# noirmist/Pytorch_Pose_Proposal_Network

Hardware: NVIDIA B200
Metric: PPN decode+NMS+parse images/s (higher is better)
Workload: dtype f32

## Files before the change

### include/ppn_decode_bench.h

```cpp
#ifndef PPN_DECODE_BENCH_H_
#define PPN_DECODE_BENCH_H_

#include "ppn_decode.h"

#ifdef __cplusplus
extern "C" {
#endif

int ppn_profile_enable(int32_t on);
int ppn_profile_read(float* stage_ms , int32_t* n_calls);

int ppn_timeline(void* dev_records, int32_t max_records);

int ppn_debug_argmax_items(const PPNShape* shape, int32_t sms, int32_t* info , int32_t* first, int32_t* size, int32_t max_items);

int ppn_tune(const char* key, int32_t value);
int ppn_tune_get(const char* key, int32_t* value);

#ifdef __cplusplus
}
#endif
#endif
```

### pytorch_pose_proposal_network_b200/_lib.py

```python
from __future__ import annotations

import ctypes as C
import os

from . import build as _build

ABI_VERSION = 7
HEAD_F32, HEAD_F16, HEAD_BF16 = 0, 1, 2
GEMM_TF32, GEMM_F16, GEMM_BF16 = 0, 1, 2
FEAT_NCHW_F32, FEAT_NHWC_16 = 0, 1
FLAG_INPUT_COMPLETE = 1
FLAG_CLEAR_UNUSED = 2
MAX_CELLS = 1024
MAX_CHAINS = 32
MAX_CHAIN_STEPS = 192
IPC_HANDLE_BYTES = 64

i32p = C.POINTER(C.c_int32)
f32p = C.POINTER(C.c_float)
u16p = C.POINTER(C.c_uint16)


class PPNShape(C.Structure):
    _fields_ = [(n, C.c_int32) for n in
                ("B", "K", "E", "H", "W", "sH", "sW", "inW", "inH", "gridW", "gridH", "off_h", "off_w", "head_dtype")]


class PPNParams(C.Structure):
    _fields_ = [("det_thresh", C.c_float), ("nms_thresh", C.c_float), ("min_num_keypoints", C.c_int32),
                ("n_nms_parts", C.c_int32), ("n_chains", C.c_int32), ("flags", C.c_int32),
                ("chain_off", i32p), ("chain_limb", i32p), ("chain_part", i32p)]


class PPNHumans(C.Structure):
    _fields_ = [("count", C.c_void_p), ("root_cell", C.c_void_p), ("part_cell", C.c_void_p),
                ("part_score", C.c_void_p), ("part_box", C.c_void_p), ("R", C.c_int32)]


class PPNHeadOptions(C.Structure):
    _fields_ = [("operand", C.c_int32), ("feat_layout", C.c_int32)]


class PPNPeople(C.Structure):
    _fields_ = [("person_off", C.c_void_p), ("bbox", C.c_void_p), ("keypoints", C.c_void_p),
                ("visible", C.c_void_p), ("size", C.c_void_p)]


TARGET_NAMES = ("delta", "weight", "weight_ij", "tx", "ty", "tx_half", "ty_half", "tw", "th", "te")


class PPNTargets(C.Structure):
    _fields_ = [(n, C.c_void_p) for n in TARGET_NAMES]


class PPNLossOptions(C.Structure):
    _fields_ = [("limb_dtype", C.c_int32)]


EXPORTS = {
    "ppn_abi_version": (C.c_int, []),
    "ppn_strerror": (C.c_char_p, [C.c_int]),
    "ppn_workspace_bytes": (C.c_int, [C.POINTER(PPNShape), C.POINTER(PPNParams), C.POINTER(C.c_size_t)]),
    "ppn_parse_launches": (C.c_int, [C.POINTER(PPNShape), C.POINTER(PPNParams)]),
    "ppn_parse_plan": (C.c_int, [C.POINTER(PPNShape), C.POINTER(PPNParams), i32p]),
    "ppn_limb_argmax": (C.c_int, [C.c_void_p, C.POINTER(PPNShape), C.c_void_p, C.c_void_p]),
    "ppn_limb_stream_probe": (C.c_int, [C.c_void_p, C.POINTER(PPNShape), C.c_void_p, C.c_int32, C.c_void_p]),
    "ppn_decode_candidates": (C.c_int, [C.c_void_p, C.POINTER(PPNShape), C.c_int32, C.c_float,
                                        C.c_void_p, C.c_void_p, C.c_void_p, C.c_void_p, C.c_void_p]),
    "ppn_restore_xy": (C.c_int, [C.c_void_p, C.c_void_p, C.c_void_p, C.c_void_p, C.c_int64, C.POINTER(PPNShape), C.c_void_p]),
    "ppn_restore_size": (C.c_int, [C.c_void_p, C.c_void_p, C.c_void_p, C.c_void_p, C.c_int64, C.POINTER(PPNShape), C.c_void_p]),
    "ppn_nms": (C.c_int, [C.c_void_p, C.c_void_p, C.c_void_p, C.c_int32, C.c_int32, C.c_float, C.c_int32,
                          C.c_void_p, C.c_void_p, C.c_void_p]),
    "ppn_tree_parse": (C.c_int, [C.c_void_p, C.POINTER(PPNShape), C.POINTER(PPNParams), C.c_void_p, C.c_void_p,
                                 C.c_void_p, C.c_void_p, C.POINTER(PPNHumans), C.c_void_p]),
    "ppn_parse": (C.c_int, [C.c_void_p, C.POINTER(PPNShape), C.POINTER(PPNParams), C.POINTER(PPNHumans),
                            C.c_void_p, C.c_size_t, C.c_void_p]),
    "ppn_parse_host_scratch_bytes": (C.c_int, [C.POINTER(PPNShape), C.POINTER(PPNParams), C.c_int32,
                                               C.POINTER(C.c_size_t)]),
    "ppn_parse_host": (C.c_int, [C.c_void_p, C.POINTER(PPNShape), C.POINTER(PPNParams), C.POINTER(PPNHumans),
                                 C.c_void_p, C.c_size_t]),
    "ppn_part_centres": (C.c_int, [C.POINTER(PPNHumans), C.c_int32, C.c_int32, C.c_void_p, C.c_void_p]),
    "ppn_skeleton": (C.c_int, [C.POINTER(PPNHumans), C.c_int32, C.c_int32, C.c_int32, i32p, C.c_void_p, C.c_void_p, C.c_void_p, C.c_void_p]),
    "ppn_packed_bytes": (C.c_int, [C.c_int32, C.c_int32, C.POINTER(C.c_size_t), C.POINTER(C.c_size_t)]),
    "ppn_pack_humans": (C.c_int, [C.POINTER(PPNHumans), C.c_int32, C.c_int32, C.c_int32, C.c_void_p, C.c_size_t, C.c_void_p]),
    "ppn_parse_dense": (C.c_int, [C.c_void_p, C.POINTER(PPNShape), C.POINTER(PPNParams), C.POINTER(PPNHumans),
                                  C.c_void_p, C.c_size_t, C.c_int32, C.c_int32, C.c_void_p, C.c_size_t, C.c_void_p]),
    "ppn_parse_dense_remote": (C.c_int, [C.c_void_p, C.POINTER(PPNShape), C.POINTER(PPNParams), C.POINTER(PPNHumans),
                                         C.c_void_p, C.c_size_t, C.c_void_p, C.c_size_t, C.c_int32, C.c_int32,
                                         C.c_void_p, C.c_size_t, C.c_void_p]),
    "ppn_peer_alloc": (C.c_int, [C.c_size_t, C.POINTER(C.c_void_p), C.c_char_p]),
    "ppn_peer_open": (C.c_int, [C.c_char_p, C.POINTER(C.c_void_p)]),
    "ppn_peer_close": (C.c_int, [C.c_void_p]),
    "ppn_peer_free": (C.c_int, [C.c_void_p]),
    "ppn_peer_copy": (C.c_int, [C.c_void_p, C.c_void_p, C.c_size_t, C.c_void_p]),
    "ppn_peer_post": (C.c_int, [C.c_void_p, C.c_longlong, C.c_void_p]),
    "ppn_peer_wait": (C.c_int, [C.c_void_p, C.c_int32, C.c_longlong, C.c_uint32, C.c_void_p, C.c_void_p]),
    "ppn_head_workspace_bytes": (C.c_int, [C.POINTER(PPNShape), C.POINTER(C.c_size_t)]),
    "ppn_head_gemm_argmax": (C.c_int, [C.c_void_p, C.c_void_p, C.c_void_p, C.c_int32, C.POINTER(PPNShape), C.c_void_p, C.c_void_p,
                                       C.c_void_p, C.c_void_p, C.c_void_p]),
    "ppn_head_parse": (C.c_int, [C.c_void_p, C.c_void_p, C.c_void_p, C.c_int32, C.POINTER(PPNShape), C.POINTER(PPNParams),
                                 C.POINTER(PPNHumans), C.c_void_p, C.c_size_t, C.c_void_p, C.c_void_p, C.c_void_p]),
    "ppn_head_workspace_bytes_opt": (C.c_int, [C.POINTER(PPNShape), C.c_int32, C.POINTER(PPNHeadOptions), C.POINTER(C.c_size_t)]),
    "ppn_head_gemm_argmax_opt": (C.c_int, [C.c_void_p, C.c_void_p, C.c_void_p, C.c_int32, C.POINTER(PPNShape), C.POINTER(PPNHeadOptions),
                                           C.c_void_p, C.c_size_t, C.c_void_p, C.c_void_p, C.c_void_p, C.c_void_p, C.c_void_p]),
    "ppn_head_parse_opt": (C.c_int, [C.c_void_p, C.c_void_p, C.c_void_p, C.c_int32, C.POINTER(PPNShape), C.POINTER(PPNParams),
                                     C.POINTER(PPNHeadOptions), C.POINTER(PPNHumans), C.c_void_p, C.c_size_t, C.c_void_p, C.c_void_p,
                                     C.c_void_p]),
    "ppn_encode_targets": (C.c_int, [C.POINTER(PPNPeople), C.POINTER(PPNShape), i32p, C.POINTER(PPNTargets), C.c_void_p]),
    "ppn_loss_workspace_bytes": (C.c_int, [C.POINTER(PPNShape), C.POINTER(C.c_size_t)]),
    "ppn_loss_forward": (C.c_int, [C.c_void_p, C.POINTER(PPNShape), C.POINTER(PPNTargets), C.c_void_p, C.c_void_p,
                                   C.c_size_t, C.c_void_p]),
    "ppn_loss_backward": (C.c_int, [C.c_void_p, C.POINTER(PPNShape), C.POINTER(PPNTargets), C.c_void_p, C.c_void_p,
                                    C.c_void_p]),
    "ppn_loss_workspace_bytes_opt": (C.c_int, [C.POINTER(PPNShape), C.POINTER(PPNLossOptions), C.POINTER(C.c_size_t)]),
    "ppn_loss_forward_opt": (C.c_int, [C.c_void_p, C.POINTER(PPNShape), C.POINTER(PPNTargets), C.POINTER(PPNLossOptions),
                                       C.c_void_p, C.c_void_p, C.c_size_t, C.c_void_p]),
    "ppn_loss_backward_opt": (C.c_int, [C.c_void_p, C.POINTER(PPNShape), C.POINTER(PPNTargets), C.POINTER(PPNLossOptions),
                                        C.c_void_p, C.c_void_p, C.c_void_p]),
    "ppn_encode_targets_opt": (C.c_int, [C.POINTER(PPNPeople), C.POINTER(PPNShape), i32p, C.POINTER(PPNTargets), C.c_int32,
                                         C.c_void_p]),
    "ppn_loss_forward_logits": (C.c_int, [C.c_void_p, C.POINTER(PPNShape), C.POINTER(PPNTargets), C.POINTER(PPNLossOptions),
                                          C.c_void_p, C.c_void_p, C.c_size_t, C.c_void_p]),
    "ppn_loss_backward_logits": (C.c_int, [C.c_void_p, C.POINTER(PPNShape), C.POINTER(PPNTargets), C.POINTER(PPNLossOptions),
                                           C.c_void_p, C.c_void_p, C.c_void_p]),
    "ppn_sigmoid": (C.c_int, [C.c_void_p, C.c_int32, C.c_void_p, C.c_size_t, C.c_void_p]),
    "ppn_debug_argmax_items": (C.c_int, [C.POINTER(PPNShape), C.c_int32, i32p, i32p, i32p, C.c_int32]),
    "ppn_timeline": (C.c_int, [C.c_void_p, C.c_int32]),
    "ppn_profile_enable": (C.c_int, [C.c_int32]),
    "ppn_profile_read": (C.c_int, [f32p, i32p]),
    "ppn_tune": (C.c_int, [C.c_char_p, C.c_int32]),
    "ppn_tune_get": (C.c_int, [C.c_char_p, i32p]),
}

_lib = None


class PPNError(RuntimeError):
    def __init__(self, code: int, where: str):
        self.code = code
        msg = lib().ppn_strerror(code)
        super().__init__(f"{where}: {msg.decode() if msg else 'error'} (code {code})")


def lib_path() -> str:
    return os.environ.get("PPN_DECODE_LIB", _build.LIB_PATH)


def lib():
    global _lib
    if _lib is not None:
        return _lib
    path = lib_path()
    if not os.path.exists(path):
        raise ImportError(
            f"{path} not found: build it with `python -m pytorch_pose_proposal_network_b200.build` "
            "(needs nvcc); this package has no CPU or PyTorch fallback")
    handle = C.CDLL(path)
    for name, (restype, argtypes) in EXPORTS.items():
        try:
            fn = getattr(handle, name)
        except AttributeError as e:
            raise ImportError(f"{path} does not export {name}") from e
        fn.restype = restype
        fn.argtypes = argtypes
    if handle.ppn_abi_version() != ABI_VERSION:
        raise ImportError(f"{path}: ABI version {handle.ppn_abi_version()} != {ABI_VERSION}")
    _lib = handle
    return _lib


def check(code: int, where: str):
    if code != 0:
        raise PPNError(code, where)


def tune(**knobs):
    for k, v in knobs.items():
        check(lib().ppn_tune(k.replace("_", ".", 1).encode(), int(v)), f"ppn_tune({k})")


def tune_get(key: str) -> int:
    v = C.c_int32()
    check(lib().ppn_tune_get(key.encode(), C.byref(v)), f"ppn_tune_get({key})")
    return v.value


STAGES = ("limb_argmax", "decode_candidates", "nms", "tree_parse")


def profile_enable(on: bool = True):
    check(lib().ppn_profile_enable(1 if on else 0), "ppn_profile_enable")


def profile_read():
    ms = (C.c_float * 4)()
    n = C.c_int32()
    check(lib().ppn_profile_read(ms, C.byref(n)), "ppn_profile_read")
    return dict(zip(STAGES, (float(v) for v in ms))), n.value
```

### pytorch_pose_proposal_network_b200/csrc/ppn_capi.cu

```cuda
#include <algorithm>
#include <cstdio>
#include <cstring>
#include <mutex>

#include "ppn_decode.h"
#include "ppn_decode_bench.h"
#include "ppn_kernels.h"

namespace {

ppn::Tuning g_tuning_shared;
std::mutex g_tune_mu;
ppn::Tuning tuning_now() {
    std::lock_guard<std::mutex> lock(g_tune_mu);
    return g_tuning_shared;
}

constexpr int kStages = 4;
constexpr int kMaxProfiled = 4096;
struct Profile {
    bool on = false;
    int used = 0;
    cudaEvent_t* ev = nullptr;
} g_prof;

inline cudaEvent_t* profile_slot() {
    if (!g_prof.on || g_prof.used >= kMaxProfiled) return nullptr;
    return g_prof.ev + (size_t)(g_prof.used++) * (2 * kStages);
}

struct SideLane {
    cudaStream_t stream = nullptr;
    cudaEvent_t fork = nullptr, join = nullptr;
};
thread_local SideLane t_side[64];

cudaError_t side_lane(SideLane** out) {
    int dev = 0;
    cudaError_t e = cudaGetDevice(&dev);
    if (e != cudaSuccess) return e;
    if (dev < 0 || dev >= 64) return cudaErrorInvalidDevice;
    SideLane& l = t_side[dev];
    if (!l.stream) {
        if ((e = cudaStreamCreateWithFlags(&l.stream, cudaStreamNonBlocking)) != cudaSuccess) return e;
        if ((e = cudaEventCreateWithFlags(&l.fork, cudaEventDisableTiming)) != cudaSuccess) return e;
        if ((e = cudaEventCreateWithFlags(&l.join, cudaEventDisableTiming)) != cudaSuccess) return e;
    }
    *out = &l;
    return cudaSuccess;
}

inline int cuda_rc(cudaError_t e) { return e == cudaSuccess ? PPN_OK : (int)e; }

struct Timeline { unsigned long long* buf = nullptr; int cap = 0, used = 0, phase = 0; } g_timeline;
inline ppn::Geom timeline_slot(ppn::Geom g) {
    if (g_timeline.buf && g_timeline.used < g_timeline.cap) { g.tl = g_timeline.buf; g.tl_slot = g_timeline.used++; g.tl_phase = g_timeline.phase; }
    else g.tl = nullptr;
    return g;
}

int check_shape(const PPNShape* s) {
    if (!s) return PPN_E_BADARG;
    if (s->B < 0 || s->K < 1 || s->E < 0 || s->H < 1 || s->W < 1 || s->sH < 1 || s->sW < 1) return PPN_E_BADARG;
    if (s->inW < 1 || s->inH < 1 || s->gridW < 0 || s->gridH < 0) return PPN_E_BADARG;
    if ((long long)s->sH * s->sW > 65535) return PPN_E_UNSUPPORTED;
    if (s->K > 255 || s->E > 255) return PPN_E_UNSUPPORTED;
    const long long per_img = ((long long)6 * s->K + (long long)s->sH * s->sW * s->E) * s->H * s->W;
    if (per_img > 0x7fffffffLL) return PPN_E_UNSUPPORTED;
    if (s->head_dtype < PPN_HEAD_F32 || s->head_dtype > PPN_HEAD_BF16) return PPN_E_BADARG;
    return PPN_OK;
}

ppn::Geom make_geom(const PPNShape* s) {
    ppn::Geom g;
    g.B = s->B; g.K = s->K; g.E = s->E; g.H = s->H; g.W = s->W; g.HW = s->H * s->W;
    g.sH = s->sH; g.sW = s->sW; g.S = s->sH * s->sW; g.C = 6 * s->K + g.S * s->E;
    g.off_h = s->off_h; g.off_w = s->off_w;
    g.gridW = (float)s->gridW; g.gridH = (float)s->gridH; g.inW = (float)s->inW; g.inH = (float)s->inH;
    g.img_stride = (size_t)g.C * g.HW;
    g.limb_off = (size_t)6 * g.K * g.HW;
    g.tl = nullptr;
    g.tl_slot = 0;
    g.tl_phase = 0;
    auto magic = [](int d) -> uint32_t { return d <= 1 ? 0u : (uint32_t)(((1ull << 32) + d - 1) / d); };
    g.magic_W = magic(g.W);
    g.magic_K = magic(g.K);
    g.dtype = s->head_dtype;
    return g;
}

int make_chains(const PPNShape* s, const PPNParams* p, ppn::ChainTable* ch) {
    if (!p) return PPN_E_BADARG;
    if (p->n_chains < 0 || p->n_chains > PPN_MAX_CHAINS) return PPN_E_CHAINS;
    if (p->n_chains > 0 && (!p->chain_off || !p->chain_limb || !p->chain_part)) return PPN_E_BADARG;
    std::memset(ch, 0, sizeof(*ch));
    ch->n_chains = p->n_chains;
    if (p->n_chains == 0) return PPN_OK;
    if (p->chain_off[0] != 0) return PPN_E_CHAINS;
    for (int c = 0; c < p->n_chains; ++c)
        if (p->chain_off[c + 1] < p->chain_off[c]) return PPN_E_CHAINS;
    const int total = p->chain_off[p->n_chains];
    if (total > PPN_MAX_CHAIN_STEPS) return PPN_E_CHAINS;
    for (int c = 0; c <= p->n_chains; ++c) ch->off[c] = (uint8_t)p->chain_off[c];
    for (int q = 0; q < total; ++q) {
        if (p->chain_limb[q] < 0 || p->chain_limb[q] >= s->E || p->chain_part[q] < 0 || p->chain_part[q] >= s->K)
            return PPN_E_CHAINS;
        ch->limb[q] = (uint8_t)p->chain_limb[q];
        ch->part[q] = (uint8_t)p->chain_part[q];
    }
    int limb_of[256], pred_of[256];
    for (int t = 0; t < 256; ++t) limb_of[t] = pred_of[t] = -1;
    ch->parallel_ok = 1;
    for (int c = 0; c < p->n_chains && ch->parallel_ok; ++c)
        for (int q = p->chain_off[c]; q < p->chain_off[c + 1]; ++q) {
            const int t = p->chain_part[q], e = p->chain_limb[q];
            const int pred = q == p->chain_off[c] ? 0 : p->chain_part[q - 1];
            if (t == 0) { ch->parallel_ok = 0; break; }
            if (limb_of[t] < 0) { limb_of[t] = e; pred_of[t] = pred; }
            else if (limb_of[t] != e || pred_of[t] != pred) { ch->parallel_ok = 0; break; }
        }
    return PPN_OK;
}

inline size_t elem_bytes(const PPNShape* s) { return s->head_dtype == PPN_HEAD_F32 ? 4 : 2; }
inline bool misaligned(const void* p, const PPNShape* s) { return (reinterpret_cast<uintptr_t>(p) & (elem_bytes(s) - 1)) != 0; }

inline size_t align_up(size_t v, size_t a) { return (v + a - 1) / a * a; }

struct Workspace {
    size_t amax, keep_idx, keep_count, total;
};

Workspace carve(const PPNShape* s, int n_parts) {
    Workspace w;
    const size_t B = (size_t)s->B, HW = (size_t)s->H * s->W, P = (size_t)n_parts;
    size_t off = 0;
    auto take = [&](size_t bytes) { const size_t at = off; off = align_up(off + bytes, 256); return at; };
    w.amax = take(B * s->E * HW * sizeof(uint16_t));
    w.keep_idx = take(B * P * HW * sizeof(int32_t));
    w.keep_count = take(B * P * sizeof(int32_t));
    w.total = off;
    return w;
}


int check_params(const PPNShape* s, const PPNParams* p) {
    if (!p) return PPN_E_BADARG;
    if (p->n_nms_parts < 1 || p->n_nms_parts > s->K) return PPN_E_BADARG;
    return PPN_OK;
}

int check_humans(const PPNHumans* h) {
    if (!h || !h->count || !h->root_cell || !h->part_cell || !h->part_score || !h->part_box || h->R < 1) return PPN_E_BADARG;
    return PPN_OK;
}

}

namespace {
struct PackedLayout { size_t header, idcell, score, box, total; };
PackedLayout packed_layout(int B, int cap) {
    PackedLayout l;
    l.header = 0;
    l.idcell = align_up((size_t)(2 + 3 * (size_t)B) * sizeof(int32_t), 256);
    l.score = l.idcell + align_up((size_t)cap * sizeof(uint32_t), 256);
    l.box = l.score + align_up((size_t)cap * sizeof(float), 256);
    l.total = l.box + align_up((size_t)cap * 4 * sizeof(float), 256);
    return l;
}
}

namespace {
int pack_after(const PPNHumans* out, const PPNShape* shape, const ppn::DenseTarget* d, cudaStream_t st) {
    if (out->R > 65536) return PPN_E_UNSUPPORTED;
    return cuda_rc(ppn::launch_pack_humans(out->count, out->part_cell, out->part_score, out->part_box, shape->B, out->R,
                                           shape->K, d->cap, d->header, d->idcell, d->score, d->box, st));
}
}

extern "C" {

int ppn_abi_version(void) { return PPN_ABI_VERSION; }

const char* ppn_strerror(int code) {
    switch (code) {
        case PPN_OK: return "ok";
        case PPN_E_BADARG: return "ppn: bad argument (null pointer, non-positive size or misaligned base)";
        case PPN_E_UNSUPPORTED: return "ppn: shape not supported by the kernels";
        case PPN_E_WORKSPACE: return "ppn: workspace smaller than ppn_workspace_bytes()";
        case PPN_E_CHAINS: return "ppn: track orders too long or indexing outside K/E";
        case PPN_E_NO_DEVICE: return "ppn: no usable CUDA device";
        default: break;
    }
    if (code > 0) return cudaGetErrorString((cudaError_t)code);
    return "ppn: unknown error";
}

int ppn_tune(const char* key, int32_t value) {
    if (!key) return PPN_E_BADARG;
    std::lock_guard<std::mutex> lock(g_tune_mu);
    ppn::Tuning& t = g_tuning_shared;
    if (!std::strcmp(key, "argmax.variant")) t.argmax_variant = value;
    else if (!std::strcmp(key, "argmax.stage_bytes")) t.argmax_stage_bytes = value <= 0 ? 0 : (value < 1024 ? 1024 : value);
    else if (!std::strcmp(key, "argmax.stages")) t.argmax_stages = value < 2 ? 2 : (value > 32 ? 32 : value);
    else if (!std::strcmp(key, "argmax.threads")) t.argmax_threads = value < 32 ? 32 : (value > 992 ? 992 : value);
    else if (!std::strcmp(key, "argmax.ctas_per_sm")) t.argmax_ctas_per_sm = value < 1 ? 1 : (value > 8 ? 8 : value);
    else if (!std::strcmp(key, "argmax.split")) t.argmax_split = value;
    else if (!std::strcmp(key, "argmax.cluster")) t.argmax_cluster = value;
    else if (!std::strcmp(key, "argmax.cluster_ring")) t.argmax_cluster_ring = value != 0;
    else if (!std::strcmp(key, "argmax.smem_cap")) t.argmax_smem_cap = value < 0 ? 0 : value;
    else if (!std::strcmp(key, "parse.overlap")) t.parse_overlap = value < 0 ? 0 : (value > 2 ? 2 : value);
    else if (!std::strcmp(key, "argmax.tail_opt")) t.argmax_tail_opt = value < 0 ? 0 : (value > 8 ? 8 : value);
    else if (!std::strcmp(key, "argmax16.threads")) t.argmax16_threads = value < 32 ? 32 : (value > 992 ? 992 : value);
    else if (!std::strcmp(key, "argmax16.stage_bytes")) t.argmax16_stage_bytes = value < 1024 ? 1024 : value;
    else if (!std::strcmp(key, "argmax.dynamic")) t.argmax_dynamic = value != 0;
    else if (!std::strcmp(key, "parse.stage_all")) t.parse_stage_all = value;
    else if (!std::strcmp(key, "parse.chain_calls")) t.parse_chain_calls = value != 0;
    else if (!std::strcmp(key, "parse.persist")) t.parse_persist = value < 0 ? 0 : (value > 4 ? 4 : value);
    else if (!std::strcmp(key, "parse.k12_threads")) t.parse_k12_threads = value < 0 ? 0 : value;
    else if (!std::strcmp(key, "parse.fused")) t.parse_fused = value < 0 ? -1 : (value != 0);
    else if (!std::strcmp(key, "parse.threads")) t.parse_threads = value;
    else if (!std::strcmp(key, "head.subs")) t.head_subs = (t.head_subs & 0x1300) | (value < 1 ? 0 : (value > 7 ? 7 : value));
    else if (!std::strcmp(key, "head.dry")) t.head_subs = (t.head_subs & 0x10ff) | ((value & 3) << 8);
    else if (!std::strcmp(key, "head.acc")) t.head_subs = (t.head_subs & 0x3ff) | (value == 128 ? 0x1000 : 0);
    else if (!std::strcmp(key, "host.chunk_images")) t.host_chunk_images = value < 1 ? 1 : value;
    else if (!std::strcmp(key, "encode.sweep")) t.encode_sweep = value != 0;
    else if (!std::strcmp(key, "encode.ctas_per_sm")) t.encode_ctas_per_sm = value < 1 ? 1 : (value > 8 ? 8 : value);
    else if (!std::strcmp(key, "nms.blockwise")) ppn::set_nms_blockwise(value);
    else if (!std::strcmp(key, "timeline.phase")) g_timeline.phase = value;
    else return PPN_E_BADARG;
    return PPN_OK;
}

int ppn_tune_get(const char* key, int32_t* value) {
    if (!key || !value) return PPN_E_BADARG;
    const ppn::Tuning t = tuning_now();
    if (!std::strcmp(key, "argmax.variant")) *value = t.argmax_variant;
    else if (!std::strcmp(key, "argmax.stage_bytes")) *value = t.argmax_stage_bytes;
    else if (!std::strcmp(key, "argmax.stages")) *value = t.argmax_stages;
    else if (!std::strcmp(key, "argmax.threads")) *value = t.argmax_threads;
    else if (!std::strcmp(key, "argmax.ctas_per_sm")) *value = t.argmax_ctas_per_sm;
    else if (!std::strcmp(key, "argmax.split")) *value = t.argmax_split;
    else if (!std::strcmp(key, "argmax.cluster")) *value = t.argmax_cluster;
    else if (!std::strcmp(key, "argmax.cluster_ring")) *value = t.argmax_cluster_ring;
    else if (!std::strcmp(key, "argmax.smem_cap")) *value = t.argmax_smem_cap;
    else if (!std::strcmp(key, "parse.overlap")) *value = t.parse_overlap;
    else if (!std::strcmp(key, "argmax.tail_opt")) *value = t.argmax_tail_opt;
    else if (!std::strcmp(key, "argmax16.threads")) *value = t.argmax16_threads;
    else if (!std::strcmp(key, "argmax16.stage_bytes")) *value = t.argmax16_stage_bytes;
    else if (!std::strcmp(key, "argmax.dynamic")) *value = t.argmax_dynamic;
    else if (!std::strcmp(key, "parse.stage_all")) *value = t.parse_stage_all;
    else if (!std::strcmp(key, "parse.chain_calls")) *value = t.parse_chain_calls;
    else if (!std::strcmp(key, "parse.persist")) *value = t.parse_persist;
    else if (!std::strcmp(key, "parse.k12_threads")) *value = t.parse_k12_threads;
    else if (!std::strcmp(key, "parse.fused")) *value = t.parse_fused;
    else if (!std::strcmp(key, "parse.threads")) *value = t.parse_threads;
    else if (!std::strcmp(key, "host.chunk_images")) *value = t.host_chunk_images;
    else if (!std::strcmp(key, "encode.sweep")) *value = t.encode_sweep;
    else if (!std::strcmp(key, "encode.ctas_per_sm")) *value = t.encode_ctas_per_sm;
    else if (!std::strcmp(key, "nms.blockwise")) *value = ppn::get_nms_blockwise();
    else return PPN_E_BADARG;
    return PPN_OK;
}

int ppn_workspace_bytes(const PPNShape* shape, const PPNParams* params, size_t* bytes) {
    int rc = check_shape(shape);
    if (rc) return rc;
    if ((rc = check_params(shape, params))) return rc;
    if (!bytes) return PPN_E_BADARG;
    *bytes = 2 * carve(shape, params->n_nms_parts).total;
    return PPN_OK;
}

int ppn_parse_launches(const PPNShape* shape, const PPNParams* params) {
    const ppn::Tuning g_tuning = tuning_now();
    if (check_shape(shape) || check_params(shape, params)) return 0;
    if (shape->B <= 0) return 0;
    const ppn::Geom g = make_geom(shape);
    ppn::FusedSplit split;
    const bool P1 = params->n_nms_parts == 1 && g_tuning.parse_overlap != 1;
    const bool fits = P1 && ppn::parse_fused_split(g, g_tuning.parse_stage_all, g_tuning, &split);
    const bool fused = P1 && (g_tuning.parse_fused < 0 ? (fits && split.n_sub == 1) : (g_tuning.parse_fused != 0 && ppn::parse_fused_supported(g, g_tuning.parse_stage_all)));
    if (fused) return 2 * (fits ? split.n_sub : 1);
    return 3;
}

int ppn_parse_plan(const PPNShape* shape, const PPNParams* params, int32_t* info) {
    const ppn::Tuning g_tuning = tuning_now();
    if (!info) return PPN_E_BADARG;
    int rc = check_shape(shape);
    if (rc) return rc;
    if ((rc = check_params(shape, params))) return rc;
    info[0] = ppn_parse_launches(shape, params);
    info[1] = 1; info[2] = 0; info[3] = 0;
    if (shape->B <= 0) return PPN_OK;
    ppn::FusedSplit split;
    if (params->n_nms_parts == 1 && ppn::parse_fused_split(make_geom(shape), g_tuning.parse_stage_all, g_tuning, &split)) {
        info[1] = split.n_sub;
        info[2] = (int32_t)split.ring_cap;
        info[3] = split.staged ? 1 : 0;
    }
    return PPN_OK;
}

int ppn_limb_argmax(const void* head, const PPNShape* shape, uint16_t* amax, void* stream) {
    const ppn::Tuning g_tuning = tuning_now();
    int rc = check_shape(shape);
    if (rc) return rc;
    if (shape->B == 0 || shape->E == 0) return PPN_OK;
    if (!head || !amax) return PPN_E_BADARG;
    if (misaligned(head, shape)) return PPN_E_BADARG;
    return cuda_rc(ppn::launch_limb_argmax(head, amax, make_geom(shape), g_tuning, (cudaStream_t)stream));
}

int ppn_limb_stream_probe(const void* head, const PPNShape* shape, uint16_t* amax, int32_t smem_cap, void* stream) {
    const ppn::Tuning g_tuning = tuning_now();
    int rc = check_shape(shape);
    if (rc) return rc;
    if (shape->B == 0 || shape->E == 0) return PPN_OK;
    if (!head || !amax) return PPN_E_BADARG;
    if (misaligned(head, shape)) return PPN_E_BADARG;
    ppn::Tuning t = g_tuning;
    t.argmax_dry = 1;
    t.argmax_cluster = 0;
    if (smem_cap > 0) t.argmax_smem_cap = smem_cap;
    return cuda_rc(ppn::launch_limb_argmax(head, amax, make_geom(shape), t, (cudaStream_t)stream));
}

int ppn_decode_candidates(const void* head, const PPNShape* shape, int32_t n_parts, float det_thresh,
                          int32_t* cand_cell, float* cand_score, float* cand_box, int32_t* cand_count, void* stream) {
    int rc = check_shape(shape);
    if (rc) return rc;
    if (n_parts < 1 || n_parts > shape->K) return PPN_E_BADARG;
    if (shape->B == 0) return PPN_OK;
    if (!head || !cand_cell || !cand_score || !cand_box || !cand_count) return PPN_E_BADARG;
    if (reinterpret_cast<uintptr_t>(cand_box) & 15) return PPN_E_BADARG;
    return cuda_rc(ppn::launch_decode_candidates(head, make_geom(shape), n_parts, det_thresh, cand_cell, cand_score,
                                                 cand_box, cand_count, (cudaStream_t)stream));
}

int ppn_restore_xy(const float* x, const float* y, float* rx, float* ry, int64_t n_planes, const PPNShape* shape, void* stream) {
    int rc = check_shape(shape);
    if (rc) return rc;
    if (n_planes < 0) return PPN_E_BADARG;
    if (n_planes == 0) return PPN_OK;
    if (!x || !y || !rx || !ry) return PPN_E_BADARG;
    return cuda_rc(ppn::launch_restore_xy(x, y, rx, ry, (size_t)n_planes * shape->H * shape->W, shape->H, shape->W,
                                          (float)shape->gridW, (float)shape->gridH, (cudaStream_t)stream));
}

int ppn_restore_size(const float* w, const float* h, float* rw, float* rh, int64_t n_planes, const PPNShape* shape, void* stream) {
    int rc = check_shape(shape);
    if (rc) return rc;
    if (n_planes < 0) return PPN_E_BADARG;
    if (n_planes == 0) return PPN_OK;
    if (!w || !h || !rw || !rh) return PPN_E_BADARG;
    return cuda_rc(ppn::launch_restore_size(w, h, rw, rh, (size_t)n_planes * shape->H * shape->W, (float)shape->inW,
                                            (float)shape->inH, (cudaStream_t)stream));
}

int ppn_nms(const float* box, const float* score, const int32_t* count, int32_t n_problems, int32_t stride,
            float nms_thresh, int32_t limit, int32_t* keep_idx, int32_t* keep_count, void* stream) {
    if (n_problems < 0 || stride < 1) return PPN_E_BADARG;
    if (n_problems == 0) return PPN_OK;
    if (!box || !count || !keep_idx || !keep_count) return PPN_E_BADARG;
    if (reinterpret_cast<uintptr_t>(box) & 15) return PPN_E_BADARG;
    return cuda_rc(ppn::launch_nms(box, score, count, n_problems, stride, nms_thresh, limit, keep_idx, keep_count,
                                   (cudaStream_t)stream));
}

int ppn_tree_parse(const void* head, const PPNShape* shape, const PPNParams* params, const uint16_t* amax,
                   const int32_t* cand_cell, const int32_t* keep_idx, const int32_t* keep_count,
                   const PPNHumans* out, void* stream) {
    int rc = check_shape(shape);
    if (rc) return rc;
    if ((rc = check_params(shape, params))) return rc;
    if ((rc = check_humans(out))) return rc;
    ppn::ChainTable ch;
    if ((rc = make_chains(shape, params, &ch))) return rc;
    if (shape->B == 0) return PPN_OK;
    if (!head || !keep_idx || !keep_count || (!amax && shape->E > 0)) return PPN_E_BADARG;
    if ((long long)shape->H * shape->W > PPN_MAX_CELLS) return PPN_E_UNSUPPORTED;
    if (reinterpret_cast<uintptr_t>(out->part_box) & 15) return PPN_E_BADARG;
    return cuda_rc(ppn::launch_tree_parse(head, make_geom(shape), ch, params->det_thresh, params->min_num_keypoints,
                                          params->n_nms_parts, amax, cand_cell, keep_idx, keep_count, out->count,
                                          out->root_cell, out->part_cell, out->part_score, out->part_box, out->R,
                                          (cudaStream_t)stream));
}

namespace {
__global__ void peer_post_kernel(long long* counter, long long value) {
    __threadfence_system();
    asm volatile("st.release.sys.global.u64 [%0], %1;" :: "l"(counter), "l"(value) : "memory");
}
__global__ void peer_wait_kernel(const long long* counters, int n, long long target, unsigned long long timeout_ns, int* timed_out) {
    const int r = threadIdx.x;
    if (r >= n) return;
    unsigned long long t0, t;
    asm volatile("mov.u64 %0, %%globaltimer;" : "=l"(t0));
    for (;;) {
        long long v;
        asm volatile("ld.acquire.sys.global.u64 %0, [%1];" : "=l"(v) : "l"(counters + r) : "memory");
        if (v >= target) return;
        asm volatile("mov.u64 %0, %%globaltimer;" : "=l"(t));
        if (t - t0 > timeout_ns) { if (timed_out) *timed_out = 1; return; }
        __nanosleep(200);
    }
}
}

int ppn_peer_post(void* counter, long long value, void* stream) {
    if (!counter || (reinterpret_cast<uintptr_t>(counter) & 7)) return PPN_E_BADARG;
    peer_post_kernel<<<1, 1, 0, (cudaStream_t)stream>>>(static_cast<long long*>(counter), value);
    return cuda_rc(cudaGetLastError());
}

int ppn_peer_wait(const void* counters, int32_t n, long long target, uint32_t timeout_ms, int32_t* timed_out, void* stream) {
    if (!counters || n < 1 || n > 1024 || (reinterpret_cast<uintptr_t>(counters) & 7)) return PPN_E_BADARG;
    peer_wait_kernel<<<1, (n + 31) / 32 * 32, 0, (cudaStream_t)stream>>>(static_cast<const long long*>(counters), n, target,
                                                                      (unsigned long long)timeout_ms * 1000000ull, timed_out);
    return cuda_rc(cudaGetLastError());
}

static int parse_impl(const void* head, const PPNShape* shape, const PPNParams* params, const PPNHumans* out,
                      void* workspace, size_t workspace_bytes, void* stream, const ppn::DenseTarget* dense);

int ppn_parse(const void* head, const PPNShape* shape, const PPNParams* params, const PPNHumans* out,
              void* workspace, size_t workspace_bytes, void* stream) {
    return parse_impl(head, shape, params, out, workspace, workspace_bytes, stream, nullptr);
}

int ppn_parse_dense(const void* head, const PPNShape* shape, const PPNParams* params, const PPNHumans* out,
                    void* packed, size_t packed_bytes, int32_t cap_entries, int32_t skip_slots,
                    void* workspace, size_t workspace_bytes, void* stream) {
    int rc = check_shape(shape);
    if (rc) return rc;
    if (cap_entries < 0) return PPN_E_BADARG;
    if (shape->K > 65535 || (long long)shape->H * shape->W > 65536) return PPN_E_UNSUPPORTED;
    if (shape->B == 0) return PPN_OK;
    if (!packed || (reinterpret_cast<uintptr_t>(packed) & 255)) return PPN_E_BADARG;
    const PackedLayout l = packed_layout(shape->B, cap_entries);
    if (packed_bytes < l.total) return PPN_E_WORKSPACE;
    unsigned char* p = static_cast<unsigned char*>(packed);
    ppn::DenseTarget d;
    d.header = reinterpret_cast<int32_t*>(p + l.header);
    d.idcell = reinterpret_cast<uint32_t*>(p + l.idcell);
    d.score = reinterpret_cast<float*>(p + l.score);
    d.box = reinterpret_cast<float*>(p + l.box);
    d.cap = cap_entries;
    d.skip_slots = skip_slots != 0;
    return parse_impl(head, shape, params, out, workspace, workspace_bytes, stream, &d);
}

int ppn_parse_dense_remote(const void* head, const PPNShape* shape, const PPNParams* params, const PPNHumans* out,
                           void* local_header, size_t local_header_bytes, void* remote_packed, size_t remote_bytes,
                           int32_t cap_entries, int32_t skip_slots, void* workspace, size_t workspace_bytes, void* stream) {
    int rc = check_shape(shape);
    if (rc) return rc;
    if (cap_entries < 0) return PPN_E_BADARG;
    if (shape->K > 32 || (long long)shape->H * shape->W > PPN_MAX_CELLS) return PPN_E_UNSUPPORTED;
    if (shape->B == 0) return PPN_OK;
    if (!local_header || !remote_packed || (reinterpret_cast<uintptr_t>(local_header) & 255) ||
        (reinterpret_cast<uintptr_t>(remote_packed) & 255)) return PPN_E_BADARG;
    const PackedLayout l = packed_layout(shape->B, cap_entries);
    if (remote_bytes < l.total || local_header_bytes < (size_t)(2 + 3 * (size_t)shape->B) * sizeof(int32_t)) return PPN_E_WORKSPACE;
    unsigned char* p = static_cast<unsigned char*>(remote_packed);
    ppn::DenseTarget d;
    d.header = static_cast<int32_t*>(local_header);
    d.rheader = reinterpret_cast<int32_t*>(p + l.header);
    d.idcell = reinterpret_cast<uint32_t*>(p + l.idcell);
    d.score = reinterpret_cast<float*>(p + l.score);
    d.box = reinterpret_cast<float*>(p + l.box);
    d.cap = cap_entries;
    d.skip_slots = skip_slots != 0;
    return parse_impl(head, shape, params, out, workspace, workspace_bytes, stream, &d);
}

int ppn_peer_alloc(size_t bytes, void** dev_ptr, unsigned char* handle) {
    if (!dev_ptr || !handle || bytes == 0) return PPN_E_BADARG;
    static_assert(sizeof(cudaIpcMemHandle_t) == PPN_IPC_HANDLE_BYTES, "IPC handle size");
    void* p = nullptr;
    cudaError_t e = cudaMalloc(&p, bytes);
    if (e != cudaSuccess) return (int)e;
    if ((e = cudaMemset(p, 0, bytes)) != cudaSuccess) { cudaFree(p); return (int)e; }
    cudaIpcMemHandle_t h;
    if ((e = cudaIpcGetMemHandle(&h, p)) != cudaSuccess) { cudaFree(p); return (int)e; }
    std::memcpy(handle, &h, sizeof(h));
    *dev_ptr = p;
    return PPN_OK;
}

int ppn_peer_open(const unsigned char* handle, void** dev_ptr) {
    if (!dev_ptr || !handle) return PPN_E_BADARG;
    cudaIpcMemHandle_t h;
    std::memcpy(&h, handle, sizeof(h));
    return cuda_rc(cudaIpcOpenMemHandle(dev_ptr, h, cudaIpcMemLazyEnablePeerAccess));
}

int ppn_peer_close(void* dev_ptr) { return dev_ptr ? cuda_rc(cudaIpcCloseMemHandle(dev_ptr)) : PPN_E_BADARG; }
int ppn_peer_free(void* dev_ptr) { return dev_ptr ? cuda_rc(cudaFree(dev_ptr)) : PPN_E_BADARG; }

int ppn_peer_copy(void* dst, const void* src, size_t bytes, void* stream) {
    if (!dst || !src) return PPN_E_BADARG;
    if (bytes == 0) return PPN_OK;
    return cuda_rc(cudaMemcpyAsync(dst, src, bytes, cudaMemcpyDefault, (cudaStream_t)stream));
}

static int parse_impl(const void* head, const PPNShape* shape, const PPNParams* params, const PPNHumans* out,
                      void* workspace, size_t workspace_bytes, void* stream, const ppn::DenseTarget* dense) {
    const ppn::Tuning g_tuning = tuning_now();
    int rc = check_shape(shape);
    if (rc) return rc;
    if ((rc = check_params(shape, params))) return rc;
    if ((rc = check_humans(out))) return rc;
    ppn::ChainTable ch;
    if ((rc = make_chains(shape, params, &ch))) return rc;
    if (shape->B == 0) return PPN_OK;
    if (!head || !workspace) return PPN_E_BADARG;
    if (misaligned(head, shape) || (reinterpret_cast<uintptr_t>(workspace) & 255)) return PPN_E_BADARG;
    if ((long long)shape->H * shape->W > PPN_MAX_CELLS) return PPN_E_UNSUPPORTED;
    if (reinterpret_cast<uintptr_t>(out->part_box) & 15) return PPN_E_BADARG;
    const int P = params->n_nms_parts;
    const Workspace w = carve(shape, P);
    if (workspace_bytes < 2 * w.total) return PPN_E_WORKSPACE;
    unsigned char* ws = static_cast<unsigned char*>(workspace) + (ppn::next_call_parity((cudaStream_t)stream) ? w.total : 0);
    uint16_t* amax = reinterpret_cast<uint16_t*>(ws + w.amax);
    int32_t* keep_idx = reinterpret_cast<int32_t*>(ws + w.keep_idx);
    int32_t* keep_count = reinterpret_cast<int32_t*>(ws + w.keep_count);
    const ppn::Geom g = make_geom(shape);
    cudaStream_t st = (cudaStream_t)stream;
    cudaError_t e;
    if ((params->flags & PPN_FLAG_CLEAR_UNUSED) && !(dense && dense->skip_slots)) {
        const size_t slots = (size_t)shape->B * out->R, SK = slots * shape->K;
        if ((e = cudaMemsetAsync(out->root_cell, 0xFF, slots * sizeof(int32_t), st)) != cudaSuccess) return (int)e;
        if ((e = cudaMemsetAsync(out->part_cell, 0xFF, SK * sizeof(int32_t), st)) != cudaSuccess) return (int)e;
        if ((e = cudaMemsetAsync(out->part_score, 0, SK * sizeof(float), st)) != cudaSuccess) return (int)e;
        if ((e = cudaMemsetAsync(out->part_box, 0, SK * 4 * sizeof(float), st)) != cudaSuccess) return (int)e;
        ppn::chain_break(st);
    }
    cudaEvent_t* ev = profile_slot();
    const int mode = ev ? 0 : g_tuning.parse_overlap;
    ppn::FusedSplit split;
    const bool fits_beside = P == 1 && ppn::parse_fused_split(g, g_tuning.parse_stage_all, g_tuning, &split);
    const bool fused = P == 1 && mode != 1 && (g_tuning.parse_fused < 0 ? (fits_beside && split.n_sub == 1) : (g_tuning.parse_fused != 0 &&
                       ppn::parse_fused_supported(g, g_tuning.parse_stage_all)));
    const bool dense_fused = dense && fused && shape->K <= 32;
    if (dense && dense->rheader && !dense_fused) return PPN_E_UNSUPPORTED;
    if (fused) {
        using namespace ppn;
        Tuning tuning = g_tuning;
        const int n_sub = fits_beside ? split.n_sub : 1;
        const int sub_B = fits_beside ? split.sub_B : g.B;
        const int staged_forced = fits_beside ? (split.staged ? 1 : 0) : -1;
        if (fits_beside) tuning.argmax_smem_cap = (int)split.ring_cap;
        const bool overlap_calls = (params->flags & PPN_FLAG_INPUT_COMPLETE) != 0;
        const bool chain = mode == 2 && g_tuning.parse_chain_calls != 0;
        cudaStreamCaptureStatus cap = cudaStreamCaptureStatusNone;
        if ((e = cudaStreamIsCapturing(st, &cap)) != cudaSuccess) return (int)e;
        const bool capturing = cap != cudaStreamCaptureStatusNone;
        const size_t es = elem_bytes(shape);
        const size_t K = (size_t)shape->K, R = (size_t)out->R;
        auto launch_k3 = [&](int j) -> cudaError_t {
            Geom gj = timeline_slot(g);
            const int b0 = j * sub_B;
            gj.B = std::min(sub_B, g.B - b0);
            const bool attr = chain && (j > 0 || !overlap_calls || capturing || chain_clean(st));
            const int bits = mode != 2 ? 0 : ((overlap_calls || j > 0) ? (PDL_TRIGGER | PDL_WAIT_END) : (PDL_WAIT_START | PDL_TRIGGER));
            bool chained = false, zeroed = false;
            int32_t* zero2 = (dense_fused && j == 0) ? dense->header : nullptr;
            cudaError_t err = launch_limb_argmax(static_cast<const unsigned char*>(head) + (size_t)b0 * g.img_stride * es,
                                                 amax + (size_t)b0 * g.E * g.HW, gj, tuning, st, attr, &chained, bits, zero2, &zeroed);
            if (err == cudaSuccess && zero2 && !zeroed) err = cudaMemsetAsync(dense->header, 0, 2 * sizeof(int32_t), st);
            return err;
        };
        auto launch_k124 = [&](int j) -> cudaError_t {
            Geom gj = timeline_slot(g);
            const int b0 = j * sub_B;
            gj.B = std::min(sub_B, g.B - b0);
            DenseTarget dj;
            if (dense_fused) { dj = *dense; dj.B_total = g.B; dj.b0 = b0; }
            return launch_parse_fused(static_cast<const unsigned char*>(head) + (size_t)b0 * g.img_stride * es, gj, ch,
                                      params->det_thresh, params->nms_thresh, params->min_num_keypoints,
                                      amax + (size_t)b0 * g.E * g.HW, out->count + b0, out->root_cell + (size_t)b0 * R,
                                      out->part_cell + (size_t)b0 * R * K, out->part_score + (size_t)b0 * R * K,
                                      out->part_box + (size_t)b0 * R * K * 4, out->R, st,
                                      mode == 2 ,
                                      (overlap_calls && chain && !capturing) ? 2 : 1, g_tuning.parse_stage_all, staged_forced,
                                      dense_fused ? &dj : nullptr);
        };
        if (ev) {
            cudaEventRecord(ev[0], st);
            for (int j = 0; j < n_sub; ++j) if ((e = launch_k3(j)) != cudaSuccess) return (int)e;
            cudaEventRecord(ev[1], st);
            for (int q = 2; q < 7; ++q) cudaEventRecord(ev[q], st);
            for (int j = 0; j < n_sub; ++j) if ((e = launch_k124(j)) != cudaSuccess) return (int)e;
            cudaEventRecord(ev[7], st);
        } else {
            for (int j = 0; j < n_sub; ++j) {
                if ((e = launch_k3(j)) != cudaSuccess) return (int)e;
                if ((e = launch_k124(j)) != cudaSuccess) return (int)e;
            }
        }
        if (dense && !dense_fused) return pack_after(out, shape, dense, st);
        return PPN_OK;
    }
    if (dense && dense->rheader) return PPN_E_UNSUPPORTED;
    if (mode == 2) {
        using namespace ppn;
        const bool overlap_calls = (params->flags & PPN_FLAG_INPUT_COMPLETE) != 0;
        const bool chain_calls = g_tuning.parse_chain_calls != 0;
        cudaStreamCaptureStatus cap = cudaStreamCaptureStatusNone;
        if ((e = cudaStreamIsCapturing(st, &cap)) != cudaSuccess) return (int)e;
        const bool capturing = cap != cudaStreamCaptureStatusNone;
        Tuning tuning = g_tuning;
        int k12_ctas = g_tuning.parse_persist, k4_ctas = g_tuning.parse_persist > 0 ? 1 : 0;
        if (k12_ctas > 0) {
            const size_t ring_cap = chain3_ring_cap(g, g_tuning.parse_stage_all, k12_ctas);
            if (ring_cap) tuning.argmax_smem_cap = (int)ring_cap;
            else k12_ctas = k4_ctas = 0;
        }
        const bool early = overlap_calls && chain_calls && !capturing && k4_ctas > 0;
        const bool attr12 = chain_calls && (!overlap_calls || capturing || chain_clean(st));
        const int bits12 = PDL_TRIGGER | (!attr12 ? 0 : (overlap_calls ? PDL_WAIT_END : PDL_WAIT_START));
        bool chained = false;
        if ((e = launch_decode_nms(head, timeline_slot(g), P, params->det_thresh, params->nms_thresh, keep_idx, keep_count, st, attr12,
                                   bits12, k12_ctas, g_tuning.parse_k12_threads)) != cudaSuccess) return (int)e;
        if ((e = launch_limb_argmax(head, amax, timeline_slot(g), tuning, st, true, &chained)) != cudaSuccess) return (int)e;
        if ((e = launch_tree_parse(head, timeline_slot(g), ch, params->det_thresh, params->min_num_keypoints, P, amax, nullptr, keep_idx,
                                   keep_count, out->count, out->root_cell, out->part_cell, out->part_score, out->part_box,
                                   out->R, st, chained, chained ? (PDL_WAIT_START | PDL_TRIGGER) : 0, g_tuning.parse_stage_all,
                                   g_tuning.parse_threads, chained ? (early ? 2 : 1) : 0, k4_ctas)) != cudaSuccess) return (int)e;
        if (!chained) chain_break(st);
        if (!dense) return PPN_OK;
        rc = pack_after(out, shape, dense, st);
        chain_break(st);
        return rc;
    }
    ppn::chain_break(st);
    cudaStream_t side = st;
    SideLane* lane = nullptr;
    if (mode == 1) {
        if ((e = side_lane(&lane)) != cudaSuccess) return (int)e;
        side = lane->stream;
        if ((e = cudaEventRecord(lane->fork, st)) != cudaSuccess) return (int)e;
        if ((e = cudaStreamWaitEvent(side, lane->fork, 0)) != cudaSuccess) return (int)e;
    }
    if (ev) cudaEventRecord(ev[0], st);
    if ((e = ppn::launch_limb_argmax(head, amax, g, g_tuning, st)) != cudaSuccess) return (int)e;
    if (ev) cudaEventRecord(ev[1], st);
    if (ev) { cudaEventRecord(ev[2], side); cudaEventRecord(ev[3], side); cudaEventRecord(ev[4], side); }
    if ((e = ppn::launch_decode_nms(head, g, P, params->det_thresh, params->nms_thresh, keep_idx, keep_count, side)) != cudaSuccess) return (int)e;
    if (ev) cudaEventRecord(ev[5], side);
    if (lane) {
        if ((e = cudaEventRecord(lane->join, side)) != cudaSuccess) return (int)e;
        if ((e = cudaStreamWaitEvent(st, lane->join, 0)) != cudaSuccess) return (int)e;
    }
    if (ev) cudaEventRecord(ev[6], st);
    if ((e = ppn::launch_tree_parse(head, g, ch, params->det_thresh, params->min_num_keypoints, P, amax, nullptr ,
                                    keep_idx, keep_count, out->count, out->root_cell, out->part_cell, out->part_score,
                                    out->part_box, out->R, st, false, 0, g_tuning.parse_stage_all, g_tuning.parse_threads)) != cudaSuccess) return (int)e;
    if (ev) cudaEventRecord(ev[7], st);
    return dense ? pack_after(out, shape, dense, st) : PPN_OK;
}

namespace {
struct HeadWorkspace { size_t dec, amax, keys, total; };
HeadWorkspace carve_head(const PPNShape* s) {
    HeadWorkspace w;
    const size_t B = (size_t)s->B, HW = (size_t)s->H * s->W;
    w.dec = 0;
    w.amax = align_up(B * 6 * s->K * HW * sizeof(float), 256);
    w.keys = w.amax + align_up(B * s->E * HW * sizeof(uint16_t), 256);
    w.total = w.keys + align_up(B * s->E * HW * sizeof(unsigned long long), 256);
    return w;
}
int check_head(const float* feat, const float* weight, int32_t Cin, const PPNShape* s) {
    if ((long long)s->H * s->W > 65536) return PPN_E_UNSUPPORTED;
    if (Cin < 32 || Cin % 32 != 0 || (s->H * s->W) % 4 != 0) return PPN_E_UNSUPPORTED;
    if (s->head_dtype != PPN_HEAD_F32) return PPN_E_UNSUPPORTED;
    if (!feat || !weight) return PPN_E_BADARG;
    if ((reinterpret_cast<uintptr_t>(feat) & 15) || (reinterpret_cast<uintptr_t>(weight) & 15)) return PPN_E_BADARG;
    return PPN_OK;
}
}

int ppn_head_workspace_bytes(const PPNShape* shape, size_t* bytes) {
    int rc = check_shape(shape);
    if (rc) return rc;
    if (!bytes) return PPN_E_BADARG;
    *bytes = carve_head(shape).total;
    return PPN_OK;
}

int ppn_head_gemm_argmax(const float* feat, const float* weight, const float* bias, int32_t Cin, const PPNShape* shape,
                         float* dec, uint16_t* amax, float* emit_logits, float* emit_head, void* stream) {
    const ppn::Tuning g_tuning = tuning_now();
    int rc = check_shape(shape);
    if (rc) return rc;
    if (shape->B == 0) return PPN_OK;
    if ((rc = check_head(feat, weight, Cin, shape))) return rc;
    if (!dec || (!amax && shape->E > 0) || (reinterpret_cast<uintptr_t>(bias) & 15)) return PPN_E_BADARG;
    const ppn::Geom g = make_geom(shape);
    cudaStream_t st = (cudaStream_t)stream;
    void* keys = nullptr;
    cudaError_t e = cudaMallocAsync(&keys, std::max<size_t>(ppn::head_keys_bytes(g), 256), st);
    if (e != cudaSuccess) return cuda_rc(e);
    e = ppn::launch_head_gemm_argmax(feat, weight, bias, Cin, g, dec, amax, static_cast<unsigned long long*>(keys), emit_logits,
                                     emit_head, st, false, 0, g_tuning.head_subs);
    const cudaError_t e2 = cudaFreeAsync(keys, st);
    return cuda_rc(e != cudaSuccess ? e : e2);
}

namespace {
struct HeadWorkspaceOpt { size_t dec, amax, keys, xt, wt, total; };
bool opt_16bit(const PPNHeadOptions* o) { return o->operand == PPN_GEMM_F16 || o->operand == PPN_GEMM_BF16; }
int check_head_opt(const void* feat, const float* weight, int32_t Cin, const PPNShape* s, const PPNHeadOptions* o) {
    if (!o) return PPN_E_BADARG;
    if (o->operand < PPN_GEMM_TF32 || o->operand > PPN_GEMM_BF16) return PPN_E_BADARG;
    if (o->feat_layout != PPN_FEAT_NCHW_F32 && o->feat_layout != PPN_FEAT_NHWC_16) return PPN_E_BADARG;
    if (!opt_16bit(o) && o->feat_layout != PPN_FEAT_NCHW_F32) return PPN_E_UNSUPPORTED;
    if (s->B == 0) return PPN_OK;
    if (!opt_16bit(o)) return check_head(static_cast<const float*>(feat), weight, Cin, s);
    if (s->head_dtype != PPN_HEAD_F32) return PPN_E_UNSUPPORTED;
    if (!ppn::head16_supported(Cin, make_geom(s))) return PPN_E_UNSUPPORTED;
    if (!feat || !weight) return PPN_E_BADARG;
    if ((reinterpret_cast<uintptr_t>(feat) & 15) || (reinterpret_cast<uintptr_t>(weight) & 15)) return PPN_E_BADARG;
    return PPN_OK;
}
HeadWorkspaceOpt carve_head_opt(const PPNShape* s, int32_t Cin, const PPNHeadOptions* o) {
    const HeadWorkspace w = carve_head(s);
    HeadWorkspaceOpt r;
    r.dec = w.dec; r.amax = w.amax; r.keys = w.keys; r.xt = r.wt = r.total = w.total;
    if (opt_16bit(o)) {
        const ppn::Geom g = make_geom(s);
        r.wt = r.xt + (o->feat_layout == PPN_FEAT_NCHW_F32 ? align_up(ppn::head16_packed_feat_bytes(Cin, g), 1024) : 0);
        r.total = r.wt + align_up(ppn::head16_packed_weight_bytes(Cin, g), 1024);
    }
    return r;
}
}

int ppn_head_workspace_bytes_opt(const PPNShape* shape, int32_t Cin, const PPNHeadOptions* opt, size_t* bytes) {
    int rc = check_shape(shape);
    if (rc) return rc;
    if (!bytes || !opt || Cin < 1) return PPN_E_BADARG;
    *bytes = carve_head_opt(shape, Cin, opt).total;
    return PPN_OK;
}

int ppn_head_gemm_argmax_opt(const void* feat, const float* weight, const float* bias, int32_t Cin, const PPNShape* shape,
                             const PPNHeadOptions* opt, void* workspace, size_t workspace_bytes,
                             float* dec, uint16_t* amax, float* emit_logits, float* emit_head, void* stream) {
    int rc = check_shape(shape);
    if (rc) return rc;
    if ((rc = check_head_opt(feat, weight, Cin, shape, opt))) return rc;
    if (!opt_16bit(opt))
        return ppn_head_gemm_argmax(static_cast<const float*>(feat), weight, bias, Cin, shape, dec, amax, emit_logits, emit_head, stream);
    if (shape->B == 0) return PPN_OK;
    if (!dec || (!amax && shape->E > 0) || (reinterpret_cast<uintptr_t>(bias) & 15)) return PPN_E_BADARG;
    if (!workspace || (reinterpret_cast<uintptr_t>(workspace) & 255)) return PPN_E_BADARG;
    const HeadWorkspaceOpt w = carve_head_opt(shape, Cin, opt);
    if (workspace_bytes < w.total) return PPN_E_WORKSPACE;
    unsigned char* ws = static_cast<unsigned char*>(workspace);
    return cuda_rc(ppn::launch_head_gemm16_argmax(feat, opt->feat_layout == PPN_FEAT_NCHW_F32, weight, bias, Cin,
                                                  opt->operand == PPN_GEMM_BF16, make_geom(shape), ws + w.xt, ws + w.wt, dec, amax,
                                                  reinterpret_cast<unsigned long long*>(ws + w.keys), emit_logits, emit_head,
                                                  (cudaStream_t)stream, 0, tuning_now().head_subs));
}

int ppn_head_parse_opt(const void* feat, const float* weight, const float* bias, int32_t Cin, const PPNShape* shape,
                       const PPNParams* params, const PPNHeadOptions* opt, const PPNHumans* out, void* workspace,
                       size_t workspace_bytes, float* emit_logits, float* emit_head, void* stream) {
    const ppn::Tuning g_tuning = tuning_now();
    int rc = check_shape(shape);
    if (rc) return rc;
    if ((rc = check_params(shape, params))) return rc;
    if ((rc = check_humans(out))) return rc;
    ppn::ChainTable ch;
    if ((rc = make_chains(shape, params, &ch))) return rc;
    if ((rc = check_head_opt(feat, weight, Cin, shape, opt))) return rc;
    if (shape->B == 0) return PPN_OK;
    if (!workspace || (reinterpret_cast<uintptr_t>(workspace) & 255)) return PPN_E_BADARG;
    if (params->n_nms_parts != 1 || (long long)shape->H * shape->W > PPN_MAX_CELLS) return PPN_E_UNSUPPORTED;
    if ((reinterpret_cast<uintptr_t>(out->part_box) & 15) || (reinterpret_cast<uintptr_t>(bias) & 15)) return PPN_E_BADARG;
// ... 125 lines not shown
    a.sweep = g_tuning.encode_sweep;
    a.sweep_ctas_per_sm = g_tuning.encode_ctas_per_sm;
    a.magic_sW = shape->sW <= 1 ? 0u : (uint32_t)(((1ull << 32) + shape->sW - 1) / shape->sW);
    a.gridW = (float)shape->gridW; a.gridH = (float)shape->gridH;
    a.inW = (double)shape->inW; a.inH = (double)shape->inH;
    int dev = 0, sms = 0;
    cudaError_t e = cudaGetDevice(&dev);
    if (e != cudaSuccess) return (int)e;
    if ((e = cudaDeviceGetAttribute(&sms, cudaDevAttrMultiProcessorCount, dev)) != cudaSuccess) return (int)e;
    return cuda_rc(ppn::launch_encode_targets(a, shape->B, sms, (cudaStream_t)stream));
}

namespace {
inline bool bad_ptr(const void* p, size_t align) { return !p || (reinterpret_cast<uintptr_t>(p) & (align - 1)); }
inline bool bad_f32(const void* p) { return bad_ptr(p, 4); }
inline size_t dtype_bytes(int32_t dtype) { return dtype == PPN_HEAD_F32 ? 4 : 2; }

int check_loss_types(const PPNShape* shape, const PPNLossOptions* opt) {
    if (!opt || opt->limb_dtype < PPN_HEAD_F32 || opt->limb_dtype > PPN_HEAD_BF16) return PPN_E_BADARG;
    if (opt->limb_dtype != PPN_HEAD_F32 && opt->limb_dtype != shape->head_dtype) return PPN_E_UNSUPPORTED;
    return PPN_OK;
}

int loss_args(const void* head, const PPNShape* shape, const PPNTargets* t, const PPNLossOptions* opt, ppn::LossArgs* a) {
    int rc = check_shape(shape);
    if (rc) return rc;
    if ((rc = check_loss_types(shape, opt))) return rc;
    if (shape->B < 1) return PPN_E_BADARG;
    std::memset(a, 0, sizeof(*a));
    const ppn::Geom g = make_geom(shape);
    a->B = g.B; a->K = g.K; a->W = g.W; a->HW = g.HW; a->L = g.S * g.E * g.HW;
    a->img_stride = g.img_stride; a->limb_off = g.limb_off;
    a->gW = g.gridW; a->gH = g.gridH; a->inW = g.inW; a->inH = g.inH;
    a->head_dtype = shape->head_dtype;
    a->limb_dtype = opt->limb_dtype;
    ppn::loss_plan(a);
    if (!t) return PPN_E_BADARG;
    const float* small[] = {t->delta, t->weight, t->tx, t->ty, t->tx_half, t->ty_half, t->tw, t->th};
    for (const float* p : small)
        if (bad_f32(p)) return PPN_E_BADARG;
    const size_t limb_align = dtype_bytes(opt->limb_dtype);
    if (bad_ptr(head, elem_bytes(shape)) || (a->L > 0 && (bad_ptr(t->te, limb_align) || bad_ptr(t->weight_ij, limb_align))))
        return PPN_E_BADARG;
    a->head = head;
    a->delta = t->delta; a->weight = t->weight; a->weight_ij = t->weight_ij; a->tx = t->tx; a->ty = t->ty;
    a->tx_half = t->tx_half; a->ty_half = t->ty_half; a->tw = t->tw; a->th = t->th; a->te = t->te;
    return PPN_OK;
}

int sm_count(int* sms) {
    int dev = 0;
    cudaError_t e = cudaGetDevice(&dev);
    if (e == cudaSuccess) e = cudaDeviceGetAttribute(sms, cudaDevAttrMultiProcessorCount, dev);
    return cuda_rc(e);
}

const PPNLossOptions kLossF32 = {PPN_HEAD_F32};
int check_f32_loss(const PPNShape* shape) {
    int rc = check_shape(shape);
    if (rc) return rc;
    return shape->head_dtype != PPN_HEAD_F32 ? PPN_E_UNSUPPORTED : PPN_OK;
}
}

int ppn_loss_workspace_bytes_opt(const PPNShape* shape, const PPNLossOptions* opt, size_t* bytes) {
    int rc = check_shape(shape);
    if (rc) return rc;
    if (!bytes) return PPN_E_BADARG;
    if ((rc = check_loss_types(shape, opt))) return rc;
    if (shape->B < 1) return PPN_E_BADARG;
    ppn::LossArgs a;
    std::memset(&a, 0, sizeof(a));
    a.B = shape->B; a.K = shape->K; a.HW = shape->H * shape->W; a.L = shape->sH * shape->sW * shape->E * a.HW;
    ppn::loss_plan(&a);
    *bytes = ppn::loss_workspace_bytes(a);
    return PPN_OK;
}

int ppn_loss_workspace_bytes(const PPNShape* shape, size_t* bytes) {
    int rc = check_shape(shape);
    if (rc) return rc;
    if (!bytes) return PPN_E_BADARG;
    if ((rc = check_f32_loss(shape))) return rc;
    return ppn_loss_workspace_bytes_opt(shape, &kLossF32, bytes);
}

namespace {
int loss_forward(const void* head, const PPNShape* shape, const PPNTargets* targets, const PPNLossOptions* opt,
                 float* loss, void* workspace, size_t workspace_bytes, void* stream, bool from_logits) {
    ppn::LossArgs a;
    int rc = loss_args(head, shape, targets, opt, &a);
    if (rc) return rc;
    if (bad_f32(loss) || !workspace || (reinterpret_cast<uintptr_t>(workspace) & 7)) return PPN_E_BADARG;
    if (workspace_bytes < ppn::loss_workspace_bytes(a)) return PPN_E_WORKSPACE;
    a.partial = static_cast<double*>(workspace);
    int sms = 0;
    if ((rc = sm_count(&sms))) return rc;
    return cuda_rc(ppn::launch_loss_forward(a, loss, sms, (cudaStream_t)stream, from_logits));
}

int loss_backward(const void* head, const PPNShape* shape, const PPNTargets* targets, const PPNLossOptions* opt,
                  const float* grad_loss, void* grad_head, void* stream, bool from_logits) {
    ppn::LossArgs a;
    int rc = loss_args(head, shape, targets, opt, &a);
    if (rc) return rc;
    if (bad_f32(grad_loss) || bad_ptr(grad_head, elem_bytes(shape))) return PPN_E_BADARG;
    a.grad_loss = grad_loss;
    a.grad = grad_head;
    int sms = 0;
    if ((rc = sm_count(&sms))) return rc;
    return cuda_rc(ppn::launch_loss_backward(a, sms, (cudaStream_t)stream, from_logits));
}
}

int ppn_loss_forward_opt(const void* head, const PPNShape* shape, const PPNTargets* targets, const PPNLossOptions* opt,
                         float* loss, void* workspace, size_t workspace_bytes, void* stream) {
    return loss_forward(head, shape, targets, opt, loss, workspace, workspace_bytes, stream, false);
}

int ppn_loss_forward(const float* head, const PPNShape* shape, const PPNTargets* targets, float* loss,
                     void* workspace, size_t workspace_bytes, void* stream) {
    const int rc = check_f32_loss(shape);
    return rc ? rc : ppn_loss_forward_opt(head, shape, targets, &kLossF32, loss, workspace, workspace_bytes, stream);
}

int ppn_loss_backward_opt(const void* head, const PPNShape* shape, const PPNTargets* targets, const PPNLossOptions* opt,
                          const float* grad_loss, void* grad_head, void* stream) {
    return loss_backward(head, shape, targets, opt, grad_loss, grad_head, stream, false);
}

int ppn_loss_backward(const float* head, const PPNShape* shape, const PPNTargets* targets, const float* grad_loss,
                      float* grad_head, void* stream) {
    const int rc = check_f32_loss(shape);
    return rc ? rc : ppn_loss_backward_opt(head, shape, targets, &kLossF32, grad_loss, grad_head, stream);
}

int ppn_loss_forward_logits(const void* logits, const PPNShape* shape, const PPNTargets* targets, const PPNLossOptions* opt,
                            float* loss, void* workspace, size_t workspace_bytes, void* stream) {
    return loss_forward(logits, shape, targets, opt, loss, workspace, workspace_bytes, stream, true);
}

int ppn_loss_backward_logits(const void* logits, const PPNShape* shape, const PPNTargets* targets, const PPNLossOptions* opt,
                             const float* grad_loss, void* grad_logits, void* stream) {
    return loss_backward(logits, shape, targets, opt, grad_loss, grad_logits, stream, true);
}

int ppn_sigmoid(const void* x, int32_t x_dtype, float* y, size_t n, void* stream) {
    if (x_dtype < PPN_HEAD_F32 || x_dtype > PPN_HEAD_BF16) return PPN_E_BADARG;
    if (n == 0) return PPN_OK;
    if (bad_ptr(x, dtype_bytes(x_dtype)) || bad_f32(y)) return PPN_E_BADARG;
    return cuda_rc(ppn::launch_sigmoid(x, x_dtype, y, n, (cudaStream_t)stream));
}

int ppn_debug_argmax_items(const PPNShape* shape, int32_t sms, int32_t* info, int32_t* first, int32_t* size, int32_t max_items) {
    int rc = check_shape(shape);
    if (rc) return rc;
    if (!info || sms < 1) return PPN_E_BADARG;
    const ppn::Tuning g_tuning = tuning_now();
    ppn::ArgmaxPlan p;
    if (!ppn::plan_argmax(make_geom(shape), g_tuning, sms, &p) || !p.split_mats) return PPN_E_UNSUPPORTED;
    struct Ctx { int32_t* first; int32_t* size; int32_t max; } ctx = {first, size, max_items};
    int n_items = 0;
    ppn::argmax_item_partition(p, shape->B * shape->E, &n_items, [](void* c, int it, int m0, int nm) -> int {
        Ctx* x = static_cast<Ctx*>(c);
        if (x->first && x->size && it < x->max) { x->first[it] = m0; x->size[it] = nm; }
        return 0;
    }, &ctx);
    info[0] = p.G; info[1] = p.n_big; info[2] = p.small_m; info[3] = n_items;
    return PPN_OK;
}

int ppn_timeline(void* dev_records, int32_t max_records) {
    g_timeline.buf = static_cast<unsigned long long*>(dev_records);
    g_timeline.cap = dev_records ? max_records : 0;
    g_timeline.used = 0;
    return PPN_OK;
}

int ppn_profile_enable(int32_t on) {
    if (on && !g_prof.ev) {
        g_prof.ev = new cudaEvent_t[(size_t)kMaxProfiled * (2 * kStages)];
        for (size_t i = 0; i < (size_t)kMaxProfiled * (2 * kStages); ++i) {
            cudaError_t e = cudaEventCreate(&g_prof.ev[i]);
            if (e != cudaSuccess) return (int)e;
        }
    }
    g_prof.on = on != 0;
    g_prof.used = 0;
    return PPN_OK;
}

int ppn_profile_read(float* stage_ms, int32_t* n_calls) {
    if (!stage_ms || !n_calls) return PPN_E_BADARG;
    for (int s = 0; s < kStages; ++s) stage_ms[s] = 0.0f;
    *n_calls = g_prof.used;
    for (int c = 0; c < g_prof.used; ++c) {
        cudaEvent_t* ev = g_prof.ev + (size_t)c * (2 * kStages);
        cudaError_t e = cudaEventSynchronize(ev[2 * kStages - 1]);
        if (e != cudaSuccess) return (int)e;
        for (int s = 0; s < kStages; ++s) {
            float ms = 0.0f;
            if ((e = cudaEventElapsedTime(&ms, ev[2 * s], ev[2 * s + 1])) != cudaSuccess) return (int)e;
            stage_ms[s] += ms;
        }
    }
    g_prof.used = 0;
    return PPN_OK;
}

namespace {
struct HostPlan {
    int chunk;
    size_t head_bytes;
    size_t ws_bytes;
    size_t off_head[2], off_ws[2], off_count, off_root, off_cell, off_score, off_box, total;
};
HostPlan plan_host(const PPNShape* s, const PPNParams* p, int R) {
    const ppn::Tuning g_tuning = tuning_now();
    HostPlan h;
    h.chunk = g_tuning.host_chunk_images;
    if (h.chunk > s->B) h.chunk = s->B > 0 ? s->B : 1;
    PPNShape cs = *s;
    cs.B = h.chunk;
    const size_t per_img = ((size_t)6 * s->K + (size_t)s->sH * s->sW * s->E) * s->H * s->W * elem_bytes(s);
    h.head_bytes = align_up(per_img * h.chunk, 256);
    h.ws_bytes = 2 * carve(&cs, p->n_nms_parts).total;
    size_t off = 0;
    auto take = [&](size_t bytes) { const size_t at = off; off = align_up(off + bytes, 256); return at; };
    h.off_head[0] = take(h.head_bytes); h.off_head[1] = take(h.head_bytes);
    h.off_ws[0] = take(h.ws_bytes); h.off_ws[1] = take(h.ws_bytes);
    const size_t B = (size_t)s->B, K = (size_t)s->K;
    h.off_count = take(B * sizeof(int32_t));
    h.off_root = take(B * R * sizeof(int32_t));
    h.off_cell = take(B * R * K * sizeof(int32_t));
    h.off_score = take(B * R * K * sizeof(float));
    h.off_box = take(B * R * K * 4 * sizeof(float));
    h.total = off;
    return h;
}
}

int ppn_parse_host_scratch_bytes(const PPNShape* shape, const PPNParams* params, int32_t R, size_t* bytes) {
    int rc = check_shape(shape);
    if (rc) return rc;
    if ((rc = check_params(shape, params))) return rc;
    if (!bytes || R < 1) return PPN_E_BADARG;
    *bytes = plan_host(shape, params, R).total;
    return PPN_OK;
}

int ppn_parse_host(const void* head_host, const PPNShape* shape, const PPNParams* params, const PPNHumans* out_host,
                   void* dev_scratch, size_t dev_scratch_bytes) {
    int rc = check_shape(shape);
    if (rc) return rc;
    if ((rc = check_params(shape, params))) return rc;
    if ((rc = check_humans(out_host))) return rc;
    if (shape->B == 0) return PPN_OK;
    if (!head_host || !dev_scratch || (reinterpret_cast<uintptr_t>(dev_scratch) & 255)) return PPN_E_BADARG;
    const int R = out_host->R;
    const HostPlan h = plan_host(shape, params, R);
    if (dev_scratch_bytes < h.total) return PPN_E_WORKSPACE;
    unsigned char* d = static_cast<unsigned char*>(dev_scratch);
    const size_t K = (size_t)shape->K;
    const size_t per_img_b = ((size_t)6 * shape->K + (size_t)shape->sH * shape->sW * shape->E) * shape->H * shape->W * elem_bytes(shape);

    struct HostLane { cudaStream_t s[2] = {nullptr, nullptr}; };
    static thread_local HostLane t_lanes[64];
    int dev = 0;
    cudaError_t e = cudaGetDevice(&dev);
    if (e != cudaSuccess) return (int)e;
    if (dev < 0 || dev >= 64) return (int)cudaErrorInvalidDevice;
    cudaStream_t* streams = t_lanes[dev].s;
    for (int i = 0; i < 2; ++i)
        if (!streams[i] && (e = cudaStreamCreateWithFlags(&streams[i], cudaStreamNonBlocking)) != cudaSuccess) return (int)e;
    auto fail = [&](int code) { cudaStreamSynchronize(streams[0]); cudaStreamSynchronize(streams[1]); return code; };

    int32_t* d_count = reinterpret_cast<int32_t*>(d + h.off_count);
    int32_t* d_root = reinterpret_cast<int32_t*>(d + h.off_root);
    int32_t* d_cell = reinterpret_cast<int32_t*>(d + h.off_cell);
    float* d_score = reinterpret_cast<float*>(d + h.off_score);
    float* d_box = reinterpret_cast<float*>(d + h.off_box);

    PPNParams chunk_params = *params;
    chunk_params.flags &= ~PPN_FLAG_INPUT_COMPLETE;
    int slot = 0;
    for (int b0 = 0; b0 < shape->B; b0 += h.chunk, slot ^= 1) {
        const int nb = (shape->B - b0 < h.chunk) ? shape->B - b0 : h.chunk;
        cudaStream_t st = streams[slot];
        void* d_head = d + h.off_head[slot];
        if ((e = cudaMemcpyAsync(d_head, static_cast<const unsigned char*>(head_host) + (size_t)b0 * per_img_b,
                                 (size_t)nb * per_img_b, cudaMemcpyHostToDevice, st)) != cudaSuccess) return fail((int)e);
        PPNShape cs = *shape;
        cs.B = nb;
        PPNHumans dev_out;
        dev_out.count = d_count + b0;
        dev_out.root_cell = d_root + (size_t)b0 * R;
        dev_out.part_cell = d_cell + (size_t)b0 * R * K;
        dev_out.part_score = d_score + (size_t)b0 * R * K;
        dev_out.part_box = d_box + (size_t)b0 * R * K * 4;
        dev_out.R = R;
        if ((rc = ppn_parse(d_head, &cs, &chunk_params, &dev_out, d + h.off_ws[slot], h.ws_bytes, st))) return fail(rc);
        if ((e = cudaMemcpyAsync(out_host->count + b0, dev_out.count, (size_t)nb * sizeof(int32_t), cudaMemcpyDeviceToHost, st)) != cudaSuccess) return fail((int)e);
    }
    for (int i = 0; i < 2; ++i)
        if ((e = cudaStreamSynchronize(streams[i])) != cudaSuccess) return (int)e;
    int m = 0;
    for (int b = 0; b < shape->B; ++b) m = std::max(m, std::min(out_host->count[b], R));
    if (m > 0) {
        cudaStream_t st = streams[0];
        const size_t B = (size_t)shape->B;
        if ((e = cudaMemcpy2DAsync(out_host->root_cell, (size_t)R * 4, d_root, (size_t)R * 4, (size_t)m * 4, B, cudaMemcpyDeviceToHost, st)) != cudaSuccess) return fail((int)e);
        if ((e = cudaMemcpy2DAsync(out_host->part_cell, (size_t)R * K * 4, d_cell, (size_t)R * K * 4, (size_t)m * K * 4, B, cudaMemcpyDeviceToHost, st)) != cudaSuccess) return fail((int)e);
        if ((e = cudaMemcpy2DAsync(out_host->part_score, (size_t)R * K * 4, d_score, (size_t)R * K * 4, (size_t)m * K * 4, B, cudaMemcpyDeviceToHost, st)) != cudaSuccess) return fail((int)e);
        if ((e = cudaMemcpy2DAsync(out_host->part_box, (size_t)R * K * 16, d_box, (size_t)R * K * 16, (size_t)m * K * 16, B, cudaMemcpyDeviceToHost, st)) != cudaSuccess) return fail((int)e);
        if ((e = cudaStreamSynchronize(st)) != cudaSuccess) return (int)e;
    }
    if ((params->flags & PPN_FLAG_CLEAR_UNUSED) && m < R) {
        const size_t tail = (size_t)(R - m);
        for (size_t b = 0; b < (size_t)shape->B; ++b) {
            const size_t s = b * R + m;
            std::fill_n(out_host->root_cell + s, tail, -1);
            std::fill_n(out_host->part_cell + s * K, tail * K, -1);
            std::fill_n(out_host->part_score + s * K, tail * K, 0.0f);
            std::fill_n(out_host->part_box + s * K * 4, tail * K * 4, 0.0f);
        }
    }
    return PPN_OK;
}
// ... 3 lines not shown
```

### pytorch_pose_proposal_network_b200/csrc/ppn_device.cuh

```cuda
#pragma once
#include <cuda_bf16.h>
#include <cuda_fp16.h>
#include <cuda_runtime.h>
#include <stdint.h>

namespace ppn {

struct ChainTable {
    int32_t n_chains;
    int32_t parallel_ok;
    uint8_t off[33];
    uint8_t limb[192];
    uint8_t part[192];
};

struct Geom {
    int32_t B, K, E, H, W, HW, sH, sW, S, C;
    int32_t off_h, off_w;
    float gridW, gridH, inW, inH;
    size_t img_stride;
    size_t limb_off;
    uint32_t magic_W, magic_K;
    int32_t dtype;
    unsigned long long* tl;
    int32_t tl_slot;
    int32_t tl_phase;
};

enum : int { TL_START = 0, TL_END = 1, TL_WAITED = 2 };
__device__ __forceinline__ void tl_mark(const Geom& g, int what) {
    if (g.tl && threadIdx.x == 0) {
        unsigned long long t;
        asm volatile("mov.u64 %0, %%globaltimer;" : "=l"(t));
        unsigned long long* rec = g.tl + 4 * (size_t)g.tl_slot;
        if (what == TL_END) atomicMax(rec + 1, t); else atomicMin(rec + what, t);
    }
}

__device__ __forceinline__ void tl_phase(const Geom& g, int phase) {
    if (g.tl && threadIdx.x == 0 && g.tl_phase == phase) {
        unsigned long long t;
        asm volatile("mov.u64 %0, %%globaltimer;" : "=l"(t));
        if (phase >= 100) atomicMax(g.tl + 4 * (size_t)g.tl_slot + 3, t);
        else atomicMin(g.tl + 4 * (size_t)g.tl_slot + 3, t);
    }
}

__device__ __forceinline__ void tl_phase_warp(const Geom& g, int phase) {
    if (g.tl && (threadIdx.x & 31) == 0 && g.tl_phase == phase) {
        unsigned long long t;
        asm volatile("mov.u64 %0, %%globaltimer;" : "=l"(t));
        atomicMin(g.tl + 4 * (size_t)g.tl_slot + 3, t);
    }
}

enum HeadDtype : int { HEAD_F32 = 0, HEAD_F16 = 1, HEAD_BF16 = 2 };

__device__ __forceinline__ float widen(float v) { return v; }
__device__ __forceinline__ float widen(__half v) { return __half2float(v); }
__device__ __forceinline__ float widen(__nv_bfloat16 v) { return __bfloat162float(v); }

template <typename T>
__device__ __forceinline__ float ldf(const T* p) { return widen(__ldg(p)); }

template <typename T> __device__ __forceinline__ T narrow(float v) { return v; }
template <> __device__ __forceinline__ __half narrow<__half>(float v) { return __float2half_rn(v); }
template <> __device__ __forceinline__ __nv_bfloat16 narrow<__nv_bfloat16>(float v) { return __float2bfloat16_rn(v); }
__device__ __forceinline__ uint32_t bits16(__half v) { return __half_as_ushort(v); }
__device__ __forceinline__ uint32_t bits16(__nv_bfloat16 v) { return __bfloat16_as_ushort(v); }
template <typename T> __device__ __forceinline__ uint32_t pack2(float lo, float hi) {
    return bits16(narrow<T>(lo)) | (bits16(narrow<T>(hi)) << 16);
}

__device__ __forceinline__ float sigmoid_f32(float x) { return __fdiv_rn(1.0f, __fadd_rn(1.0f, expf(-x))); }

template <typename T>
__device__ __forceinline__ float delta_at(const T* __restrict__ img, const Geom& g, int k, int c) {
    return __fmul_rn(ldf(img + (size_t)k * g.HW + c), ldf(img + (size_t)(g.K + k) * g.HW + c));
}

__device__ __forceinline__ float4 box_from(float x, float y, float bw, float bh, int h, int w, const Geom& g) {
    const float rx = __fmul_rn(__fadd_rn(x, (float)w), g.gridW);
    const float ry = __fmul_rn(__fadd_rn(y, (float)h), g.gridH);
    const float hw = __fmul_rn(__fmul_rn(g.inW, bw), 0.5f);
    const float hh = __fmul_rn(__fmul_rn(g.inH, bh), 0.5f);
    return make_float4(__fsub_rn(ry, hh), __fsub_rn(rx, hw), __fadd_rn(ry, hh), __fadd_rn(rx, hw));
}

template <typename T>
__device__ __forceinline__ float4 box_at(const T* __restrict__ img, const Geom& g, int k, int c) {
    const int h = c / g.W, w = c - h * g.W;
    const size_t HW = g.HW;
    return box_from(ldf(img + (size_t)(2 * g.K + k) * HW + c), ldf(img + (size_t)(3 * g.K + k) * HW + c),
                    ldf(img + (size_t)(4 * g.K + k) * HW + c), ldf(img + (size_t)(5 * g.K + k) * HW + c), h, w, g);
}

__device__ __forceinline__ float np_max(float a, float b) { return (a >= b || a != a) ? a : b; }
__device__ __forceinline__ float np_min(float a, float b) { return (a <= b || a != a) ? a : b; }

__device__ __forceinline__ bool suppresses(const float4 tested, float area_tested,
                                           const float4 kept, float area_kept, float thr, bool thr_positive) {
    const float tly = np_max(tested.x, kept.x), tlx = np_max(tested.y, kept.y);
    const float bry = np_min(tested.z, kept.z), brx = np_min(tested.w, kept.w);
    const bool overlap = tly < bry && tlx < brx;
    if (thr_positive && !overlap) return false;
    const float prod = __fmul_rn(__fsub_rn(bry, tly), __fsub_rn(brx, tlx));
    const float inter = __fmul_rn(prod, overlap ? 1.0f : 0.0f);
    const float iou = __fdiv_rn(inter, __fsub_rn(__fadd_rn(area_tested, area_kept), inter));
    return iou >= thr;
}

__device__ __forceinline__ float box_area(const float4 b) {
    return __fmul_rn(__fsub_rn(b.z, b.x), __fsub_rn(b.w, b.y));
}

__device__ __forceinline__ void argmax_step(float& best, int& idx, float v, int a) {
    const bool take = !(v <= best) && (best == best);
    best = take ? v : best;
    idx = take ? a : idx;
}

__device__ __forceinline__ bool argmax_beats(float v2, int i2, float v1, int i1) {
    const bool n1 = v1 != v1, n2 = v2 != v2;
    if (n1 || n2) return n2 && (!n1 || i2 < i1);
    return v2 > v1 || (v2 == v1 && i2 < i1);
}

__device__ __forceinline__ uint32_t smem_u32(const void* p) {
    return static_cast<uint32_t>(__cvta_generic_to_shared(p));
}
__device__ __forceinline__ void mbar_init(uint64_t* bar, uint32_t count) {
    asm volatile("mbarrier.init.shared::cta.b64 [%0], %1;" ::"r"(smem_u32(bar)), "r"(count) : "memory");
}
__device__ __forceinline__ void fence_mbar_init() {
    asm volatile("fence.mbarrier_init.release.cluster;" ::: "memory");
}
__device__ __forceinline__ void mbar_arrive_expect_tx(uint64_t* bar, uint32_t bytes) {
    asm volatile("mbarrier.arrive.expect_tx.shared::cta.b64 _, [%0], %1;" ::"r"(smem_u32(bar)), "r"(bytes) : "memory");
}
__device__ __forceinline__ void mbar_arrive(uint64_t* bar) {
    asm volatile("mbarrier.arrive.shared::cta.b64 _, [%0];" ::"r"(smem_u32(bar)) : "memory");
}
__device__ __forceinline__ void mbar_wait(uint64_t* bar, uint32_t parity) {
    asm volatile(
        "{\n"
        ".reg .pred p;\n"
        "PPN_WAIT:\n"
        "mbarrier.try_wait.parity.shared::cta.b64 p, [%0], %1;\n"
        "@p bra PPN_DONE;\n"
        "bra PPN_WAIT;\n"
        "PPN_DONE:\n"
        "}" ::"r"(smem_u32(bar)), "r"(parity) : "memory");
}
__device__ __forceinline__ void bulk_g2s(void* dst_smem, const void* src_gmem, uint32_t bytes, uint64_t* bar) {
    const uint64_t evict_first = 0x12F0000000000000ull;
    asm volatile(
        "cp.async.bulk.shared::cluster.global.mbarrier::complete_tx::bytes.L2::cache_hint [%0], [%1], %2, [%3], %4;"
        ::"r"(smem_u32(dst_smem)), "l"(src_gmem), "r"(bytes), "r"(smem_u32(bar)), "l"(evict_first) : "memory");
}
enum : int {
    PDL_TRIGGER = 1,
    PDL_WAIT_START = 2,
    PDL_WAIT_END = 4,
};
__device__ __forceinline__ void pdl_launch_dependents() { asm volatile("griddepcontrol.launch_dependents;" ::: "memory"); }
__device__ __forceinline__ void pdl_wait() { asm volatile("griddepcontrol.wait;" ::: "memory"); }

__device__ __forceinline__ void bulk_prefetch_l2(const void* src_gmem, uint32_t bytes) {
    asm volatile("cp.async.bulk.prefetch.L2.global [%0], %1;" ::"l"(src_gmem), "r"(bytes) : "memory");
}
__device__ __forceinline__ void named_bar_sync(int id, int n_threads) {
    asm volatile("bar.sync %0, %1;" ::"r"(id), "r"(n_threads) : "memory");
}
__device__ __forceinline__ float4 ldg_stream(const float4* p) {
    float4 v;
    asm volatile("ld.global.nc.L1::no_allocate.v4.f32 {%0, %1, %2, %3}, [%4];"
                 : "=f"(v.x), "=f"(v.y), "=f"(v.z), "=f"(v.w) : "l"(p));
    return v;
}

}
```

### pytorch_pose_proposal_network_b200/csrc/ppn_kernels.cu

```cuda
#include <algorithm>
#include <atomic>
#include <mutex>

#include "ppn_kernels.h"

namespace ppn {


struct Partial { float v; int32_t i; };

__host__ __device__ __forceinline__ int item_first(const ArgmaxPlan& p, int item) {
    return item < p.n_big ? item * p.G : p.n_big * p.G + (item - p.n_big) * p.small_m;
}
__host__ __device__ __forceinline__ int item_size(const ArgmaxPlan& p, int item) { return item < p.n_big ? p.G : p.small_m; }
__host__ __device__ __forceinline__ int item_count(const ArgmaxPlan& p, int n_mats) {
    const int rest = n_mats - p.n_big * p.G;
    return p.n_big + (rest + p.small_m - 1) / p.small_m;
}

__global__ void __launch_bounds__(1024, 1)
limb_argmax_tma_kernel(const float* __restrict__ head, uint16_t* __restrict__ amax, Geom g, ArgmaxPlan p, int pdl,
                       int* __restrict__ ticket, int32_t* __restrict__ zero2) {
    extern __shared__ __align__(128) unsigned char smem[];
    unsigned char* ring = smem;
// ... 960 lines not shown
                            }
                        } else {
                            for (int q = seen; q < m_pub; ++q) {
                                const float4 kb = kall[q];
                                hit |= suppresses_finite(bj, aj, kb, box_area(kb), thr, thr_pos);
                            }
                        }
                        dead = hit;
                    }
                    seen = m_pub;
                }
                if (wd >= w) break;
            }
            if (fin) break;
            if (tg) { if (w == 0) tl_phase_warp(*tg, 14); else if (w == 1) tl_phase_warp(*tg, 16); }
            unsigned und = ~__ballot_sync(0xffffffffu, dead);
            unsigned kept = 0u;
            while (und) {
                const bool mine = (und >> lane) & 1u;
                const bool killed = mine && (col & kept) != 0u;
                const bool free_ = mine && !killed && (col & und) == 0u;
                const unsigned k = __ballot_sync(0xffffffffu, free_);
                const unsigned d = __ballot_sync(0xffffffffu, killed);
                kept |= k;
                und &= ~(k | d);
            }
            bool done = false;
            if (limit > 0 && seen + __popc(kept) >= limit) {
                int need = limit - seen;
                unsigned trimmed = 0u;
                for (unsigned rest = kept; need > 0 && rest; --need) { const unsigned low = rest & (0u - rest); trimmed |= low; rest ^= low; }
                kept = trimmed;
                done = true;
            }
            if ((kept >> lane) & 1u) {
                const int idx = s.sidx[i0 + lane];
                const int pos = seen + __popc(kept & ((1u << lane) - 1u));
                out[pos] = map ? map[idx] : idx;
                kall[pos] = bj;
            }
            __syncwarp();
            if (lane == 0)
                st_release_cta_shared(&s.ctl[0], ((done || w == Wd - 1) ? 0x80000000u : 0u) | ((unsigned)(w + 1) << 16) |
                                                     (unsigned)(seen + __popc(kept)));
            if (tg) {
                if (w == 0) tl_phase_warp(*tg, 15); else if (w == 1) tl_phase_warp(*tg, 17); else if (w == 2) tl_phase_warp(*tg, 18);
                if (w == Wd - 1) tl_phase_warp(*tg, 19);
            }
            if (done) break;
        }
        __syncthreads();
        return s.ctl[0] & 0xffff;
    }
    int m = 0;
    for (int w = 0; w < Wd; ++w) {
        const int i0 = w << 5;
        if (warp == 0) {
            unsigned cur = s.rem[w];
            const int nb = min(32, n - i0);
            const unsigned valid = nb == 32 ? 0xffffffffu : ((1u << nb) - 1u);
            const unsigned diag = (lane < nb) ? s.diag[i0 + lane] : 0u;
            unsigned kept = 0;
            unsigned open = ~cur & valid;
            if (__popc(open) <= kNmsWalkMax) {
                while (open) {
                    const int t = __ffs((int)open) - 1;
                    kept |= 1u << t;
                    open &= ~(__shfl_sync(0xffffffffu, diag, t) | (1u << t));
                }
            } else {
#pragma unroll
                for (int t = 0; t < 32; ++t) {
                    const unsigned d = __shfl_sync(0xffffffffu, diag, t);
                    const unsigned take = (~cur >> t) & 1u;
                    kept |= take << t;
                    cur |= d & (0u - take);
                }
                kept &= valid;
            }
            bool done = false;
            if (limit > 0 && m + __popc(kept) >= limit) {
                int need = limit - m;
                unsigned trimmed = 0;
                for (unsigned rest = kept; need > 0 && rest; --need) { const unsigned low = rest & (0u - rest); trimmed |= low; rest ^= low; }
                kept = trimmed;
                done = true;
            }
            if ((kept >> lane) & 1u) {
                const int idx = s.sidx[i0 + lane];
                const int pos = __popc(kept & ((1u << lane) - 1u));
                out[m + pos] = map ? map[idx] : idx;
                s.kbox[pos] = s.sbox[i0 + lane];
                s.karea[pos] = s.sarea[i0 + lane];
            }
            if (lane == 0) { s.ctl[0] = (int)kept; s.ctl[1] = m + __popc(kept); s.ctl[2] = done || w == Wd - 1; }
        }
        __syncthreads();
        const unsigned kept = (unsigned)s.ctl[0];
        m = s.ctl[1];
        if (s.ctl[2]) break;
        const int n_kept = __popc(kept);
        if (n_kept == 0) { __syncthreads(); continue; }
        const int n_words = Wd - w - 1;
        int G = n_words > 0 ? n_warps / n_words : 1;
        G = G < 1 ? 1 : (G > n_kept ? n_kept : G);
        const int chunk = (n_kept + G - 1) / G;
        for (int item = warp; item < n_words * G; item += n_warps) {
            const int grp = item / n_words, w2 = w + 1 + (item - grp * n_words);
            const int q0 = grp * chunk, q1 = min(n_kept, q0 + chunk);
            const int j = (w2 << 5) + lane;
            const unsigned remw = s.rem[w2];
            bool bit = false;
            if (j < n && !((remw >> lane) & 1u)) {
                const float4 bj = s.sbox[j];
                const float aj = s.sarea[j];
                if (any_nan) {
                    for (int q = q0; q < q1; ++q) bit |= suppresses(bj, aj, s.kbox[q], s.karea[q], thr, thr_pos);
                } else {
#pragma unroll 4
                    for (int q = q0; q < q1; ++q) bit |= suppresses_finite(bj, aj, s.kbox[q], s.karea[q], thr, thr_pos);
                }
            }
            const unsigned word = __ballot_sync(0xffffffffu, bit);
            if (lane == 0 && word) {
                if (G == 1) s.rem[w2] = remw | word; else atomicOr(&s.rem[w2], word);
            }
        }
        __syncthreads();
    }
    return m;
}

__global__ void __launch_bounds__(512)
nms_smem_kernel(const float4* __restrict__ box, const float* __restrict__ score, const int32_t* __restrict__ count,
                int stride, float thr, int limit, int32_t* __restrict__ keep_idx, int32_t* __restrict__ keep_count, int blockwise) {
    extern __shared__ __align__(128) unsigned char smem[];
    const int prob = blockIdx.x;
    const int n = min(count[prob], stride);
    const int tid = threadIdx.x, T = blockDim.x;
    if (n <= 0) { if (tid == 0) keep_count[prob] = 0; return; }
    const NmsSmem s = nms_carve(smem, stride);
    for (int i = tid; i < n; i += T) {
        s.key[i] = score ? score_key(score[(size_t)prob * stride + i], i) : (unsigned long long)(unsigned)(n - 1 - i);
        s.rank[i] = 0;
    }
    __syncthreads();
    const int m = nms_core(s, box + (size_t)prob * stride, n, thr, limit, keep_idx + (size_t)prob * stride, nullptr, nullptr, blockwise != 0);
    if (tid == 0) keep_count[prob] = m;
}

template <typename T>
__global__ void __launch_bounds__(512, 3)
decode_nms_kernel(const T* __restrict__ head, Geom g, int n_parts, float det_thr, float nms_thr,
                  int32_t* __restrict__ keep_cell, int32_t* __restrict__ keep_count, int pdl) {
    extern __shared__ __align__(128) unsigned char smem[];
    tl_mark(g, TL_START);
    if (pdl & PDL_WAIT_START) pdl_wait();
    tl_mark(g, TL_WAITED);
    if (pdl & PDL_TRIGGER) pdl_launch_dependents();
    __shared__ int warp_tot[16];
    __shared__ int base_s;
    float4* ubox = reinterpret_cast<float4*>(smem);
    int32_t* ucell = reinterpret_cast<int32_t*>(ubox + g.HW);
    const NmsSmem s = nms_carve(reinterpret_cast<unsigned char*>(ucell + ((g.HW + 3) & ~3)), g.HW);
    const int tid = threadIdx.x, lane = tid & 31, warp = tid >> 5;
    const int n_lists = g.B * n_parts;
    for (int item = blockIdx.x; item < n_lists; item += gridDim.x) {
        const int b = item / n_parts, k = item - b * n_parts;
        const T* img = head + (size_t)b * g.img_stride;
        if (tid == 0) base_s = 0;
        for (int i = tid; i < g.HW; i += blockDim.x) s.rank[i] = 0;
        __syncthreads();
        for (int c0 = 0; c0 < g.HW; c0 += blockDim.x) {
            const int c = c0 + tid;
            float d = 0.0f;
            float4 bx = make_float4(0.f, 0.f, 0.f, 0.f);
            bool hit = false;
            if (c < g.HW) {
                d = delta_at(img, g, k, c);
                bx = box_at(img, g, k, c);
                hit = d > det_thr;
            }
            const unsigned bal = __ballot_sync(0xffffffffu, hit);
            if (lane == 0) warp_tot[warp] = __popc(bal);
            __syncthreads();
            int off = base_s, total = 0;
            for (int wi = 0; wi < (int)(blockDim.x >> 5); ++wi) {
                const int t = warp_tot[wi];
                if (wi < warp) off += t;
                total += t;
            }
            if (hit) {
                const int slot = off + __popc(bal & ((1u << lane) - 1u));
                ucell[slot] = c;
                ubox[slot] = bx;
                s.key[slot] = score_key(d, slot);
            }
            __syncthreads();
            if (tid == 0) base_s += total;
            __syncthreads();
        }
        const int n = base_s;
        const size_t list = (size_t)item * g.HW;
        int m = 0;
        if (n > 0) m = nms_core(s, ubox, n, nms_thr, 0, keep_cell + list, ucell, nullptr, (pdl & NMS_BLOCKWISE) != 0, false);
        if (tid == 0) keep_count[item] = m;
        __syncthreads();
    }
    tl_mark(g, TL_END);
    if (tid == 0 && (pdl & PDL_WAIT_END)) pdl_wait();
}

__global__ void __launch_bounds__(1024)
nms_global_kernel(const float4* __restrict__ box, const float* __restrict__ score, const int32_t* __restrict__ count,
                  int stride, float thr, int limit, int32_t* __restrict__ keep_idx, int32_t* __restrict__ keep_count) {
    const int prob = blockIdx.x;
    const int n = min(count[prob], stride);
    const int tid = threadIdx.x, T = blockDim.x;
    int32_t* out = keep_idx + (size_t)prob * stride;
    const float4* pbox = box + (size_t)prob * stride;
    const float* psc = score ? score + (size_t)prob * stride : nullptr;
    __shared__ int m_s;
    if (n <= 0) { if (tid == 0) keep_count[prob] = 0; return; }
    for (int i = tid; i < n; i += T) {
        int rank = i;
        if (psc) {
            const unsigned long long mine = score_key(psc[i], i);
            rank = 0;
            for (int j = 0; j < n; ++j) rank += (score_key(psc[j], j) > mine);
        }
        out[rank] = i;
    }
    if (tid == 0) m_s = 0;
    __syncthreads();
    for (int i = 0; i < n; ++i) {
        const int oi = out[i];
        if (oi < 0) continue;
        const float4 bi = pbox[oi];
        const float ai = box_area(bi);
        __syncthreads();
        if (tid == 0) out[m_s] = oi;
        for (int j = i + 1 + tid; j < n; j += T) {
            const int oj = out[j];
            if (oj >= 0) {
                const float4 bj = pbox[oj];
                if (suppresses(bj, box_area(bj), bi, ai, thr, thr > 0.0f)) out[j] = oj | (int)0x80000000;
            }
        }
        __syncthreads();
        if (tid == 0) m_s += 1;
        __syncthreads();
        if (limit > 0 && m_s >= limit) break;
    }
    if (tid == 0) keep_count[prob] = m_s;
}

constexpr int kMaxDyxTable = 2048;

enum : int {
    FUSED_GUARD = 8,
    FUSED_TRIGGER_EARLY = 16,
    FUSED_PUBLISH = 32,
    FUSED_WAIT_TOP = 64,
};

__device__ __forceinline__ int ld_acquire(const int* p) {
    int v;
    asm volatile("ld.acquire.gpu.global.s32 %0, [%1];" : "=r"(v) : "l"(p) : "memory");
    return v;
}


__device__ __forceinline__ int fast_div(int x, uint32_t magic) {
    return magic ? (int)__umulhi((unsigned)x, magic) : x;
}

template <bool kStaged, typename HT>
__device__ __forceinline__ float delta_lookup(const HT* resp, const HT* conf, int at) {
    if (kStaged) return __fmul_rn(widen(resp[at]), widen(conf[at]));
    return __fmul_rn(ldf(resp + at), ldf(conf + at));
}

template <bool kStaged, typename HT>
__device__ __forceinline__ void walk_chain(const ChainTable& ch, int cidx, int root, const Geom& g, float thr,
                                           const HT* s_resp, const HT* s_conf, const uint16_t* s_amax,
                                           const int32_t* s_dyx, bool use_tab, int16_t* my_pos) {
    int ih = fast_div(root, g.magic_W), iw = root - ih * g.W;
    for (int q = ch.off[cidx]; q < ch.off[cidx + 1]; ++q) {
        const int ei = ch.limb[q], t = ch.part[q];
        const int a = s_amax[ei * g.HW + ih * g.W + iw];
        int jh, jw;
        if (use_tab) {
            const int d = s_dyx[a];
            jh = ih + (d >> 16);
            jw = iw + (int)(int16_t)(d & 0xffff);
        } else {
            const int dy = a / g.sW, dx = a - dy * g.sW;
            jh = ih + dy - g.off_h;
            jw = iw + dx - g.off_w;
        }
        if (jh < 0 || jw < 0 || jh >= g.H || jw >= g.W) break;
        const int j = jh * g.W + jw;
        if (delta_lookup<kStaged, HT>(s_resp, s_conf, t * g.HW + j) < thr) break;
        my_pos[t] = (int16_t)j;
        ih = jh;
        iw = jw;
    }
}

template <bool kStaged, typename HT>
__global__ void __launch_bounds__(1024)
tree_parse_kernel(const HT* __restrict__ head, Geom g, ChainTable ch, float thr, int min_kp, int n_parts,
                  const uint16_t* __restrict__ amax, const int32_t* __restrict__ cand_cell,
                  const int32_t* __restrict__ keep_idx, const int32_t* __restrict__ keep_count,
                  int32_t* __restrict__ h_count, int32_t* __restrict__ h_root, int32_t* __restrict__ h_cell,
                  float* __restrict__ h_score, float4* __restrict__ h_box, int R, int use_tma, int stage_all, int pdl,
                  int* __restrict__ sync, int seq, int xywh_parts) {
    extern __shared__ __align__(128) unsigned char smem[];
    const int KHW = g.K * g.HW;
    const int n_groups = stage_all;
    HT* s_planes = reinterpret_cast<HT*>(smem);
    uint16_t* s_amax = reinterpret_cast<uint16_t*>(smem + ((((size_t)n_groups * KHW * sizeof(HT)) + 15) & ~(size_t)15));
    int32_t* s_root = reinterpret_cast<int32_t*>(s_amax + (((size_t)g.E * g.HW + 7) & ~(size_t)7));
    int32_t* s_slot = s_root + g.HW;
    int32_t* s_dyx = s_slot + g.HW;
    int16_t* s_pos = reinterpret_cast<int16_t*>(s_dyx + (g.S <= kMaxDyxTable ? g.S : 0));
    HT* s_xywh = reinterpret_cast<HT*>((reinterpret_cast<uintptr_t>(s_pos) + (size_t)g.HW * g.K * 2 + 15) & ~(uintptr_t)15);
    __shared__ __align__(8) uint64_t bar;
    __shared__ int warp_tot[32];
    __shared__ int base_s;

    const int tid = threadIdx.x, T = blockDim.x, lane = tid & 31, warp = tid >> 5;
    const bool use_tab = g.S <= kMaxDyxTable;
    const uint32_t bytes_planes = (uint32_t)n_groups * KHW * (uint32_t)sizeof(HT), bytes_am = (uint32_t)g.E * g.HW * 2u;

    tl_mark(g, TL_START);
    if (pdl & FUSED_GUARD) {
        if (tid == 0) while (ld_acquire(sync) < seq) __nanosleep(200);
        __syncthreads();
    }
    if (pdl & FUSED_TRIGGER_EARLY) pdl_launch_dependents();
    if (use_tma && tid == 0) {
        mbar_init(&bar, 1);
        fence_mbar_init();
    }
    if (use_tab)
        for (int a = tid; a < g.S; a += T) {
            const int dy = a / g.sW, dx = a - dy * g.sW;
            s_dyx[a] = ((dy - g.off_h) << 16) | ((dx - g.off_w) & 0xffff);
        }
    __syncthreads();
    uint32_t parity = 0;
    bool first = true;
    for (int b = blockIdx.x; b < g.B; b += gridDim.x, parity ^= 1u) {
        const HT* img = head + (size_t)b * g.img_stride;
        const HT* s_resp = kStaged ? s_planes : img;
        const HT* s_conf = s_resp + KHW;
        const uint16_t* am = amax + (size_t)b * g.E * g.HW;

        if (use_tma) {
            if (tid == 0) {
                mbar_arrive_expect_tx(&bar, bytes_planes + bytes_am);
                if (bytes_planes) bulk_g2s(s_planes, img, bytes_planes, &bar);
            }
        } else {
            for (int i = tid; i < n_groups * KHW; i += T) s_planes[i] = __ldg(img + i);
        }
        if (tid == 0) base_s = 0;
        if (first) {
            if (pdl & PDL_WAIT_START) pdl_wait();
            tl_mark(g, TL_WAITED);
            if (pdl & PDL_TRIGGER) pdl_launch_dependents();
            first = false;
        }
        if (use_tma) {
            if (tid == 0 && bytes_am) bulk_g2s(s_amax, am, bytes_am, &bar);
        } else {
            for (int i = tid; i < g.E * g.HW; i += T) s_amax[i] = am[i];
        }
        const int n_keep = min(keep_count[(size_t)b * n_parts], g.HW);
        const bool crowded = n_keep * 8 >= g.HW * 3;
        if (use_tma && tid == 0 && n_groups < 6 && crowded)
            bulk_prefetch_l2(img + (size_t)n_groups * KHW, (uint32_t)(6 - n_groups) * KHW * (uint32_t)sizeof(HT));
        const int32_t* keep = keep_idx + (size_t)b * n_parts * g.HW;
        const int32_t* cells = cand_cell ? cand_cell + (size_t)b * n_parts * g.HW : nullptr;

        for (int i = tid; i < n_keep * g.K; i += T) s_pos[i] = -1;
        for (int r = tid; r < n_keep; r += T) s_root[r] = cells ? cells[keep[r]] : keep[r];
        __syncthreads();
        for (int r = tid; r < n_keep; r += T) s_pos[r * g.K] = (int16_t)s_root[r];
        if (use_tma) mbar_wait(&bar, parity);
        if (n_keep == 0) {
            if (tid == 0) h_count[b] = 0;
            __syncthreads();
            continue;
        }
        __syncthreads();

        const int n_pad = (n_keep + 31) & ~31;
        const int n_par = ch.parallel_ok ? ch.n_chains : 1;
        for (int item = tid; item < n_par * n_pad; item += T) {
            const int cidx = item / n_pad, r = item - cidx * n_pad;
            if (r < n_keep) {
                int16_t* my_pos = s_pos + r * g.K;
                if (ch.parallel_ok) {
                    walk_chain<kStaged, HT>(ch, cidx, s_root[r], g, thr, s_resp, s_conf, s_amax, s_dyx, use_tab, my_pos);
                } else {
                    for (int c = 0; c < ch.n_chains; ++c)
                        walk_chain<kStaged, HT>(ch, c, s_root[r], g, thr, s_resp, s_conf, s_amax, s_dyx, use_tab, my_pos);
                }
            }
        }
        __syncthreads();

        for (int r0 = 0; r0 < n_keep; r0 += T) {
            const int r = r0 + tid;
            bool valid = false;
            if (r < n_keep) {
                int present = 0;
                for (int t = 1; t < g.K; ++t) present += (s_pos[r * g.K + t] >= 0);
                valid = min_kp <= present;
            }
            const unsigned bal = __ballot_sync(0xffffffffu, valid);
            if (lane == 0) warp_tot[warp] = __popc(bal);
            __syncthreads();
            int off = base_s, total = 0;
            for (int wi = 0; wi < (T >> 5); ++wi) {
                const int v = warp_tot[wi];
                if (wi < warp) off += v;
                total += v;
            }
            const int slot = off + __popc(bal & ((1u << lane) - 1u));
            if (r < n_keep) s_slot[r] = (valid && slot < R) ? slot : -1;
            __syncthreads();
            if (tid == 0) base_s += total;
        }
        __syncthreads();

        if (crowded && xywh_parts > 0 && n_groups < 6) {
            const int P = xywh_parts, PHW = P * g.HW;
            constexpr int kVec = 16 / (int)sizeof(HT);
            const bool vec_ok = (g.HW % kVec) == 0 && (g.img_stride % kVec) == 0 && (reinterpret_cast<uintptr_t>(head) & 15) == 0;
            for (int t0 = 0; t0 < g.K; t0 += P) {
                const int np = min(P, g.K - t0), n_el = np * g.HW;
                if (vec_ok) {
                    const int n_vec = n_el / kVec;
                    for (int j = tid; j < n_vec; j += T) {
                        uint4 v[4];
#pragma unroll
                        for (int q = 0; q < 4; ++q)
                            v[q] = __ldg(reinterpret_cast<const uint4*>(img + (size_t)(2 + q) * KHW + (size_t)t0 * g.HW) + j);
#pragma unroll
                        for (int q = 0; q < 4; ++q) reinterpret_cast<uint4*>(s_xywh + q * PHW)[j] = v[q];
                    }
                } else {
                    for (int q = 0; q < 4; ++q)
                        for (int j = tid; j < n_el; j += T) s_xywh[q * PHW + j] = __ldg(img + (size_t)(2 + q) * KHW + (size_t)t0 * g.HW + j);
                }
                __syncthreads();
                const uint32_t magic_np = np <= 1 ? 0u : (uint32_t)(((1ull << 32) + np - 1) / np);
                for (int pi = tid; pi < n_keep * np; pi += T) {
                    const int r = fast_div(pi, magic_np), tt = pi - r * np, t = t0 + tt;
                    const int sl = s_slot[r];
                    if (sl < 0) continue;
                    const int c = s_pos[r * g.K + t];
                    float score = 0.0f;
                    float4 box = make_float4(0.f, 0.f, 0.f, 0.f);
                    if (c >= 0) {
                        const int at = t * g.HW + c, a2 = tt * g.HW + c;
                        const int h = fast_div(c, g.magic_W), w = c - h * g.W;
                        score = delta_lookup<kStaged, HT>(s_resp, s_conf, at);
                        box = box_from(widen(s_xywh[a2]), widen(s_xywh[PHW + a2]), widen(s_xywh[2 * PHW + a2]),
                                       widen(s_xywh[3 * PHW + a2]), h, w, g);
                    }
                    const size_t human = (size_t)b * R + sl, o = human * g.K + t;
                    if (t == 0) h_root[human] = c;
                    h_cell[o] = c;
                    h_score[o] = score;
                    h_box[o] = box;
                }
                __syncthreads();
            }
        }
        const int n_pairs = (crowded && xywh_parts > 0 && n_groups < 6) ? 0 : n_keep * g.K;
        for (int p0 = tid; p0 < n_pairs; p0 += 4 * T) {
            int cc[4], tt[4], ss[4];
            float xs[4], ys[4], ws[4], hs[4];
#pragma unroll
            for (int u = 0; u < 4; ++u) {
                const int pair = p0 + u * T;
                cc[u] = -2;
                if (pair < n_pairs) {
                    const int r = fast_div(pair, g.magic_K), t = pair - r * g.K;
                    const int sl = s_slot[r];
                    if (sl >= 0) {
                        cc[u] = s_pos[pair];
                        tt[u] = t;
                        ss[u] = sl;
                        if (cc[u] >= 0) {
                            const int at = t * g.HW + cc[u];
                            if (n_groups == 6) {
                                xs[u] = widen(s_planes[2 * KHW + at]); ys[u] = widen(s_planes[3 * KHW + at]);
                                ws[u] = widen(s_planes[4 * KHW + at]); hs[u] = widen(s_planes[5 * KHW + at]);
                            } else {
                                xs[u] = ldf(img + (size_t)2 * KHW + at); ys[u] = ldf(img + (size_t)3 * KHW + at);
                                ws[u] = ldf(img + (size_t)4 * KHW + at); hs[u] = ldf(img + (size_t)5 * KHW + at);
                            }
                        }
                    }
                }
            }
#pragma unroll
            for (int u = 0; u < 4; ++u) {
                if (cc[u] == -2) continue;
                const int c = cc[u];
                float score = 0.0f;
                float4 box = make_float4(0.f, 0.f, 0.f, 0.f);
                if (c >= 0) {
                    const int at = tt[u] * g.HW + c;
                    const int h = fast_div(c, g.magic_W), w = c - h * g.W;
                    score = delta_lookup<kStaged, HT>(s_resp, s_conf, at);
                    box = box_from(xs[u], ys[u], ws[u], hs[u], h, w, g);
                }
                const size_t human = (size_t)b * R + ss[u], o = human * g.K + tt[u];
                if (tt[u] == 0) h_root[human] = c;
                h_cell[o] = c;
                h_score[o] = score;
                h_box[o] = box;
            }
        }
        if (tid == 0) h_count[b] = base_s;
        __syncthreads();
    }
    tl_mark(g, TL_END);
    if (pdl & FUSED_PUBLISH) {
        __syncthreads();
        if (tid == 0 && atomicAdd(sync + 1, 1) == (int)gridDim.x - 1) {
            sync[1] = 0;
            __threadfence();
            atomicMax(sync, seq + 1);
        }
    }
}

struct FusedSmem { uint32_t delta, root, dyx, uni, amax, slot, estart, pmask, pos, total; };

__host__ __device__ inline FusedSmem fused_layout(const Geom& g, bool staged) {
    FusedSmem l;
    uint32_t off = 0;
    l.delta = off; off += staged ? (uint32_t)g.K * g.HW * 4u : 0u;
    l.root = off;  off += (uint32_t)g.HW * 4u;
    l.dyx = off;   off += g.S <= 2048 ? (uint32_t)g.S * 4u : 0u;
    off = (off + 15u) & ~15u;
    l.uni = off;
    const uint32_t nms = (uint32_t)g.HW * 16u + (((uint32_t)g.HW + 3u) & ~3u) * 4u + (uint32_t)nms_bytes_per_list(g.HW);
    l.amax = l.uni;
    l.slot = l.amax + ((((uint32_t)g.E * g.HW * 2u) + 15u) & ~15u);
    l.estart = l.slot + (uint32_t)g.HW * 4u;
    l.pmask = l.estart + (uint32_t)g.HW * 4u;
    l.pos = l.pmask + (uint32_t)g.HW * 4u;
    const uint32_t walk = (l.pos - l.uni) + ((((uint32_t)g.HW * g.K * 2u) + 15u) & ~15u);
    l.total = l.uni + (nms > walk ? nms : walk);
    return l;
}

struct DenseOut {
    int32_t* header;
    int32_t* rheader;
    uint32_t* idcell;
    float* score;
    float4* box;
    int32_t cap;
    int32_t skip_slots;
    int32_t B_total, b0;
};

template <bool kStaged, typename HT>
__global__ void __launch_bounds__(512, 3)
parse_fused_kernel(const HT* __restrict__ head, Geom g, ChainTable ch, float det_thr, float nms_thr, int min_kp,
                   const uint16_t* __restrict__ amax, int32_t* __restrict__ h_count, int32_t* __restrict__ h_root,
                   int32_t* __restrict__ h_cell, float* __restrict__ h_score, float4* __restrict__ h_box, int R,
                   int pdl, int* __restrict__ sync, int seq, DenseOut dense) {
    extern __shared__ __align__(128) unsigned char smem[];
    const FusedSmem L = fused_layout(g, kStaged);
    float* s_delta = reinterpret_cast<float*>(smem + L.delta);
    int32_t* s_root = reinterpret_cast<int32_t*>(smem + L.root);
    int32_t* s_dyx = reinterpret_cast<int32_t*>(smem + L.dyx);
    float4* ubox = reinterpret_cast<float4*>(smem + L.uni);
    int32_t* ucell = reinterpret_cast<int32_t*>(ubox + g.HW);
    const NmsSmem s = nms_carve(reinterpret_cast<unsigned char*>(ucell + ((g.HW + 3) & ~3)), g.HW);
    uint16_t* s_amax = reinterpret_cast<uint16_t*>(smem + L.amax);
    int32_t* s_slot = reinterpret_cast<int32_t*>(smem + L.slot);
    int32_t* s_estart = reinterpret_cast<int32_t*>(smem + L.estart);
    uint32_t* s_pmask = reinterpret_cast<uint32_t*>(smem + L.pmask);
    int16_t* s_pos = reinterpret_cast<int16_t*>(smem + L.pos);
    __shared__ int warp_tot[16];
    __shared__ int warp_ent[16];
    __shared__ int base_s;
    __shared__ int ebase_s;
    __shared__ int n_keep_s;

    const int b = blockIdx.x;
    const int tid = threadIdx.x, T = blockDim.x, lane = tid & 31, warp = tid >> 5;
    const int KHW = g.K * g.HW;
    const HT* img = head + (size_t)b * g.img_stride;
    const bool use_tab = g.S <= kMaxDyxTable;

    tl_mark(g, TL_START);
    if (pdl & FUSED_WAIT_TOP) pdl_wait();
    if (pdl & FUSED_GUARD) {
        if (tid == 0) while (ld_acquire(sync) < seq) __nanosleep(200);
        __syncthreads();
    }
    if (pdl & FUSED_TRIGGER_EARLY) pdl_launch_dependents();
    if (tid == 0 && ((size_t)2 * g.K * g.HW * sizeof(HT)) % 16 == 0 && (g.img_stride * sizeof(HT)) % 16 == 0 &&
        (reinterpret_cast<uintptr_t>(head) & 15) == 0)
        bulk_prefetch_l2(head + (size_t)blockIdx.x * g.img_stride, (uint32_t)2 * g.K * g.HW * (uint32_t)sizeof(HT));

    tl_phase(g, 1);
    if (tid == 0) { base_s = 0; n_keep_s = 0; }
    for (int i = tid; i < g.HW; i += T) s.rank[i] = 0;
    if (use_tab)
        for (int a = tid; a < g.S; a += T) {
            const int dy = a / g.sW, dx = a - dy * g.sW;
            s_dyx[a] = ((dy - g.off_h) << 16) | ((dx - g.off_w) & 0xffff);
        }
    __syncthreads();
    for (int c0 = 0; c0 < g.HW; c0 += T) {
        const int c = c0 + tid;
        float d = 0.0f;
        float4 bx = make_float4(0.f, 0.f, 0.f, 0.f);
        bool hit = false;
        if (c < g.HW) {
            d = delta_at(img, g, 0, c);
            bx = box_at(img, g, 0, c);
            hit = d > det_thr;
        }
        const unsigned bal = __ballot_sync(0xffffffffu, hit);
        if (lane == 0) warp_tot[warp] = __popc(bal);
        __syncthreads();
        int off = base_s, total = 0;
        for (int wi = 0; wi < (T >> 5); ++wi) {
            const int t = warp_tot[wi];
            if (wi < warp) off += t;
            total += t;
        }
        if (hit) {
            const int slot = off + __popc(bal & ((1u << lane) - 1u));
            ucell[slot] = c;
            ubox[slot] = bx;
            s.key[slot] = score_key(d, slot);
        }
        __syncthreads();
        if (tid == 0) base_s += total;
        __syncthreads();
    }
    tl_phase(g, 2);
    if (kStaged)
        for (int i = tid; i < KHW; i += T) s_delta[i] = __fmul_rn(ldf(img + i), ldf(img + KHW + i));
    tl_phase(g, 3);
    const int n_cand = base_s;
    if (n_cand > 0) {
        const int m = nms_core(s, ubox, n_cand, nms_thr, 0, s_root, ucell, &g, (pdl & NMS_BLOCKWISE) != 0);
        if (tid == 0) n_keep_s = m;
    }
    __syncthreads();
    const int n_keep = n_keep_s;
    tl_phase(g, 4);
    if (tid == 0 && n_keep * 8 >= g.HW * 3 && ((size_t)KHW * sizeof(HT)) % 16 == 0 && (g.img_stride * sizeof(HT)) % 16 == 0 &&
        (reinterpret_cast<uintptr_t>(head) & 15) == 0)
        bulk_prefetch_l2(img + (size_t)2 * KHW, (uint32_t)4 * KHW * (uint32_t)sizeof(HT));
    for (int i = tid; i < n_keep * g.K; i += T) s_pos[i] = -1;
    __syncthreads();
    for (int r = tid; r < n_keep; r += T) s_pos[r * g.K] = (int16_t)s_root[r];

    if (pdl & PDL_WAIT_START) pdl_wait();
    tl_mark(g, TL_WAITED);
    if (pdl & PDL_TRIGGER) pdl_launch_dependents();
    if (n_keep > 0) {
        const uint16_t* am = amax + (size_t)b * g.E * g.HW;
        const int n16 = (g.E * g.HW) >> 3;
        if ((reinterpret_cast<uintptr_t>(am) & 15) == 0) {
            const uint4* src = reinterpret_cast<const uint4*>(am);
            uint4* dst = reinterpret_cast<uint4*>(s_amax);
            for (int i = tid; i < n16; i += T) dst[i] = __ldcg(src + i);
            for (int i = (n16 << 3) + tid; i < g.E * g.HW; i += T) s_amax[i] = __ldcg(am + i);
        } else {
            for (int i = tid; i < g.E * g.HW; i += T) s_amax[i] = __ldcg(am + i);
        }
    }
    __syncthreads();

    tl_phase(g, 5);
// ... 184 lines not shown
                    size_t n, int R, int K, float2* __restrict__ centre) {
    const size_t i = (size_t)blockIdx.x * blockDim.x + threadIdx.x;
    if (i >= n) return;
    const size_t human = i / K;
    const int b = (int)(human / R), slot = (int)(human - (size_t)b * R);
    float2 c = make_float2(0.0f, 0.0f);
    if (slot < count[b] && cell[i] >= 0) {
        const float4 bx = box[i];
        c = make_float2(__fmul_rn(__fadd_rn(bx.x, bx.z), 0.5f), __fmul_rn(__fadd_rn(bx.y, bx.w), 0.5f));
    }
    centre[i] = c;
}

struct EdgePairs { uint8_t src[256]; uint8_t dst[256]; };

__global__ void __launch_bounds__(256)
skeleton_kernel(const int32_t* __restrict__ count, const int32_t* __restrict__ cell, const float4* __restrict__ box, size_t n,
                int R, int K, int E, EdgePairs edges, int4* __restrict__ rect, float2* __restrict__ keypoint,
                float4* __restrict__ segment) {
    const size_t i = (size_t)blockIdx.x * blockDim.x + threadIdx.x;
    if (i >= n) return;
    const int per = 1 + K + E;
    const size_t human = i / per;
    const int item = (int)(i - human * per);
    const int b = (int)(human / R), slot = (int)(human - (size_t)b * R);
    const bool live = slot < count[b];
    const float nan = __int_as_float(0x7fc00000);
    const size_t base = human * K;
    auto centre = [&](int k, float& x, float& y) -> bool {
        if (!live || cell[base + k] < 0) return false;
        const float4 bx = box[base + k];
        y = __fmul_rn(__fadd_rn(bx.x, bx.z), 0.5f);
        x = __fmul_rn(__fadd_rn(bx.y, bx.w), 0.5f);
        return true;
    };
    if (item == 0) {
        int4 r = make_int4(0, 0, 0, 0);
        if (live && cell[base] >= 0) {
            const float4 bx = box[base];
            r = make_int4(__float2int_rz(bx.y), __float2int_rz(bx.x), __float2int_rz(bx.w), __float2int_rz(bx.z));
        }
        rect[human] = r;
    } else if (item <= K) {
        const int k = item - 1;
        float x, y;
        keypoint[base + k] = centre(k, x, y) ? make_float2(x, y) : make_float2(nan, nan);
    } else {
        const int e = item - 1 - K;
        float bx, by, ex, ey;
        const bool ok = centre(edges.src[e], bx, by) && centre(edges.dst[e], ex, ey);
        segment[human * E + e] = ok ? make_float4(bx, by, ex, ey) : make_float4(nan, nan, nan, nan);
    }
}

__global__ void __launch_bounds__(256)
pack_count_kernel(const int32_t* __restrict__ count, const int32_t* __restrict__ cell, int R, int K,
                  int32_t* __restrict__ header, int B) {
    __shared__ int red[8];
    const int b = blockIdx.x, tid = threadIdx.x, lane = tid & 31, warp = tid >> 5;
    const int n = min(count[b], R);
    const int32_t* c = cell + (size_t)b * R * K;
    int present = 0;
    for (int i = tid; i < n * K; i += blockDim.x) present += (c[i] >= 0);
#pragma unroll
    for (int o = 16; o > 0; o >>= 1) present += __shfl_xor_sync(0xffffffffu, present, o);
    if (lane == 0) red[warp] = present;
    __syncthreads();
    if (tid == 0) {
        int tot = 0;
        for (int wi = 0; wi < (int)(blockDim.x >> 5); ++wi) tot += red[wi];
        header[2 + b] = count[b];
        header[2 + B + b] = tot;
    }
}

__global__ void __launch_bounds__(256)
pack_entries_kernel(const int32_t* __restrict__ count, const int32_t* __restrict__ cell, const float* __restrict__ score,
                    const float4* __restrict__ box, int B, int R, int K, int cap, int32_t* __restrict__ header,
                    uint32_t* __restrict__ e_idcell, float* __restrict__ e_score, float4* __restrict__ e_box) {
    extern __shared__ __align__(16) int s_start[];
    __shared__ int red[8];
    const int b = blockIdx.x, tid = threadIdx.x, lane = tid & 31, warp = tid >> 5, n_warps = blockDim.x >> 5;
    const int32_t* per_image = header + 2 + B;
    int before = 0;
    for (int i = tid; i < b; i += blockDim.x) before += per_image[i];
#pragma unroll
    for (int o = 16; o > 0; o >>= 1) before += __shfl_xor_sync(0xffffffffu, before, o);
    if (lane == 0) red[warp] = before;
    __syncthreads();
    int off = 0;
    for (int wi = 0; wi < n_warps; ++wi) off += red[wi];
    if (tid == 0) {
        header[2 + 2 * B + b] = off;
        if (b == B - 1) {
            const int total = off + per_image[b];
            header[0] = total;
            header[1] = total > cap ? 1 : 0;
        }
    }
    const int n = min(count[b], R);
    const int32_t* c = cell + (size_t)b * R * K;
    for (int h = warp; h < n; h += n_warps) {
        int cnt = 0;
        for (int t0 = 0; t0 < K; t0 += 32) {
            const int t = t0 + lane;
            cnt += __popc(__ballot_sync(0xffffffffu, t < K && c[h * K + t] >= 0));
        }
        if (lane == 0) s_start[h + 1] = cnt;
    }
    __syncthreads();
    if (warp == 0) {
        int carry = 0;
        for (int h0 = 0; h0 < n; h0 += 32) {
            const int h = h0 + lane;
            int v = h < n ? s_start[h + 1] : 0, incl = v;
#pragma unroll
            for (int o = 1; o < 32; o <<= 1) {
                const int up = __shfl_up_sync(0xffffffffu, incl, o);
                if (lane >= o) incl += up;
            }
            if (h < n) s_start[h + 1] = carry + incl;
            carry += __shfl_sync(0xffffffffu, incl, 31);
        }
        if (lane == 0) s_start[0] = 0;
    }
    __syncthreads();
    for (int h = warp; h < n; h += n_warps) {
        int base = off + s_start[h];
        for (int t0 = 0; t0 < K; t0 += 32) {
            const int t = t0 + lane;
            const int cc = t < K ? c[h * K + t] : -1;
            const unsigned bal = __ballot_sync(0xffffffffu, cc >= 0);
            const int pos = base + __popc(bal & ((1u << lane) - 1u));
            if (cc >= 0 && pos < cap) {
                const size_t src = ((size_t)b * R + h) * K + t;
                e_idcell[pos] = ((uint32_t)t << 16) | (uint32_t)cc;
                e_score[pos] = score[src];
                e_box[pos] = box[src];
            }
            base += __popc(bal);
        }
    }
}

#define PPN_DISPATCH_HEAD(dtype, ...)                                                        \
    switch (dtype) {                                                                         \
        case HEAD_F32: { using T = float; __VA_ARGS__; } break;                              \
        case HEAD_F16: { using T = __half; __VA_ARGS__; } break;                             \
        case HEAD_BF16: { using T = __nv_bfloat16; __VA_ARGS__; } break;                     \
        default: return cudaErrorInvalidValue;                                               \
    }

constexpr int kTicketSlots = 64;
constexpr int kSlotWords = 8;
struct StreamSlot { cudaStream_t stream = nullptr; unsigned launches = 0; unsigned calls = 0; int published = 0; bool fast_open = false; };
struct DeviceInfo { int* tickets = nullptr; StreamSlot slot[kTicketSlots]; int slots_used = 0;
                    int sms = 0; int smem_optin = 0; size_t tma = 0, tma_multi = 0, tma16[2] = {0, 0}, decode_nms[3] = {0, 0, 0}, ldg = 0, nms = 0,
                           tree[3] = {0, 0, 0}, tree_light[3] = {0, 0, 0}, fused[2][3] = {{0, 0, 0}, {0, 0, 0}}, cluster[3] = {0, 0, 0}; };
static DeviceInfo g_dev[64];

static cudaError_t device_info(DeviceInfo** out) {
    int dev = 0;
    cudaError_t e = cudaGetDevice(&dev);
    if (e != cudaSuccess) return e;
    if (dev < 0 || dev >= 64) return cudaErrorInvalidDevice;
    DeviceInfo& d = g_dev[dev];
    if (!d.sms) {
        int sms = 0, optin = 0;
        if ((e = cudaDeviceGetAttribute(&optin, cudaDevAttrMaxSharedMemoryPerBlockOptin, dev)) != cudaSuccess) return e;
        if ((e = cudaDeviceGetAttribute(&sms, cudaDevAttrMultiProcessorCount, dev)) != cudaSuccess) return e;
        d.smem_optin = optin;
        d.sms = sms;
    }
    *out = &d;
    return cudaSuccess;
}

static std::mutex g_ticket_mu;

static cudaError_t slot_for(DeviceInfo* d, cudaStream_t st, StreamSlot** slot, int** words) {
    std::lock_guard<std::mutex> lock(g_ticket_mu);
    if (!d->tickets) {
        cudaError_t e = cudaMalloc(&d->tickets, kTicketSlots * kSlotWords * sizeof(int));
        if (e != cudaSuccess) return e;
        if ((e = cudaMemset(d->tickets, 0, kTicketSlots * kSlotWords * sizeof(int))) != cudaSuccess) return e;
    }
    *slot = nullptr;
    *words = nullptr;
    for (int i = 0; i < d->slots_used; ++i)
        if (d->slot[i].stream == st) { *slot = &d->slot[i]; *words = d->tickets + kSlotWords * i; return cudaSuccess; }
    if (d->slots_used == kTicketSlots) {
        for (int i = 0; i < kTicketSlots; ++i) {
            const cudaError_t q = cudaStreamQuery(d->slot[i].stream);
            if (q == cudaErrorNotReady) continue;
            if (q != cudaSuccess) (void)cudaGetLastError();
            d->slot[i].stream = st;
            d->slot[i].fast_open = false;
            *slot = &d->slot[i];
            *words = d->tickets + kSlotWords * i;
            return cudaSuccess;
        }
        return cudaSuccess;
    }
    d->slot[d->slots_used].stream = st;
    *slot = &d->slot[d->slots_used];
    *words = d->tickets + kSlotWords * d->slots_used++;
    return cudaSuccess;
}

unsigned next_call_parity(cudaStream_t st) {
    static thread_local unsigned t_calls = 0;
    DeviceInfo* d = nullptr;
    cudaStreamCaptureStatus cap = cudaStreamCaptureStatusNone;
    if (device_info(&d) != cudaSuccess || cudaStreamIsCapturing(st, &cap) != cudaSuccess || cap != cudaStreamCaptureStatusNone)
        return t_calls++ & 1u;
    StreamSlot* slot = nullptr;
    int* words = nullptr;
    if (slot_for(d, st, &slot, &words) != cudaSuccess || !slot) return t_calls++ & 1u;
    std::lock_guard<std::mutex> lock(g_ticket_mu);
    return slot->calls++ & 1u;
}

static cudaError_t ticket_for(DeviceInfo* d, cudaStream_t st, int** out) {
    StreamSlot* slot = nullptr;
    int* words = nullptr;
    cudaError_t e = slot_for(d, st, &slot, &words);
    if (e != cudaSuccess) return e;
    *out = slot ? words + 2 * (slot->launches++ & 1u) : nullptr;
    return cudaSuccess;
}

template <typename F>
static cudaError_t ensure_smem(F kernel, size_t want, size_t* have) {
    if (*have != 0 && want <= *have) return cudaSuccess;
    const size_t grant = want > 48 * 1024 ? want : 48 * 1024;
    cudaError_t e = cudaFuncSetAttribute(kernel, cudaFuncAttributeMaxDynamicSharedMemorySize, (int)grant);
    if (e != cudaSuccess) return e;
    e = cudaFuncSetAttribute(kernel, cudaFuncAttributePreferredSharedMemoryCarveout, (int)cudaSharedmemCarveoutMaxShared);
    if (e == cudaSuccess) *have = grant;
    return e;
}

template <typename... KArgs, typename... Args>
static cudaError_t launch_kernel(void (*kernel)(KArgs...), dim3 grid, dim3 block, size_t smem, cudaStream_t st, bool pdl,
                                 Args... args) {
    cudaLaunchConfig_t cfg = {};
    cfg.gridDim = grid;
    cfg.blockDim = block;
    cfg.dynamicSmemBytes = smem;
    cfg.stream = st;
    cudaLaunchAttribute attr[1];
    attr[0].id = cudaLaunchAttributeProgrammaticStreamSerialization;
    attr[0].val.programmaticStreamSerializationAllowed = 1;
    cfg.attrs = attr;
    cfg.numAttrs = pdl ? 1 : 0;
    return cudaLaunchKernelEx(&cfg, kernel, static_cast<KArgs>(args)...);
}

static void plan_tail(ArgmaxPlan* p, long long n_mats, long long grid, int divide) {
    const long long full_items = n_mats / p->G;
    const long long waves = grid > 0 ? full_items / grid : 0;
    p->small_m = divide > 1 && waves >= 2 ? std::max(1, p->G / divide) : p->G;
    p->n_big = p->small_m == p->G ? (int)((n_mats + p->G - 1) / p->G) : (int)((waves - 1) * grid);
    if (p->small_m == p->G) p->n_big = (int)full_items;
}

void argmax_item_partition(const ArgmaxPlan& p, int n_mats, int* n_items, int (*first_size)(void*, int, int, int), void* ctx) {
    *n_items = item_count(p, n_mats);
    for (int it = 0; it < *n_items; ++it) {
        const int m0 = item_first(p, it);
        first_size(ctx, it, m0, std::min(item_size(p, it), n_mats - m0));
    }
}

static void plan_tail_rows(ArgmaxPlan* p, int S, int row_bytes) {
    p->rows_s = p->rows;
    p->chunks_s = p->chunks;
    if (!row_bytes || p->small_m >= p->G) return;
    int max_rows = (int)(p->stage_bytes / ((size_t)row_bytes * p->small_m));
    max_rows = std::max(1, std::min(max_rows, S));
    p->chunks_s = (S + max_rows - 1) / max_rows;
    p->rows_s = (S + p->chunks_s - 1) / p->chunks_s;
    p->chunks_s = (S + p->rows_s - 1) / p->rows_s;
}

bool plan_argmax(const Geom& g, const Tuning& t, int sms, ArgmaxPlan* p) {
    if (g.HW % 4 != 0 || g.HW / 4 > 992) return false;
    p->CV = g.HW / 4;
    const int row_bytes = g.HW * 4;
    int G = t.argmax_threads / p->CV;
    if (G < 1) G = 1;
    while (G > 1 && p->CV * G > 992) --G;
    p->split_mats = (t.argmax_split < 0 ? (G > 1) : (t.argmax_split != 0)) ? 1 : 0;
    if (p->split_mats) {
        if (G > 32) G = 32;
        if (G > g.B * g.E) G = g.B * g.E;
    } else if (G > g.S) {
        G = g.S;
    }
    p->G = G;
    plan_tail(p, (long long)g.B * g.E, (long long)sms * (t.argmax_ctas_per_sm < 1 ? 1 : t.argmax_ctas_per_sm), t.argmax_tail_opt);
    p->threads = p->CV * G;
    p->threads_padded = (p->threads + 31) & ~31;
    const int per_row = p->split_mats ? row_bytes * G : row_bytes;
    const int stage_target = t.argmax_stage_bytes > 0 ? t.argmax_stage_bytes
                                                      : ((size_t)g.S * row_bytes <= 64 * 1024 ? 48 * 1024 : 32 * 1024);
    int max_rows = stage_target / per_row;
    if (max_rows < 1) max_rows = 1;
    if (max_rows > g.S) max_rows = g.S;
    p->chunks = (g.S + max_rows - 1) / max_rows;
    p->rows = (g.S + p->chunks - 1) / p->chunks;
    p->chunks = (g.S + p->rows - 1) / p->rows;
    p->stage_bytes = (uint32_t)(((size_t)p->rows * per_row + 127) & ~(size_t)127);
    plan_tail_rows(p, g.S, p->split_mats ? row_bytes : 0);
    p->stages = t.argmax_stages;
    p->dry = t.argmax_dry;
    p->ctas_per_sm = t.argmax_ctas_per_sm < 1 ? 1 : t.argmax_ctas_per_sm;
    p->smem_bytes = (size_t)p->stages * p->stage_bytes + (size_t)2 * p->stages * sizeof(uint64_t) +
                    (size_t)p->stages * sizeof(int) + (p->split_mats ? 0 : (size_t)2 * G * g.HW * sizeof(Partial));
    return true;
}

static bool plan_argmax16(const Geom& g, const Tuning& t, int sms, ArgmaxPlan* p) {
    if (g.HW % 8 != 0 || g.HW / 8 > 992) return false;
    p->CV = g.HW / 8;
    const int row_bytes = g.HW * 2;
    int G = t.argmax16_threads / p->CV;
    if (G < 1) G = 1;
    while (G > 1 && p->CV * G > 992) --G;
    if (G > 32) G = 32;
    if (G > g.B * g.E) G = g.B * g.E;
    p->ctas_per_sm = t.argmax_ctas_per_sm < 1 ? 1 : t.argmax_ctas_per_sm;
    p->split_mats = 1;
    p->G = G;
    plan_tail(p, (long long)g.B * g.E, (long long)sms * p->ctas_per_sm, t.argmax_tail_opt);
    p->threads = p->CV * G;
    p->threads_padded = (p->threads + 31) & ~31;
    const int per_row = row_bytes * G;
    int max_rows = t.argmax16_stage_bytes / per_row;
    if (max_rows < 1) max_rows = 1;
    if (max_rows > g.S) max_rows = g.S;
    p->chunks = (g.S + max_rows - 1) / max_rows;
    p->rows = (g.S + p->chunks - 1) / p->chunks;
    p->chunks = (g.S + p->rows - 1) / p->rows;
    p->stage_bytes = (uint32_t)(((size_t)p->rows * per_row + 127) & ~(size_t)127);
    plan_tail_rows(p, g.S, row_bytes);
    p->stages = t.argmax_stages;
    p->dry = t.argmax_dry;
    p->smem_bytes = (size_t)p->stages * p->stage_bytes + (size_t)2 * p->stages * sizeof(uint64_t) + (size_t)p->stages * sizeof(int);
    return true;
}

template <typename T16>
static cudaError_t launch_limb_argmax16(const T16* head, uint16_t* amax, const Geom& g, const Tuning& t, cudaStream_t st,
                                        bool pdl, bool* pdl_used, int pdl_bits, DeviceInfo* d, size_t* have, int32_t* zero2, bool* zeroed) {
    const int n_mats = g.B * g.E;
    ArgmaxPlan p;
    cudaError_t e;
    if (plan_argmax16(g, t, d->sms, &p) && (reinterpret_cast<uintptr_t>(head) & 15) == 0 && (g.img_stride * 2) % 16 == 0 &&
        (g.limb_off * 2) % 16 == 0) {
        size_t budget = (size_t)d->smem_optin / p.ctas_per_sm - (p.ctas_per_sm > 1 ? 1024 : 0);
        {
            const size_t two = p.smem_bytes - (size_t)(p.stages - 2) * (p.stage_bytes + 2 * sizeof(uint64_t) + sizeof(int));
            if (t.argmax_smem_cap > 0 && (size_t)t.argmax_smem_cap < budget && (p.stages < 2 || two <= (size_t)t.argmax_smem_cap))
                budget = (size_t)t.argmax_smem_cap;
        }
        while (p.smem_bytes > budget && p.stages > 2) {
            --p.stages;
            p.smem_bytes -= p.stage_bytes + 2 * sizeof(uint64_t) + sizeof(int);
        }
        if (p.smem_bytes <= budget) {
            int* ticket = nullptr;
            if (t.argmax_dynamic && (e = ticket_for(d, st, &ticket)) != cudaSuccess) return e;
            int grid = d->sms * p.ctas_per_sm;
            const int n_items = item_count(p, n_mats);
            if (grid > n_items) grid = n_items;
            if ((e = ensure_smem(limb_argmax_tma_multi16_kernel<T16>, p.smem_bytes, have)) != cudaSuccess) return e;
            e = launch_kernel(limb_argmax_tma_multi16_kernel<T16>, dim3(grid), dim3(p.threads_padded + 32), p.smem_bytes, st, pdl,
                              head, amax, g, p, pdl_bits, ticket, zero2);
            if (pdl_used) *pdl_used = pdl;
            if (zeroed) *zeroed = zero2 != nullptr;
// ... 82 lines not shown
            return cudaSuccess;
        }
    }
    if (g.dtype == HEAD_F16)
        return launch_limb_argmax16(static_cast<const __half*>(head_v), amax, g, t, st, pdl, pdl_used, pdl_bits, d, &d->tma16[0], zero2, zeroed);
    if (g.dtype == HEAD_BF16)
        return launch_limb_argmax16(static_cast<const __nv_bfloat16*>(head_v), amax, g, t, st, pdl, pdl_used, pdl_bits, d, &d->tma16[1], zero2, zeroed);
    if (g.dtype != HEAD_F32) return cudaErrorInvalidValue;
    const float* head = static_cast<const float*>(head_v);
    ArgmaxPlan p;
    const bool vec_ok = plan_argmax(g, t, d->sms, &p) && ((reinterpret_cast<uintptr_t>(head) & 15) == 0);
    if (vec_ok && t.argmax_variant == 0) {
        size_t budget = (size_t)d->smem_optin / p.ctas_per_sm - (p.ctas_per_sm > 1 ? 1024 : 0);
        {
            const size_t two = p.smem_bytes - (size_t)(p.stages - 2) * (p.stage_bytes + 2 * sizeof(uint64_t) + sizeof(int));
            if (t.argmax_smem_cap > 0 && (size_t)t.argmax_smem_cap < budget && (p.stages < 2 || two <= (size_t)t.argmax_smem_cap))
                budget = (size_t)t.argmax_smem_cap;
        }
        while (p.smem_bytes > budget && p.stages > 2) {
            --p.stages;
            p.smem_bytes -= p.stage_bytes + 2 * sizeof(uint64_t) + sizeof(int);
        }
        if (p.smem_bytes <= budget) {
            int* ticket = nullptr;
            if (t.argmax_dynamic && (e = ticket_for(d, st, &ticket)) != cudaSuccess) return e;
            int grid = d->sms * p.ctas_per_sm;
            if (p.split_mats) {
                const int n_items = item_count(p, n_mats);
                if (grid > n_items) grid = n_items;
                if ((e = ensure_smem(limb_argmax_tma_multi_kernel, p.smem_bytes, &d->tma_multi)) != cudaSuccess) return e;
                e = launch_kernel(limb_argmax_tma_multi_kernel, dim3(grid), dim3(p.threads_padded + 32), p.smem_bytes, st, pdl,
                                  head, amax, g, p, pdl_bits, ticket, zero2);
            } else {
                if (grid > n_mats) grid = n_mats;
                if ((e = ensure_smem(limb_argmax_tma_kernel, p.smem_bytes, &d->tma)) != cudaSuccess) return e;
                e = launch_kernel(limb_argmax_tma_kernel, dim3(grid), dim3(p.threads_padded + 32), p.smem_bytes, st, pdl,
                                  head, amax, g, p, pdl_bits, ticket, zero2);
            }
            if (pdl_used) *pdl_used = pdl;
            if (zeroed) *zeroed = zero2 != nullptr;
            return e;
        }
    }
    if (vec_ok) {
        if (p.split_mats) {
            Tuning rows_mode = t;
            rows_mode.argmax_split = 0;
            plan_argmax(g, rows_mode, d->sms, &p);
        }
        const size_t smem = (size_t)p.G * g.HW * sizeof(Partial);
        if ((e = ensure_smem(limb_argmax_ldg_kernel, smem, &d->ldg)) != cudaSuccess) return e;
        limb_argmax_ldg_kernel<<<n_mats, p.threads_padded, smem, st>>>(head, amax, g, p);
        return cudaGetLastError();
    }
    dim3 grid(n_mats, (g.HW + 255) / 256);
    limb_argmax_generic_kernel<float><<<grid, 256, 0, st>>>(head, amax, g);
    return cudaGetLastError();
}

cudaError_t launch_decode_candidates(const void* head, const Geom& g, int n_parts, float thr, int32_t* cand_cell,
                                     float* cand_score, float* cand_box, int32_t* cand_count, cudaStream_t st) {
    if (g.B == 0 || n_parts == 0) return cudaSuccess;
    dim3 grid(g.B, n_parts);
    PPN_DISPATCH_HEAD(g.dtype, decode_candidates_kernel<T><<<grid, 256, 0, st>>>(
        static_cast<const T*>(head), g, n_parts, thr, cand_cell, cand_score, reinterpret_cast<float4*>(cand_box), cand_count));
    return cudaGetLastError();
}

cudaError_t launch_restore_xy(const float* x, const float* y, float* rx, float* ry, size_t n, int H, int W,
                              float gridW, float gridH, cudaStream_t st) {
    if (n == 0) return cudaSuccess;
    restore_xy_kernel<<<(unsigned)((n + 255) / 256), 256, 0, st>>>(x, y, rx, ry, n, H * W, W, gridW, gridH);
    return cudaGetLastError();
}

cudaError_t launch_restore_size(const float* w, const float* h, float* rw, float* rh, size_t n, float inW, float inH,
                                cudaStream_t st) {
    if (n == 0) return cudaSuccess;
    restore_size_kernel<<<(unsigned)((n + 255) / 256), 256, 0, st>>>(w, h, rw, rh, n, inW, inH);
    return cudaGetLastError();
}

size_t nms_smem_bytes(int stride) { return nms_bytes_per_list(stride); }

static std::atomic<int> g_nms_blockwise{0};
void set_nms_blockwise(int on) { g_nms_blockwise.store(on != 0); }
int get_nms_blockwise() { return g_nms_blockwise.load(); }

cudaError_t launch_nms(const float* box, const float* score, const int32_t* count, int n_problems, int stride,
                       float thr, int limit, int32_t* keep_idx, int32_t* keep_count, cudaStream_t st) {
    if (n_problems == 0) return cudaSuccess;
    DeviceInfo* d = nullptr;
    cudaError_t e = device_info(&d);
    if (e != cudaSuccess) return e;
    const size_t smem = nms_smem_bytes(stride);
    if (stride <= 1024 && smem <= (size_t)d->smem_optin) {
        if ((e = ensure_smem(nms_smem_kernel, smem, &d->nms)) != cudaSuccess) return e;
        nms_smem_kernel<<<n_problems, stride <= 256 ? 256 : 512, smem, st>>>(reinterpret_cast<const float4*>(box), score, count,
                                                                             stride, thr, limit, keep_idx, keep_count,
                                                                             g_nms_blockwise.load());
        return cudaGetLastError();
    }
    nms_global_kernel<<<n_problems, 1024, 0, st>>>(reinterpret_cast<const float4*>(box), score, count, stride, thr,
                                                   limit, keep_idx, keep_count);
    return cudaGetLastError();
}

cudaError_t launch_part_centres(const int32_t* count, const int32_t* cell, const float* box, int B, int R, int K,
                                float* centre, cudaStream_t st) {
    const size_t n = (size_t)B * R * K;
    if (n == 0) return cudaSuccess;
    part_centres_kernel<<<(unsigned)((n + 255) / 256), 256, 0, st>>>(count, cell, reinterpret_cast<const float4*>(box), n, R, K,
                                                                     reinterpret_cast<float2*>(centre));
    return cudaGetLastError();
}

cudaError_t launch_skeleton(const int32_t* count, const int32_t* cell, const float* box, int B, int R, int K, int E,
                            const int32_t* edges, int32_t* rect, float* keypoint, float* segment, cudaStream_t st) {
    const size_t n = (size_t)B * R * (1 + K + E);
    if (n == 0) return cudaSuccess;
    EdgePairs ep;
    for (int e = 0; e < E; ++e) { ep.src[e] = (uint8_t)edges[2 * e]; ep.dst[e] = (uint8_t)edges[2 * e + 1]; }
    skeleton_kernel<<<(unsigned)((n + 255) / 256), 256, 0, st>>>(count, cell, reinterpret_cast<const float4*>(box), n, R, K, E, ep,
                                                                 reinterpret_cast<int4*>(rect), reinterpret_cast<float2*>(keypoint),
                                                                 reinterpret_cast<float4*>(segment));
    return cudaGetLastError();
}

cudaError_t launch_pack_humans(const int32_t* count, const int32_t* cell, const float* score, const float* box, int B, int R,
                               int K, int cap, int32_t* header, uint32_t* e_idcell, float* e_score, float* e_box,
                               cudaStream_t st) {
    if (B == 0) return cudaSuccess;
    pack_count_kernel<<<B, 256, 0, st>>>(count, cell, R, K, header, B);
    cudaError_t e = cudaGetLastError();
    if (e != cudaSuccess) return e;
    const size_t smem = (size_t)(R + 1) * sizeof(int);
    DeviceInfo* d = nullptr;
    if ((e = device_info(&d)) != cudaSuccess) return e;
    if (smem > (size_t)d->smem_optin) return cudaErrorInvalidConfiguration;
    static size_t have[64] = {};
    int dev = 0;
    if ((e = cudaGetDevice(&dev)) != cudaSuccess) return e;
    if (smem > 48 * 1024 && (e = ensure_smem(pack_entries_kernel, smem, &have[dev & 63])) != cudaSuccess) return e;
    pack_entries_kernel<<<B, 256, smem, st>>>(count, cell, score, reinterpret_cast<const float4*>(box),
                                                                        B, R, K, cap, header, e_idcell, e_score,
                                                                        reinterpret_cast<float4*>(e_box));
    return cudaGetLastError();
}

size_t decode_nms_smem_bytes(const Geom& g) {
    return (size_t)g.HW * sizeof(float4) + (size_t)((g.HW + 3) & ~3) * sizeof(int32_t) + nms_smem_bytes(g.HW);
}

cudaError_t launch_decode_nms(const void* head, const Geom& g, int n_parts, float det_thr, float nms_thr,
                              int32_t* keep_cell, int32_t* keep_count, cudaStream_t st, bool pdl_attr, int pdl_bits,
                              int ctas_per_sm, int threads_pref) {
    if (g.B == 0 || n_parts == 0) return cudaSuccess;
    DeviceInfo* d = nullptr;
    cudaError_t e = device_info(&d);
    if (e != cudaSuccess) return e;
    const size_t smem = decode_nms_smem_bytes(g);
    if (smem > (size_t)d->smem_optin) return cudaErrorInvalidConfiguration;
    const long long lists = (long long)g.B * n_parts;
    dim3 grid((unsigned)(ctas_per_sm > 0 ? std::min<long long>(lists, (long long)d->sms * ctas_per_sm) : lists));
    PPN_DISPATCH_HEAD(g.dtype, {
        if ((e = ensure_smem(decode_nms_kernel<T>, smem, &d->decode_nms[g.dtype])) != cudaSuccess) return e;
        const int threads = threads_pref > 0 ? std::min(512, std::max(64, (threads_pref + 31) & ~31)) : (g.HW <= 256 ? 256 : 512);
        return launch_kernel(decode_nms_kernel<T>, grid, dim3(threads), smem, st, pdl_attr,
                             static_cast<const T*>(head), g, n_parts, det_thr, nms_thr, keep_cell, keep_count,
                             pdl_bits | (g_nms_blockwise.load() ? NMS_BLOCKWISE : 0));
    });
    return cudaErrorInvalidValue;
}

static size_t head_elem_bytes(int dtype) { return dtype == HEAD_F32 ? 4 : 2; }

static int tree_parse_xywh_parts(const Geom& g, int n_groups) {
    if (n_groups >= 6) return 0;
    const size_t per_part = (size_t)4 * g.HW * head_elem_bytes(g.dtype);
    int P = (int)((24 * 1024) / per_part);
    if (P > g.K) P = g.K;
    return (P >= 1 && (g.K + P - 1) / P <= 4) ? P : 0;
}

static size_t tree_parse_smem_base(const Geom& g, int n_groups) {
    return ((((size_t)n_groups * g.K * g.HW * head_elem_bytes(g.dtype)) + 15) & ~(size_t)15) +
           ((((size_t)g.E * g.HW + 7) & ~(size_t)7)) * sizeof(uint16_t) +
           (size_t)2 * g.HW * sizeof(int32_t) + (g.S <= kMaxDyxTable ? (size_t)g.S * sizeof(int32_t) : 0) +
           ((((size_t)g.HW * g.K * sizeof(int16_t)) + 15) & ~(size_t)15);
}

size_t tree_parse_smem_bytes(const Geom& g, int n_groups) {
    const int P = tree_parse_xywh_parts(g, n_groups);
    return tree_parse_smem_base(g, n_groups) + (P ? 16 + (size_t)P * 4 * g.HW * head_elem_bytes(g.dtype) : 0);
}

static int tree_parse_groups(const Geom& g, int stage_all_pref, int smem_optin) {
    int n_groups;
    if (stage_all_pref < 0)
        n_groups = tree_parse_smem_base(g, 6) <= 32 * 1024 ? 6 : (tree_parse_smem_base(g, 2) <= 64 * 1024 ? 2 : 0);
    else
        n_groups = stage_all_pref >= 2 ? 6 : (stage_all_pref == 1 ? 2 : 0);
    while (n_groups > 0 && tree_parse_smem_bytes(g, n_groups) > (size_t)smem_optin) n_groups = n_groups == 6 ? 2 : 0;
    return n_groups;
}

size_t chain3_ring_cap(const Geom& g, int stage_all_pref, int k12_ctas) {
    DeviceInfo* d = nullptr;
    if (device_info(&d) != cudaSuccess) return 0;
    const size_t sm_bytes = (size_t)d->smem_optin + 1024;
    const size_t others = (size_t)k12_ctas * (decode_nms_smem_bytes(g) + 1024) +
                          tree_parse_smem_bytes(g, tree_parse_groups(g, stage_all_pref, d->smem_optin)) + 1024;
    if (others + 1024 + 64 * 1024 > sm_bytes) return 0;
    return sm_bytes - others - 1024;
}

cudaError_t launch_tree_parse(const void* head, const Geom& g, const ChainTable& ch, float thr, int min_kp, int n_parts,
                              const uint16_t* amax, const int32_t* cand_cell, const int32_t* keep_idx,
                              const int32_t* keep_count, int32_t* h_count, int32_t* h_root, int32_t* h_cell,
                              float* h_score, float* h_box, int R, cudaStream_t st, bool pdl_attr, int pdl_bits,
                              int stage_all_pref, int threads_pref, int chain_mode, int ctas_per_sm) {
    if (g.B == 0) return cudaSuccess;
    DeviceInfo* d = nullptr;
    cudaError_t e = device_info(&d);
    if (e != cudaSuccess) return e;
    const int n_groups = tree_parse_groups(g, stage_all_pref, d->smem_optin);
    const size_t smem = tree_parse_smem_bytes(g, n_groups);
    int threads = threads_pref > 0 ? threads_pref : ((g.HW <= 144 || n_groups == 0) ? 256 : 512);
    threads = ((threads < 64 ? 64 : (threads > 1024 ? 1024 : threads)) + 31) & ~31;
    if (smem > (size_t)d->smem_optin) return cudaErrorInvalidConfiguration;
    const size_t es = head_elem_bytes(g.dtype);
    const bool tma_ok = ((size_t)g.K * g.HW * 2 * es) % 16 == 0 && (g.img_stride * es) % 16 == 0 &&
                        ((size_t)g.E * g.HW * 2) % 16 == 0 && (reinterpret_cast<uintptr_t>(head) & 15) == 0 &&
                        (reinterpret_cast<uintptr_t>(amax) & 15) == 0;
    const dim3 grid((unsigned)(ctas_per_sm > 0 ? std::min<long long>(g.B, (long long)d->sms * ctas_per_sm) : g.B));
    StreamSlot* slot = nullptr;
    int* words = nullptr;
    int bits = pdl_bits, seq = 0;
    if (chain_mode > 0) {
        cudaStreamCaptureStatus cap = cudaStreamCaptureStatusNone;
        if ((e = cudaStreamIsCapturing(st, &cap)) != cudaSuccess) return e;
        if (cap == cudaStreamCaptureStatusNone && (e = slot_for(d, st, &slot, &words)) != cudaSuccess) return e;
        if (slot) { bits |= FUSED_PUBLISH; seq = slot->published; }
        if (pdl_attr && chain_mode == 2 && slot) bits = (bits & ~PDL_TRIGGER) | FUSED_GUARD | FUSED_TRIGGER_EARLY;
    }
    int* sync = words ? words + 4 : nullptr;
    PPN_DISPATCH_HEAD(g.dtype, {
        if (n_groups) {
            if ((e = ensure_smem(tree_parse_kernel<true, T>, smem, &d->tree[g.dtype])) != cudaSuccess) return e;
            e = launch_kernel(tree_parse_kernel<true, T>, grid, dim3(threads), smem, st, pdl_attr, static_cast<const T*>(head),
                              g, ch, thr, min_kp, n_parts, amax, cand_cell, keep_idx, keep_count, h_count, h_root, h_cell,
                              h_score, reinterpret_cast<float4*>(h_box), R, tma_ok ? 1 : 0, n_groups, bits, sync, seq,
                              tree_parse_xywh_parts(g, n_groups));
        } else {
            if ((e = ensure_smem(tree_parse_kernel<false, T>, smem, &d->tree_light[g.dtype])) != cudaSuccess) return e;
            e = launch_kernel(tree_parse_kernel<false, T>, grid, dim3(threads), smem, st, pdl_attr, static_cast<const T*>(head),
                              g, ch, thr, min_kp, n_parts, amax, cand_cell, keep_idx, keep_count, h_count, h_root, h_cell,
                              h_score, reinterpret_cast<float4*>(h_box), R, tma_ok ? 1 : 0, n_groups, bits, sync, seq,
                              tree_parse_xywh_parts(g, n_groups));
        }
    });
    if (e == cudaSuccess && slot) {
        std::lock_guard<std::mutex> lock(g_ticket_mu);
        slot->published = seq + 1;
        slot->fast_open = true;
    }
    return e;
}

static int fused_ctas_per_sm(const Geom& g, const Tuning& t, int smem_optin, size_t smem) {
    const int t124 = g.HW <= 256 ? 256 : 512;
    const int t3 = ((g.dtype == HEAD_F32 ? t.argmax_threads : t.argmax16_threads) + 31) / 32 * 32 + 32;
    const size_t sm_bytes = (size_t)smem_optin + 1024;
    const size_t min_ring = 3 * 32 * 1024 + 1024;
    if (smem > (size_t)smem_optin || sm_bytes < min_ring + 1024) return 0;
    long long n = (2048 - t3) / t124;
    n = std::min<long long>(n, (65536 - (long long)t3 * 56) / ((long long)t124 * 40));
    n = std::min<long long>(n, (long long)((sm_bytes - min_ring - 1024) / (smem + 1024)));
    return n < 0 ? 0 : (int)n;
}

static bool fused_split_plan(const Geom& g, const Tuning& t, DeviceInfo* d, int stage_pref, FusedSplit* out) {
    if (g.HW > 1024 || g.B < 1) return false;
    const size_t with = fused_layout(g, true).total, without = fused_layout(g, false).total;
    const int cap_with = stage_pref == 0 ? 0 : fused_ctas_per_sm(g, t, d->smem_optin, with) * d->sms;
    const int cap_without = stage_pref > 0 ? 0 : fused_ctas_per_sm(g, t, d->smem_optin, without) * d->sms;
    const int n_with = cap_with > 0 ? (g.B + cap_with - 1) / cap_with : 0;
    const int n_without = cap_without > 0 ? (g.B + cap_without - 1) / cap_without : 0;
    if (!n_with && !n_without) return false;
    bool staged = n_with && (!n_without || n_with < n_without || (n_with == n_without && (stage_pref > 0 || with <= 48 * 1024)));
    out->staged = staged;
    out->smem = staged ? with : without;
    out->n_sub = staged ? n_with : n_without;
    out->sub_B = (g.B + out->n_sub - 1) / out->n_sub;
    const int per_sm = (out->sub_B + d->sms - 1) / d->sms;
    out->ring_cap = (size_t)d->smem_optin + 1024 - (size_t)per_sm * (out->smem + 1024) - 1024;
    return true;
}

static bool fused_plan(const Geom& g, int smem_optin, int stage_pref, bool* staged, size_t* smem) {
    if (g.HW > 1024) return false;
    const size_t with = fused_layout(g, true).total, without = fused_layout(g, false).total;
    bool st = stage_pref < 0 ? with <= 48 * 1024 : (stage_pref > 0 && with <= (size_t)smem_optin);
    if (!st && without > (size_t)smem_optin) return false;
    *staged = st;
    *smem = st ? with : without;
    return true;
}

bool parse_fused_supported(const Geom& g, int stage_pref) {
    DeviceInfo* d = nullptr;
    if (device_info(&d) != cudaSuccess) return false;
    bool staged;
    size_t smem;
    return fused_plan(g, d->smem_optin, stage_pref, &staged, &smem);
}

bool parse_fused_split(const Geom& g, int stage_pref, const Tuning& t, FusedSplit* out) {
    DeviceInfo* d = nullptr;
    if (device_info(&d) != cudaSuccess) return false;
    return fused_split_plan(g, t, d, stage_pref, out);
}

size_t parse_fused_smem_bytes(const Geom& g, int stage_pref) {
    DeviceInfo* d = nullptr;
    bool staged;
    size_t smem = 0;
    if (device_info(&d) != cudaSuccess || !fused_plan(g, d->smem_optin, stage_pref, &staged, &smem)) return 0;
    return smem;
}

cudaError_t launch_parse_fused(const void* head, const Geom& g, const ChainTable& ch, float det_thr, float nms_thr, int min_kp,
                               const uint16_t* amax, int32_t* h_count, int32_t* h_root, int32_t* h_cell, float* h_score,
                               float* h_box, int R, cudaStream_t st, bool pdl_attr, int chain_mode, int stage_pref,
                               int staged_forced, const DenseTarget* dense_to, bool wait_top) {
    if (g.B == 0) return cudaSuccess;
    DeviceInfo* d = nullptr;
    cudaError_t e = device_info(&d);
    if (e != cudaSuccess) return e;
    bool staged;
    size_t smem;
    if (!fused_plan(g, d->smem_optin, stage_pref, &staged, &smem)) return cudaErrorInvalidConfiguration;
    if (staged_forced >= 0) {
        staged = staged_forced != 0;
        smem = fused_layout(g, staged).total;
        if (smem > (size_t)d->smem_optin) return cudaErrorInvalidConfiguration;
    }
    DenseOut dense = {nullptr, nullptr, nullptr, nullptr, nullptr, 0, 0, 0, 0};
    if (dense_to) {
        if (g.K > 32) return cudaErrorInvalidConfiguration;
        dense = DenseOut{dense_to->header, dense_to->rheader, dense_to->idcell, dense_to->score, reinterpret_cast<float4*>(dense_to->box),
                         dense_to->cap, dense_to->skip_slots, dense_to->B_total, dense_to->b0};
    }
    StreamSlot* slot = nullptr;
    int* words = nullptr;
    cudaStreamCaptureStatus cap = cudaStreamCaptureStatusNone;
    if ((e = cudaStreamIsCapturing(st, &cap)) != cudaSuccess) return e;
    if (cap == cudaStreamCaptureStatusNone && (e = slot_for(d, st, &slot, &words)) != cudaSuccess) return e;
    int bits = 0;
    if (pdl_attr) bits |= PDL_WAIT_START;
    if (pdl_attr && wait_top) bits |= FUSED_WAIT_TOP;
    int seq = 0;
    if (slot) { bits |= FUSED_PUBLISH; seq = slot->published; }
    if (pdl_attr && chain_mode == 2 && slot) bits |= FUSED_GUARD | FUSED_TRIGGER_EARLY;
    else if (pdl_attr) bits |= PDL_TRIGGER;
    if (g_nms_blockwise.load()) bits |= NMS_BLOCKWISE;
    const int threads = g.HW <= 256 ? 256 : 512;
    int* sync = words ? words + 4 : nullptr;
    PPN_DISPATCH_HEAD(g.dtype, {
        if (staged) {
            if ((e = ensure_smem(parse_fused_kernel<true, T>, smem, &d->fused[1][g.dtype])) != cudaSuccess) return e;
            e = launch_kernel(parse_fused_kernel<true, T>, dim3(g.B), dim3(threads), smem, st, pdl_attr, static_cast<const T*>(head), g, ch,
                              det_thr, nms_thr, min_kp, amax, h_count, h_root, h_cell, h_score, reinterpret_cast<float4*>(h_box), R,
                              bits, sync, seq, dense);
        } else {
            if ((e = ensure_smem(parse_fused_kernel<false, T>, smem, &d->fused[0][g.dtype])) != cudaSuccess) return e;
            e = launch_kernel(parse_fused_kernel<false, T>, dim3(g.B), dim3(threads), smem, st, pdl_attr, static_cast<const T*>(head), g, ch,
                              det_thr, nms_thr, min_kp, amax, h_count, h_root, h_cell, h_score, reinterpret_cast<float4*>(h_box), R,
                              bits, sync, seq, dense);
        }
    });
    if (e == cudaSuccess && slot) {
        std::lock_guard<std::mutex> lock(g_ticket_mu);
        slot->published = seq + 1;
        slot->fast_open = true;
    }
    return e;
}

bool chain_clean(cudaStream_t st) {
    DeviceInfo* d = nullptr;
    if (device_info(&d) != cudaSuccess) return false;
    std::lock_guard<std::mutex> lock(g_ticket_mu);
    for (int i = 0; i < d->slots_used; ++i)
        if (d->slot[i].stream == st) return d->slot[i].fast_open;
    return false;
}

void chain_break(cudaStream_t st) {
    DeviceInfo* d = nullptr;
    if (device_info(&d) != cudaSuccess) return;
    std::lock_guard<std::mutex> lock(g_ticket_mu);
    for (int i = 0; i < d->slots_used; ++i)
        if (d->slot[i].stream == st) d->slot[i].fast_open = false;
}

}
```

### pytorch_pose_proposal_network_b200/csrc/ppn_kernels.h

```cpp
#pragma once
#include "ppn_device.cuh"

namespace ppn {

struct Tuning {
    int argmax_variant = 0;
    int argmax_stage_bytes = 0;
    int argmax_stages = 4;
    int argmax_threads = 320;
    int argmax_ctas_per_sm = 1;
    int argmax_split = -1;
    int argmax_dynamic = 1;
    int argmax_tail_opt = 0;
    int argmax_cluster = -1;
    int argmax_cluster_ring = 0;
    int argmax_smem_cap = 0;
    int argmax16_threads = 320;
    int argmax16_stage_bytes = 48 * 1024;
    int parse_stage_all = -1;
    int parse_threads = 0;
    int parse_fused = -1;
    int parse_chain_calls = 1;
    int parse_k12_threads = 0;
    int parse_persist = 1;
    int host_chunk_images = 64;
    int encode_sweep = 1;
    int encode_ctas_per_sm = 6;
    int argmax_dry = 0;
    int head_subs = 0;
    int parse_overlap = 2;
};

struct ArgmaxPlan {
    int CV;
    int G;
    int threads;
    int threads_padded;
    int rows;
    int chunks;
    int split_mats;
    int stages;
    int ctas_per_sm;
    int dry;
    int n_big;
    int small_m;
    int rows_s, chunks_s;
    uint32_t stage_bytes;
    size_t smem_bytes;
};

bool plan_argmax(const Geom& g, const Tuning& t, int sms, ArgmaxPlan* p);
void argmax_item_partition(const ArgmaxPlan& p, int n_mats, int* n_items, int (*first_size)(void*, int, int, int), void* ctx);

cudaError_t launch_limb_argmax(const void* head, uint16_t* amax, const Geom& g, const Tuning& t, cudaStream_t st,
                               bool pdl = false, bool* pdl_used = nullptr, int pdl_bits = -1 ,
                               int32_t* zero2 = nullptr ,
                               bool* zeroed = nullptr);

cudaError_t launch_decode_candidates(const void* head, const Geom& g, int n_parts, float thr, int32_t* cand_cell,
                                     float* cand_score, float* cand_box, int32_t* cand_count, cudaStream_t st);

void set_nms_blockwise(int on);
int get_nms_blockwise();
cudaError_t launch_nms(const float* box, const float* score, const int32_t* count, int n_problems, int stride,
                       float thr, int limit, int32_t* keep_idx, int32_t* keep_count, cudaStream_t st);

cudaError_t launch_decode_nms(const void* head, const Geom& g, int n_parts, float det_thr, float nms_thr,
                              int32_t* keep_cell, int32_t* keep_count, cudaStream_t st, bool pdl_attr = false,
                              int pdl_bits = 0, int ctas_per_sm = 0 , int threads_pref = 0);
size_t chain3_ring_cap(const Geom& g, int stage_all_pref, int k12_ctas);

cudaError_t launch_restore_xy(const float* x, const float* y, float* rx, float* ry, size_t n, int H, int W,
                              float gridW, float gridH, cudaStream_t st);
cudaError_t launch_restore_size(const float* w, const float* h, float* rw, float* rh, size_t n, float inW, float inH,
                                cudaStream_t st);

cudaError_t launch_part_centres(const int32_t* count, const int32_t* cell, const float* box, int B, int R, int K,
                                float* centre, cudaStream_t st);

cudaError_t launch_skeleton(const int32_t* count, const int32_t* cell, const float* box, int B, int R, int K, int E,
                            const int32_t* edges , int32_t* rect, float* keypoint, float* segment, cudaStream_t st);

cudaError_t launch_pack_humans(const int32_t* count, const int32_t* cell, const float* score, const float* box, int B, int R,
                               int K, int cap, int32_t* header, uint32_t* e_idcell, float* e_score, float* e_box,
                               cudaStream_t st);

size_t tree_parse_smem_bytes(const Geom& g, int n_groups);

cudaError_t launch_tree_parse(const void* head, const Geom& g, const ChainTable& ch, float thr, int min_kp, int n_parts,
                              const uint16_t* amax, const int32_t* cand_cell, const int32_t* keep_idx,
                              const int32_t* keep_count, int32_t* h_count, int32_t* h_root, int32_t* h_cell,
                              float* h_score, float* h_box, int R, cudaStream_t st, bool pdl_attr = false, int pdl_bits = 0,
                              int stage_all_pref = -1, int threads_pref = 0, int chain_mode = 0 , int ctas_per_sm = 0 );

bool parse_fused_supported(const Geom& g, int stage_pref);
struct FusedSplit { int n_sub, sub_B; bool staged; size_t smem, ring_cap; };
bool parse_fused_split(const Geom& g, int stage_pref, const Tuning& t, FusedSplit* out);
size_t parse_fused_smem_bytes(const Geom& g, int stage_pref);
struct DenseTarget { int32_t* header; uint32_t* idcell; float* score; float* box; int32_t cap; int32_t skip_slots;
                     int32_t B_total; int32_t b0;
                     int32_t* rheader = nullptr; };
cudaError_t launch_parse_fused(const void* head, const Geom& g, const ChainTable& ch, float det_thr, float nms_thr, int min_kp,
                               const uint16_t* amax, int32_t* h_count, int32_t* h_root, int32_t* h_cell, float* h_score,
                               float* h_box, int R, cudaStream_t st, bool pdl_attr, int chain_mode, int stage_pref,
                               int staged_forced = -1, const DenseTarget* dense_to = nullptr, bool wait_top = false);
unsigned next_call_parity(cudaStream_t st);
bool chain_clean(cudaStream_t st);
void chain_break(cudaStream_t st);

size_t head_smem_bytes();
size_t head_keys_bytes(const Geom& g);
cudaError_t launch_head_gemm_argmax(const float* feat, const float* weight, const float* bias, int Cin, const Geom& g,
                                    float* dec, uint16_t* amax, unsigned long long* keys, float* emit_logits, float* emit_head,
                                    cudaStream_t st, bool pdl_attr, int pdl_bits, int subs);
bool head16_supported(int Cin, const Geom& g);
size_t head16_packed_feat_bytes(int Cin, const Geom& g);
size_t head16_packed_weight_bytes(int Cin, const Geom& g);
cudaError_t launch_head_gemm16_argmax(const void* feat, bool feat_nchw_f32, const float* weight, const float* bias, int Cin, bool bf16,
                                      const Geom& g, void* xt, void* wt, float* dec, uint16_t* amax, unsigned long long* keys,
                                      float* emit_logits, float* emit_head, cudaStream_t st, int pdl_bits, int subs);

struct EdgeTable { uint8_t src[256]; uint8_t dst[256]; };
struct EncodeArgs {
    const int32_t* person_off;
    const double* bbox;
    const float* keypoints;
    const uint8_t* visible;
    const double* size;
    float *delta, *weight, *tx, *ty, *tx_half, *ty_half, *tw, *th;
    void *weight_ij, *te;
    int32_t limb_dtype;
    int32_t K, E, H, W, sH, sW, rows_per_cta;
    int32_t small_only, sweep, sweep_ctas_per_sm;
    uint32_t magic_sW;
    float gridW, gridH;
    double inW, inH;
    EdgeTable edges;
};
cudaError_t launch_encode_targets(EncodeArgs a, int B, int sms, cudaStream_t st);

constexpr int kLossMaxCtas = 2048;
struct LossArgs {
    const void* head;
    void* grad;
    const float *delta, *weight, *tx, *ty, *tx_half, *ty_half, *tw, *th;
    const void *weight_ij, *te;
    int32_t head_dtype, limb_dtype;
    const float* grad_loss;
    double* partial;
    int32_t B, K, W, HW, L;
    size_t img_stride, limb_off;
    float gW, gH, inW, inH;
    long long small_items, limb_chunks, n_items;
};
void loss_plan(LossArgs* a);
size_t loss_workspace_bytes(const LossArgs& a);
cudaError_t launch_loss_forward(LossArgs a, float* loss, int sms, cudaStream_t st, bool from_logits = false);
cudaError_t launch_loss_backward(LossArgs a, int sms, cudaStream_t st, bool from_logits = false);
cudaError_t launch_sigmoid(const void* x, int dtype, float* y, size_t n, cudaStream_t st);

}
```

Before: 9.001 million.

## Use atomic ticket work-stealing and flag-based handoff between decode-NMS and tree parse

Persistent decode_nms and tree_parse kernels now take work items from a global atomic ticket counter instead of a fixed grid stride, which balances uneven per-item cost. Decode_nms publishes a completion sequence word that tree_parse spin-waits on, so limb_argmax no longer needs to wait for the end of the previous kernel and the three kernels can overlap more. It also adds per-CTA timeline instrumentation and a persist_grid knob. The cost is one atomic plus a block barrier per item and spin-wait polling, with some risk of deadlock if the producer is not resident.

```diff
diff --git a/include/ppn_decode_bench.h b/include/ppn_decode_bench.h
--- a/include/ppn_decode_bench.h
+++ b/include/ppn_decode_bench.h
@@ -12,6 +12,10 @@
 
 int ppn_timeline(void* dev_records, int32_t max_records);
 
+int ppn_timeline_ctas(void* dev_records, int32_t max_ctas);
+
+int ppn_debug_ticket_word(int32_t kind, int32_t launch, int32_t* word);
+
 int ppn_debug_argmax_items(const PPNShape* shape, int32_t sms, int32_t* info , int32_t* first, int32_t* size, int32_t max_items);
 
 int ppn_tune(const char* key, int32_t value);
diff --git a/pytorch_pose_proposal_network_b200/_lib.py b/pytorch_pose_proposal_network_b200/_lib.py
--- a/pytorch_pose_proposal_network_b200/_lib.py
+++ b/pytorch_pose_proposal_network_b200/_lib.py
@@ -126,6 +126,8 @@
     "ppn_sigmoid": (C.c_int, [C.c_void_p, C.c_int32, C.c_void_p, C.c_size_t, C.c_void_p]),
     "ppn_debug_argmax_items": (C.c_int, [C.POINTER(PPNShape), C.c_int32, i32p, i32p, i32p, C.c_int32]),
     "ppn_timeline": (C.c_int, [C.c_void_p, C.c_int32]),
+    "ppn_timeline_ctas": (C.c_int, [C.c_void_p, C.c_int32]),
+    "ppn_debug_ticket_word": (C.c_int, [C.c_int32, C.c_int32, i32p]),
     "ppn_profile_enable": (C.c_int, [C.c_int32]),
     "ppn_profile_read": (C.c_int, [f32p, i32p]),
     "ppn_tune": (C.c_int, [C.c_char_p, C.c_int32]),
diff --git a/pytorch_pose_proposal_network_b200/csrc/ppn_capi.cu b/pytorch_pose_proposal_network_b200/csrc/ppn_capi.cu
--- a/pytorch_pose_proposal_network_b200/csrc/ppn_capi.cu
+++ b/pytorch_pose_proposal_network_b200/csrc/ppn_capi.cu
@@ -52,10 +52,15 @@
 
 inline int cuda_rc(cudaError_t e) { return e == cudaSuccess ? PPN_OK : (int)e; }
 
-struct Timeline { unsigned long long* buf = nullptr; int cap = 0, used = 0, phase = 0; } g_timeline;
+struct Timeline { unsigned long long* buf = nullptr; int cap = 0, used = 0, phase = 0; unsigned long long* cta = nullptr; int cta_cap = 0; } g_timeline;
 inline ppn::Geom timeline_slot(ppn::Geom g) {
-    if (g_timeline.buf && g_timeline.used < g_timeline.cap) { g.tl = g_timeline.buf; g.tl_slot = g_timeline.used++; g.tl_phase = g_timeline.phase; }
-    else g.tl = nullptr;
+    if (g_timeline.buf && g_timeline.used < g_timeline.cap) {
+        g.tl = g_timeline.buf; g.tl_slot = g_timeline.used++; g.tl_phase = g_timeline.phase;
+        g.tl_cta = g_timeline.cta; g.tl_cta_cap = g_timeline.cta_cap;
+    } else {
+        g.tl = nullptr;
+        g.tl_cta = nullptr;
+    }
     return g;
 }
 
@@ -82,6 +87,8 @@
     g.tl = nullptr;
     g.tl_slot = 0;
     g.tl_phase = 0;
+    g.tl_cta = nullptr;
+    g.tl_cta_cap = 0;
     auto magic = [](int d) -> uint32_t { return d <= 1 ? 0u : (uint32_t)(((1ull << 32) + d - 1) / d); };
     g.magic_W = magic(g.W);
     g.magic_K = magic(g.K);
@@ -217,6 +224,7 @@
     else if (!std::strcmp(key, "parse.stage_all")) t.parse_stage_all = value;
     else if (!std::strcmp(key, "parse.chain_calls")) t.parse_chain_calls = value != 0;
     else if (!std::strcmp(key, "parse.persist")) t.parse_persist = value < 0 ? 0 : (value > 4 ? 4 : value);
+    else if (!std::strcmp(key, "parse.persist_grid")) t.parse_persist_grid = value < 0 ? 0 : value;
     else if (!std::strcmp(key, "parse.k12_threads")) t.parse_k12_threads = value < 0 ? 0 : value;
     else if (!std::strcmp(key, "parse.fused")) t.parse_fused = value < 0 ? -1 : (value != 0);
     else if (!std::strcmp(key, "parse.threads")) t.parse_threads = value;
@@ -252,6 +260,7 @@
     else if (!std::strcmp(key, "parse.stage_all")) *value = t.parse_stage_all;
     else if (!std::strcmp(key, "parse.chain_calls")) *value = t.parse_chain_calls;
     else if (!std::strcmp(key, "parse.persist")) *value = t.parse_persist;
+    else if (!std::strcmp(key, "parse.persist_grid")) *value = t.parse_persist_grid;
     else if (!std::strcmp(key, "parse.k12_threads")) *value = t.parse_k12_threads;
     else if (!std::strcmp(key, "parse.fused")) *value = t.parse_fused;
     else if (!std::strcmp(key, "parse.threads")) *value = t.parse_threads;
@@ -523,7 +532,8 @@
     const int P = params->n_nms_parts;
     const Workspace w = carve(shape, P);
     if (workspace_bytes < 2 * w.total) return PPN_E_WORKSPACE;
-    unsigned char* ws = static_cast<unsigned char*>(workspace) + (ppn::next_call_parity((cudaStream_t)stream) ? w.total : 0);
+    const size_t half = (workspace_bytes / 2) & ~(size_t)255;
+    unsigned char* ws = static_cast<unsigned char*>(workspace) + (ppn::next_call_parity((cudaStream_t)stream) ? half : 0);
     uint16_t* amax = reinterpret_cast<uint16_t*>(ws + w.amax);
     int32_t* keep_idx = reinterpret_cast<int32_t*>(ws + w.keep_idx);
     int32_t* keep_count = reinterpret_cast<int32_t*>(ws + w.keep_count);
@@ -623,13 +633,17 @@
         const bool attr12 = chain_calls && (!overlap_calls || capturing || chain_clean(st));
         const int bits12 = PDL_TRIGGER | (!attr12 ? 0 : (overlap_calls ? PDL_WAIT_END : PDL_WAIT_START));
         bool chained = false;
+        ChainPub lists;
         if ((e = launch_decode_nms(head, timeline_slot(g), P, params->det_thresh, params->nms_thresh, keep_idx, keep_count, st, attr12,
-                                   bits12, k12_ctas, g_tuning.parse_k12_threads)) != cudaSuccess) return (int)e;
-        if ((e = launch_limb_argmax(head, amax, timeline_slot(g), tuning, st, true, &chained)) != cudaSuccess) return (int)e;
+                                   bits12, k12_ctas, g_tuning.parse_k12_threads, g_tuning.parse_persist_grid,
+                                   early ? &lists : nullptr)) != cudaSuccess) return (int)e;
+        const int bits3 = lists.word ? PDL_TRIGGER : (PDL_TRIGGER | PDL_WAIT_END);
+        if ((e = launch_limb_argmax(head, amax, timeline_slot(g), tuning, st, true, &chained, bits3)) != cudaSuccess) return (int)e;
         if ((e = launch_tree_parse(head, timeline_slot(g), ch, params->det_thresh, params->min_num_keypoints, P, amax, nullptr, keep_idx,
                                    keep_count, out->count, out->root_cell, out->part_cell, out->part_score, out->part_box,
                                    out->R, st, chained, chained ? (PDL_WAIT_START | PDL_TRIGGER) : 0, g_tuning.parse_stage_all,
-                                   g_tuning.parse_threads, chained ? (early ? 2 : 1) : 0, k4_ctas)) != cudaSuccess) return (int)e;
+                                   g_tuning.parse_threads, chained ? (early ? 2 : 1) : 0, k4_ctas, g_tuning.parse_persist_grid,
+                                   lists)) != cudaSuccess) return (int)e;
         if (!chained) chain_break(st);
         if (!dense) return PPN_OK;
         rc = pack_after(out, shape, dense, st);
@@ -1061,6 +1075,12 @@
     return cuda_rc(ppn::launch_sigmoid(x, x_dtype, y, n, (cudaStream_t)stream));
 }
 
+int ppn_debug_ticket_word(int32_t kind, int32_t launch, int32_t* word) {
+    if (kind < 0 || kind >= ppn::kTicketKinds || launch < 0 || !word) return PPN_E_BADARG;
+    *word = ppn::ticket_pair_word(kind, (unsigned)launch);
+    return PPN_OK;
+}
+
 int ppn_debug_argmax_items(const PPNShape* shape, int32_t sms, int32_t* info, int32_t* first, int32_t* size, int32_t max_items) {
     int rc = check_shape(shape);
     if (rc) return rc;
@@ -1083,6 +1103,13 @@
     g_timeline.buf = static_cast<unsigned long long*>(dev_records);
     g_timeline.cap = dev_records ? max_records : 0;
     g_timeline.used = 0;
+    return PPN_OK;
+}
+
+int ppn_timeline_ctas(void* dev_records, int32_t max_ctas) {
+    if (dev_records && max_ctas < 1) return PPN_E_BADARG;
+    g_timeline.cta = static_cast<unsigned long long*>(dev_records);
+    g_timeline.cta_cap = dev_records ? max_ctas : 0;
     return PPN_OK;
 }
 
diff --git a/pytorch_pose_proposal_network_b200/csrc/ppn_device.cuh b/pytorch_pose_proposal_network_b200/csrc/ppn_device.cuh
--- a/pytorch_pose_proposal_network_b200/csrc/ppn_device.cuh
+++ b/pytorch_pose_proposal_network_b200/csrc/ppn_device.cuh
@@ -25,6 +25,8 @@
     unsigned long long* tl;
     int32_t tl_slot;
     int32_t tl_phase;
+    unsigned long long* tl_cta;
+    int32_t tl_cta_cap;
 };
 
 enum : int { TL_START = 0, TL_END = 1, TL_WAITED = 2 };
@@ -44,6 +46,31 @@
         if (phase >= 100) atomicMax(g.tl + 4 * (size_t)g.tl_slot + 3, t);
         else atomicMin(g.tl + 4 * (size_t)g.tl_slot + 3, t);
     }
+}
+
+__device__ __forceinline__ unsigned long long global_ns() {
+    unsigned long long t;
+    asm volatile("mov.u64 %0, %%globaltimer;" : "=l"(t));
+    return t;
+}
+__device__ __forceinline__ void tl_cta_reset(const Geom& g, unsigned long long* s) {
+    if (g.tl_cta && threadIdx.x == 0) s[0] = s[1] = s[2] = s[3] = 0;
+}
+enum : int { TL_ITEM_BEGIN = 0, TL_ITEM_END = 1, TL_ITEM_RESUME = 2  };
+__device__ __forceinline__ void tl_cta_item(const Geom& g, unsigned long long* s, int what) {
+    if (!g.tl_cta || threadIdx.x != 0) return;
+    const unsigned long long t = global_ns();
+    if (what == TL_ITEM_BEGIN && !s[3]) s[0] = t;
+    if (what == TL_ITEM_END) {
+        s[2] += t - s[1];
+        s[3] += 1;
+    }
+    s[1] = t;
+}
+__device__ __forceinline__ void tl_cta_store(const Geom& g, const unsigned long long* s) {
+    if (!g.tl_cta || threadIdx.x != 0 || (int)blockIdx.x >= g.tl_cta_cap) return;
+    unsigned long long* rec = g.tl_cta + 4 * ((size_t)g.tl_slot * g.tl_cta_cap + blockIdx.x);
+    rec[0] = s[0]; rec[1] = s[1]; rec[2] = s[2]; rec[3] = s[3];
 }
 
 __device__ __forceinline__ void tl_phase_warp(const Geom& g, int phase) {
diff --git a/pytorch_pose_proposal_network_b200/csrc/ppn_kernels.cu b/pytorch_pose_proposal_network_b200/csrc/ppn_kernels.cu
--- a/pytorch_pose_proposal_network_b200/csrc/ppn_kernels.cu
+++ b/pytorch_pose_proposal_network_b200/csrc/ppn_kernels.cu
@@ -1136,7 +1136,8 @@
 template <typename T>
 __global__ void __launch_bounds__(512, 3)
 decode_nms_kernel(const T* __restrict__ head, Geom g, int n_parts, float det_thr, float nms_thr,
-                  int32_t* __restrict__ keep_cell, int32_t* __restrict__ keep_count, int pdl) {
+                  int32_t* __restrict__ keep_cell, int32_t* __restrict__ keep_count, int pdl,
+                  int* __restrict__ ticket, int* __restrict__ pub, int seq) {
     extern __shared__ __align__(128) unsigned char smem[];
     tl_mark(g, TL_START);
     if (pdl & PDL_WAIT_START) pdl_wait();
@@ -1144,12 +1145,22 @@
     if (pdl & PDL_TRIGGER) pdl_launch_dependents();
     __shared__ int warp_tot[16];
     __shared__ int base_s;
+    __shared__ int item_s;
+    __shared__ unsigned long long s_tl[4];
     float4* ubox = reinterpret_cast<float4*>(smem);
     int32_t* ucell = reinterpret_cast<int32_t*>(ubox + g.HW);
     const NmsSmem s = nms_carve(reinterpret_cast<unsigned char*>(ucell + ((g.HW + 3) & ~3)), g.HW);
     const int tid = threadIdx.x, lane = tid & 31, warp = tid >> 5;
     const int n_lists = g.B * n_parts;
-    for (int item = blockIdx.x; item < n_lists; item += gridDim.x) {
+    tl_cta_reset(g, s_tl);
+    for (int item = blockIdx.x;; item += gridDim.x) {
+        if (ticket) {
+            if (tid == 0) item_s = atomicAdd(ticket, 1);
+            __syncthreads();
+            item = item_s;
+        }
+        if (item >= n_lists) break;
+        tl_cta_item(g, s_tl, TL_ITEM_BEGIN);
         const int b = item / n_parts, k = item - b * n_parts;
         const T* img = head + (size_t)b * g.img_stride;
         if (tid == 0) base_s = 0;
@@ -1190,9 +1201,22 @@
         if (n > 0) m = nms_core(s, ubox, n, nms_thr, 0, keep_cell + list, ucell, nullptr, (pdl & NMS_BLOCKWISE) != 0, false);
         if (tid == 0) keep_count[item] = m;
         __syncthreads();
+        tl_cta_item(g, s_tl, TL_ITEM_END);
     }
     tl_mark(g, TL_END);
+    tl_cta_store(g, s_tl);
     if (tid == 0 && (pdl & PDL_WAIT_END)) pdl_wait();
+    if (ticket && tid == 0) {
+        __threadfence();
+        if (atomicAdd(ticket + 1, 1) == (int)gridDim.x - 1) {
+            ticket[0] = 0;
+            ticket[1] = 0;
+            if (pub) {
+                __threadfence();
+                atomicMax(pub, seq + 1);
+            }
+        }
+    }
 }
 
 __global__ void __launch_bounds__(1024)
@@ -1299,7 +1323,8 @@
                   const int32_t* __restrict__ keep_idx, const int32_t* __restrict__ keep_count,
                   int32_t* __restrict__ h_count, int32_t* __restrict__ h_root, int32_t* __restrict__ h_cell,
                   float* __restrict__ h_score, float4* __restrict__ h_box, int R, int use_tma, int stage_all, int pdl,
-                  int* __restrict__ sync, int seq, int xywh_parts) {
+                  int* __restrict__ sync, int seq, int xywh_parts, int* __restrict__ ticket, const int* __restrict__ lists_pub,
+                  int lists_seq) {
     extern __shared__ __align__(128) unsigned char smem[];
     const int KHW = g.K * g.HW;
     const int n_groups = stage_all;
@@ -1313,12 +1338,15 @@
     __shared__ __align__(8) uint64_t bar;
     __shared__ int warp_tot[32];
     __shared__ int base_s;
+    __shared__ int item_s;
+    __shared__ unsigned long long s_tl[4];
 
     const int tid = threadIdx.x, T = blockDim.x, lane = tid & 31, warp = tid >> 5;
     const bool use_tab = g.S <= kMaxDyxTable;
     const uint32_t bytes_planes = (uint32_t)n_groups * KHW * (uint32_t)sizeof(HT), bytes_am = (uint32_t)g.E * g.HW * 2u;
 
     tl_mark(g, TL_START);
+    tl_cta_reset(g, s_tl);
     if (pdl & FUSED_GUARD) {
         if (tid == 0) while (ld_acquire(sync) < seq) __nanosleep(200);
         __syncthreads();
@@ -1336,7 +1364,14 @@
     __syncthreads();
     uint32_t parity = 0;
     bool first = true;
-    for (int b = blockIdx.x; b < g.B; b += gridDim.x, parity ^= 1u) {
+    for (int b = blockIdx.x;; b += gridDim.x, parity ^= 1u) {
+        if (ticket) {
+            if (tid == 0) item_s = atomicAdd(ticket, 1);
+            __syncthreads();
+            b = item_s;
+        }
+        if (b >= g.B) break;
+        tl_cta_item(g, s_tl, TL_ITEM_BEGIN);
         const HT* img = head + (size_t)b * g.img_stride;
         const HT* s_resp = kStaged ? s_planes : img;
         const HT* s_conf = s_resp + KHW;
@@ -1353,7 +1388,12 @@
         if (tid == 0) base_s = 0;
         if (first) {
             if (pdl & PDL_WAIT_START) pdl_wait();
+            if (lists_pub) {
+                if (tid == 0) while (ld_acquire(lists_pub) < lists_seq) __nanosleep(100);
+                __syncthreads();
+            }
             tl_mark(g, TL_WAITED);
+            tl_cta_item(g, s_tl, TL_ITEM_RESUME);
             if (pdl & PDL_TRIGGER) pdl_launch_dependents();
             first = false;
         }
@@ -1362,7 +1402,7 @@
         } else {
             for (int i = tid; i < g.E * g.HW; i += T) s_amax[i] = am[i];
         }
-        const int n_keep = min(keep_count[(size_t)b * n_parts], g.HW);
+        const int n_keep = min(__ldcg(keep_count + (size_t)b * n_parts), g.HW);
         const bool crowded = n_keep * 8 >= g.HW * 3;
         if (use_tma && tid == 0 && n_groups < 6 && crowded)
             bulk_prefetch_l2(img + (size_t)n_groups * KHW, (uint32_t)(6 - n_groups) * KHW * (uint32_t)sizeof(HT));
@@ -1370,13 +1410,14 @@
         const int32_t* cells = cand_cell ? cand_cell + (size_t)b * n_parts * g.HW : nullptr;
 
         for (int i = tid; i < n_keep * g.K; i += T) s_pos[i] = -1;
-        for (int r = tid; r < n_keep; r += T) s_root[r] = cells ? cells[keep[r]] : keep[r];
+        for (int r = tid; r < n_keep; r += T) s_root[r] = cells ? cells[keep[r]] : __ldcg(keep + r);
         __syncthreads();
         for (int r = tid; r < n_keep; r += T) s_pos[r * g.K] = (int16_t)s_root[r];
         if (use_tma) mbar_wait(&bar, parity);
         if (n_keep == 0) {
             if (tid == 0) h_count[b] = 0;
             __syncthreads();
+            tl_cta_item(g, s_tl, TL_ITEM_END);
             continue;
         }
         __syncthreads();
@@ -1515,14 +1556,23 @@
         }
         if (tid == 0) h_count[b] = base_s;
         __syncthreads();
+        tl_cta_item(g, s_tl, TL_ITEM_END);
     }
     tl_mark(g, TL_END);
-    if (pdl & FUSED_PUBLISH) {
-        __syncthreads();
-        if (tid == 0 && atomicAdd(sync + 1, 1) == (int)gridDim.x - 1) {
-            sync[1] = 0;
-            __threadfence();
-            atomicMax(sync, seq + 1);
+    tl_cta_store(g, s_tl);
+    if (ticket || (pdl & FUSED_PUBLISH)) {
+        __syncthreads();
+        if (tid == 0) {
+            int* done = ticket ? ticket + 1 : sync + 1;
+            if (ticket) __threadfence();
+            if (atomicAdd(done, 1) == (int)gridDim.x - 1) {
+                *done = 0;
+                if (ticket) ticket[0] = 0;
+                if (pdl & FUSED_PUBLISH) {
+                    __threadfence();
+                    atomicMax(sync, seq + 1);
+                }
+            }
         }
     }
 }
@@ -2013,8 +2063,15 @@
     }
 
 constexpr int kTicketSlots = 64;
-constexpr int kSlotWords = 8;
-struct StreamSlot { cudaStream_t stream = nullptr; unsigned launches = 0; unsigned calls = 0; int published = 0; bool fast_open = false; };
+constexpr int kSlotWords = 16;
+constexpr int kListsPubWord = 6;
+struct StreamSlot { cudaStream_t stream = nullptr; unsigned launches[kTicketKinds] = {}; unsigned calls = 0; int published = 0;
+                    int lists_published = 0; bool fast_open = false; };
+
+int ticket_pair_word(int kind, unsigned launch) {
+    static const int base[kTicketKinds] = {0, 8, 12};
+    return base[kind] + 2 * (int)(launch & 1u);
+}
 struct DeviceInfo { int* tickets = nullptr; StreamSlot slot[kTicketSlots]; int slots_used = 0;
                     int sms = 0; int smem_optin = 0; size_t tma = 0, tma_multi = 0, tma16[2] = {0, 0}, decode_nms[3] = {0, 0, 0}, ldg = 0, nms = 0,
                            tree[3] = {0, 0, 0}, tree_light[3] = {0, 0, 0}, fused[2][3] = {{0, 0, 0}, {0, 0, 0}}, cluster[3] = {0, 0, 0}; };
@@ -2082,12 +2139,14 @@
     return slot->calls++ & 1u;
 }
 
-static cudaError_t ticket_for(DeviceInfo* d, cudaStream_t st, int** out) {
+static cudaError_t ticket_for(DeviceInfo* d, cudaStream_t st, int** out, int kind = kTicketRing) {
     StreamSlot* slot = nullptr;
     int* words = nullptr;
     cudaError_t e = slot_for(d, st, &slot, &words);
     if (e != cudaSuccess) return e;
-    *out = slot ? words + 2 * (slot->launches++ & 1u) : nullptr;
+    if (!slot) { *out = nullptr; return cudaSuccess; }
+    std::lock_guard<std::mutex> lock(g_ticket_mu);
+    *out = words + ticket_pair_word(kind, slot->launches[kind]++);
     return cudaSuccess;
 }
 
@@ -2476,9 +2535,15 @@
     return (size_t)g.HW * sizeof(float4) + (size_t)((g.HW + 3) & ~3) * sizeof(int32_t) + nms_smem_bytes(g.HW);
 }
 
+static long long persistent_grid(long long items, int sms, int ctas_per_sm, int max_ctas) {
+    long long n = std::min<long long>(items, (long long)sms * ctas_per_sm);
+    return max_ctas > 0 ? std::min<long long>(n, max_ctas) : n;
+}
+
 cudaError_t launch_decode_nms(const void* head, const Geom& g, int n_parts, float det_thr, float nms_thr,
                               int32_t* keep_cell, int32_t* keep_count, cudaStream_t st, bool pdl_attr, int pdl_bits,
-                              int ctas_per_sm, int threads_pref) {
+                              int ctas_per_sm, int threads_pref, int max_ctas, ChainPub* publish) {
+    if (publish) *publish = ChainPub{};
     if (g.B == 0 || n_parts == 0) return cudaSuccess;
     DeviceInfo* d = nullptr;
     cudaError_t e = device_info(&d);
@@ -2486,13 +2551,29 @@
     const size_t smem = decode_nms_smem_bytes(g);
     if (smem > (size_t)d->smem_optin) return cudaErrorInvalidConfiguration;
     const long long lists = (long long)g.B * n_parts;
-    dim3 grid((unsigned)(ctas_per_sm > 0 ? std::min<long long>(lists, (long long)d->sms * ctas_per_sm) : lists));
+    dim3 grid((unsigned)(ctas_per_sm > 0 ? persistent_grid(lists, d->sms, ctas_per_sm, max_ctas) : lists));
+    int* ticket = nullptr;
+    if (ctas_per_sm > 0 && (e = ticket_for(d, st, &ticket, kTicketLists)) != cudaSuccess) return e;
+    int* pub = nullptr;
+    int seq = 0;
+    if (publish && ticket) {
+        StreamSlot* slot = nullptr;
+        int* words = nullptr;
+        if ((e = slot_for(d, st, &slot, &words)) != cudaSuccess) return e;
+        if (slot) {
+            std::lock_guard<std::mutex> lock(g_ticket_mu);
+            pub = words + kListsPubWord;
+            seq = slot->lists_published++;
+        }
+    }
     PPN_DISPATCH_HEAD(g.dtype, {
         if ((e = ensure_smem(decode_nms_kernel<T>, smem, &d->decode_nms[g.dtype])) != cudaSuccess) return e;
         const int threads = threads_pref > 0 ? std::min(512, std::max(64, (threads_pref + 31) & ~31)) : (g.HW <= 256 ? 256 : 512);
-        return launch_kernel(decode_nms_kernel<T>, grid, dim3(threads), smem, st, pdl_attr,
-                             static_cast<const T*>(head), g, n_parts, det_thr, nms_thr, keep_cell, keep_count,
-                             pdl_bits | (g_nms_blockwise.load() ? NMS_BLOCKWISE : 0));
+        e = launch_kernel(decode_nms_kernel<T>, grid, dim3(threads), smem, st, pdl_attr,
+                          static_cast<const T*>(head), g, n_parts, det_thr, nms_thr, keep_cell, keep_count,
+                          pdl_bits | (g_nms_blockwise.load() ? NMS_BLOCKWISE : 0), ticket, pub, seq);
+        if (e == cudaSuccess && pub) *publish = ChainPub{pub, seq + 1};
+        return e;
     });
     return cudaErrorInvalidValue;
 }
@@ -2543,7 +2624,8 @@
                               const uint16_t* amax, const int32_t* cand_cell, const int32_t* keep_idx,
                               const int32_t* keep_count, int32_t* h_count, int32_t* h_root, int32_t* h_cell,
                               float* h_score, float* h_box, int R, cudaStream_t st, bool pdl_attr, int pdl_bits,
-                              int stage_all_pref, int threads_pref, int chain_mode, int ctas_per_sm) {
+                              int stage_all_pref, int threads_pref, int chain_mode, int ctas_per_sm, int max_ctas,
+                              ChainPub lists_done) {
     if (g.B == 0) return cudaSuccess;
     DeviceInfo* d = nullptr;
     cudaError_t e = device_info(&d);
@@ -2557,7 +2639,9 @@
     const bool tma_ok = ((size_t)g.K * g.HW * 2 * es) % 16 == 0 && (g.img_stride * es) % 16 == 0 &&
                         ((size_t)g.E * g.HW * 2) % 16 == 0 && (reinterpret_cast<uintptr_t>(head) & 15) == 0 &&
                         (reinterpret_cast<uintptr_t>(amax) & 15) == 0;
-    const dim3 grid((unsigned)(ctas_per_sm > 0 ? std::min<long long>(g.B, (long long)d->sms * ctas_per_sm) : g.B));
+    const dim3 grid((unsigned)(ctas_per_sm > 0 ? persistent_grid(g.B, d->sms, ctas_per_sm, max_ctas) : g.B));
+    int* ticket = nullptr;
+    if (ctas_per_sm > 0 && (e = ticket_for(d, st, &ticket, kTicketImages)) != cudaSuccess) return e;
     StreamSlot* slot = nullptr;
     int* words = nullptr;
     int bits = pdl_bits, seq = 0;
@@ -2575,13 +2659,13 @@
             e = launch_kernel(tree_parse_kernel<true, T>, grid, dim3(threads), smem, st, pdl_attr, static_cast<const T*>(head),
                               g, ch, thr, min_kp, n_parts, amax, cand_cell, keep_idx, keep_count, h_count, h_root, h_cell,
                               h_score, reinterpret_cast<float4*>(h_box), R, tma_ok ? 1 : 0, n_groups, bits, sync, seq,
-                              tree_parse_xywh_parts(g, n_groups));
+                              tree_parse_xywh_parts(g, n_groups), ticket, lists_done.word, lists_done.seq);
         } else {
             if ((e = ensure_smem(tree_parse_kernel<false, T>, smem, &d->tree_light[g.dtype])) != cudaSuccess) return e;
             e = launch_kernel(tree_parse_kernel<false, T>, grid, dim3(threads), smem, st, pdl_attr, static_cast<const T*>(head),
                               g, ch, thr, min_kp, n_parts, amax, cand_cell, keep_idx, keep_count, h_count, h_root, h_cell,
                               h_score, reinterpret_cast<float4*>(h_box), R, tma_ok ? 1 : 0, n_groups, bits, sync, seq,
-                              tree_parse_xywh_parts(g, n_groups));
+                              tree_parse_xywh_parts(g, n_groups), ticket, lists_done.word, lists_done.seq);
         }
     });
     if (e == cudaSuccess && slot) {
diff --git a/pytorch_pose_proposal_network_b200/csrc/ppn_kernels.h b/pytorch_pose_proposal_network_b200/csrc/ppn_kernels.h
--- a/pytorch_pose_proposal_network_b200/csrc/ppn_kernels.h
+++ b/pytorch_pose_proposal_network_b200/csrc/ppn_kernels.h
@@ -23,6 +23,7 @@
     int parse_chain_calls = 1;
     int parse_k12_threads = 0;
     int parse_persist = 1;
+    int parse_persist_grid = 0;
     int host_chunk_images = 64;
     int encode_sweep = 1;
     int encode_ctas_per_sm = 6;
@@ -65,9 +66,15 @@
 cudaError_t launch_nms(const float* box, const float* score, const int32_t* count, int n_problems, int stride,
                        float thr, int limit, int32_t* keep_idx, int32_t* keep_count, cudaStream_t st);
 
+enum : int { kTicketRing = 0, kTicketLists = 1, kTicketImages = 2, kTicketKinds = 3 };
+int ticket_pair_word(int kind, unsigned launch);
+
+struct ChainPub { int* word = nullptr; int seq = 0; };
+
 cudaError_t launch_decode_nms(const void* head, const Geom& g, int n_parts, float det_thr, float nms_thr,
                               int32_t* keep_cell, int32_t* keep_count, cudaStream_t st, bool pdl_attr = false,
-                              int pdl_bits = 0, int ctas_per_sm = 0 , int threads_pref = 0);
+                              int pdl_bits = 0, int ctas_per_sm = 0 , int threads_pref = 0,
+                              int max_ctas = 0 , ChainPub* publish = nullptr);
 size_t chain3_ring_cap(const Geom& g, int stage_all_pref, int k12_ctas);
 
 cudaError_t launch_restore_xy(const float* x, const float* y, float* rx, float* ry, size_t n, int H, int W,
@@ -91,7 +98,9 @@
                               const uint16_t* amax, const int32_t* cand_cell, const int32_t* keep_idx,
                               const int32_t* keep_count, int32_t* h_count, int32_t* h_root, int32_t* h_cell,
                               float* h_score, float* h_box, int R, cudaStream_t st, bool pdl_attr = false, int pdl_bits = 0,
-                              int stage_all_pref = -1, int threads_pref = 0, int chain_mode = 0 , int ctas_per_sm = 0 );
+                              int stage_all_pref = -1, int threads_pref = 0, int chain_mode = 0 , int ctas_per_sm = 0 ,
+                              int max_ctas = 0 ,
+                              ChainPub lists_done = {} );
 
 bool parse_fused_supported(const Geom& g, int stage_pref);
 struct FusedSplit { int n_sub, sub_B; bool staged; size_t smem, ring_cap; };
```

New measurement: 9.004 million (median of 6 runs). No clear change (+0.0%).
